# jordi-adell/mcarray

Hardware: AMD Instinct MI355X
Metric: STFT frames/sec, 8-mic GCC-PHAT + SRP-PHAT(361) + delay-and-sum beamform @48kHz/1024-pt (higher is better)
Workload: dtype f32 (SRP operands adaptive); 1 GPU; BASELINE configs[2] geometry (8-mic ULA 0.04 m, 48 kHz, N=1024, hop 512, 361 angles, 1 source, no power floor), 8 arrays x 4096 frames per GPU per step; channel rows padded by 64 floats; arrays_per_gpu=8, frames_per_array=4096, srp_precision=adaptive, parallelism=arrays sharded over 1 GPU(s), all_gather of DOA bins+prob

## Files before the change

include/mcarray_hip.h:

```cpp
#ifndef MCARRAY_HIP_H
#define MCARRAY_HIP_H

#ifdef __cplusplus
extern "C" {
#endif

typedef enum {
    MCA_HIP_OK = 0,
    MCA_HIP_ERR_INVALID_ARGUMENT = -1,
    MCA_HIP_ERR_HIP = -2,
    MCA_HIP_ERR_OUT_OF_MEMORY = -3,
    MCA_HIP_ERR_UNSUPPORTED = -4,
    MCA_HIP_ERR_NO_DEVICE = -5
} mca_hip_status;

typedef enum {
    MCA_HIP_SRP_FP32 = 0,
    MCA_HIP_SRP_FP16X3 = 1,
    MCA_HIP_SRP_FP16 = 2,
    MCA_HIP_SRP_ADAPTIVE = 3
} mca_hip_srp_precision;

typedef enum { MCA_HIP_GCC_PHAT = 0, MCA_HIP_GCC_NONE = 1 } mca_hip_gcc_weighting;

// ... 115 lines not shown
int mca_hip_mask_reset(mca_hip_mask_ctx *ctx);
int mca_hip_mask_get_thresholds(const mca_hip_mask_ctx *ctx, double *thresholds, double *center_freqs);
int mca_hip_mask_frames_dev(mca_hip_mask_ctx *ctx, const float *pcm_dev, long long stream_stride, long long ch_stride,
                            int n_streams, int n_frames, float *out_pcm_dev, int *decisions_dev, void *stream);
int mca_hip_mask_frames_host(mca_hip_mask_ctx *ctx, const float *pcm, int n_streams, int n_frames, float *out_pcm,
                             int *decisions);
int mca_hip_mask_process_frame(mca_hip_mask_ctx *ctx, double *left, double *right, int ccs_len, int *decisions);
long long mca_hip_mask_state_size(const mca_hip_mask_ctx *ctx);
int mca_hip_mask_state_save(mca_hip_mask_ctx *ctx, void *blob, long long blob_bytes);
int mca_hip_mask_state_load(mca_hip_mask_ctx *ctx, const void *blob, long long blob_bytes);

typedef struct mca_hip_mb_ctx mca_hip_mb_ctx;
typedef struct {
    int struct_size;
    int device;
    int sample_rate;
    int fft_size;
    const double *mic_xyz;
    int nbins;
    int use_power_floor;
    int max_arrays;
} mca_hip_mb_config;
int  mca_hip_mb_create(const mca_hip_mb_config *cfg, mca_hip_mb_ctx **out);
void mca_hip_mb_destroy(mca_hip_mb_ctx *ctx);
const char *mca_hip_mb_last_error(const mca_hip_mb_ctx *ctx);
int  mca_hip_mb_reset(mca_hip_mb_ctx *ctx, void *stream);
int  mca_hip_mb_num_steps(const mca_hip_mb_ctx *ctx);
int  mca_hip_mb_get_filters(const mca_hip_mb_ctx *ctx, double *out);
int mca_hip_mb_frames_dev(mca_hip_mb_ctx *ctx, const float *pcm_dev, long long array_stride, long long ch_stride,
                          int n_arrays, int n_frames, float *doa_rad_dev, float *prob_dev, unsigned char *voiced_dev,
                          float *power_dev, int *band_idx_dev, float *energy_in_doa_dev, float *band_corr_dev, void *stream);
int mca_hip_mb_frames_host(mca_hip_mb_ctx *ctx, const float *pcm, int n_arrays, int n_frames, float *doa_rad, float *prob,
                           unsigned char *voiced, float *power, int *band_idx, float *energy_in_doa, float *band_corr);
long long mca_hip_mb_state_size(const mca_hip_mb_ctx *ctx);
int mca_hip_mb_state_save(mca_hip_mb_ctx *ctx, void *blob, long long blob_bytes);
int mca_hip_mb_state_load(mca_hip_mb_ctx *ctx, const void *blob, long long blob_bytes);

typedef struct mca_hip_mvdr_ctx mca_hip_mvdr_ctx;
typedef struct {
    int struct_size;
    int device;
    int sample_rate;
    int fft_size;
    int n_mics;
    const double *mic_xyz;
    double alpha;
    double loading;
    int max_streams;
} mca_hip_mvdr_config;
int  mca_hip_mvdr_create(const mca_hip_mvdr_config *cfg, mca_hip_mvdr_ctx **out);
void mca_hip_mvdr_destroy(mca_hip_mvdr_ctx *ctx);
const char *mca_hip_mvdr_last_error(const mca_hip_mvdr_ctx *ctx);
int  mca_hip_mvdr_reset(mca_hip_mvdr_ctx *ctx, void *stream);
int mca_hip_mvdr_frames_dev(mca_hip_mvdr_ctx *ctx, const float *pcm_dev, long long stream_stride, long long mic_stride,
                            int n_streams, int n_frames, const float *doa_rad_dev, float *out_pcm_dev,
                            float *out_spec_dev, void *stream);
int mca_hip_mvdr_frames_host(mca_hip_mvdr_ctx *ctx, const float *pcm, int n_streams, int n_frames, const float *doa_rad,
                             float *out_pcm, float *out_spec);
int mca_hip_mvdr_get_covariance(mca_hip_mvdr_ctx *ctx, int stream_index, double *out);
long long mca_hip_mvdr_state_size(const mca_hip_mvdr_ctx *ctx);
int mca_hip_mvdr_state_save(mca_hip_mvdr_ctx *ctx, void *blob, long long blob_bytes);
int mca_hip_mvdr_state_load(mca_hip_mvdr_ctx *ctx, const void *blob, long long blob_bytes);
int mca_hip_mvdr_set_timing(mca_hip_mvdr_ctx *ctx, int enable);
int mca_hip_mvdr_get_timing(mca_hip_mvdr_ctx *ctx, int kernel_id, int *launches, double *total_ms);

typedef enum {
    MCA_HIP_K_STFT_PHAT = 0,
    MCA_HIP_K_SRP_GEMM = 1,
    MCA_HIP_K_SCAN_PICK = 2,
    MCA_HIP_K_BEAMFORM = 3,
    MCA_HIP_K_GCC2_SCAN = 4,
    MCA_HIP_K_MASK = 5,
    MCA_HIP_K_FOLD = 6,
    MCA_HIP_K_REPAIR = 7,
    MCA_HIP_K_COUNT = 8
} mca_hip_kernel_id;
int mca_hip_set_timing(mca_hip_ctx *ctx, int enable);
int mca_hip_set_timing_mask(mca_hip_ctx *ctx, unsigned kernel_mask);
int mca_hip_get_timing(mca_hip_ctx *ctx, int kernel_id, int *launches, double *total_ms);
int mca_hip_reset_timing(mca_hip_ctx *ctx);
int mca_hip_get_repair_stats(mca_hip_ctx *ctx, unsigned long long *frames, unsigned long long *flagged_frames,
                             unsigned long long *recomputed_frames);
int mca_hip_get_repair_columns(mca_hip_ctx *ctx, unsigned long long *candidate_columns, unsigned long long *whole_row_frames);

const char *mca_hip_version(void);

#ifdef __cplusplus
}
#endif
#endif
```

mcarray_amd/_lib.py:

```python
import ctypes as C
import os

_HERE = os.path.dirname(os.path.abspath(__file__))
LIB_PATH = os.environ.get("MCA_HIP_LIB", os.path.join(_HERE, "libmcarray_hip.so"))

c_dp = C.POINTER(C.c_double)
c_fp = C.POINTER(C.c_float)
c_ip = C.POINTER(C.c_int)


class MCArrayHipError(RuntimeError):
    """Raised for every non-zero status of the C ABI (the C++ side throws mca::MCArrayException)."""


class Config(C.Structure):
    _fields_ = [
        ("struct_size", C.c_int),
        ("device", C.c_int),
        ("sample_rate", C.c_int),
        ("fft_size", C.c_int),
        ("n_mics", C.c_int),
        ("mic_xyz", c_dp),
        ("doa_step_deg", C.c_double),
        ("n_sources", C.c_int),
# ... 66 lines not shown
    ("mca_hip_state_load", C.c_int, [C.c_void_p, C.c_void_p, C.c_longlong]),
    ("mca_hip_localise_frames_dev", C.c_int,
     [C.c_void_p, C.c_void_p, C.c_longlong, C.c_longlong, C.c_int, C.c_int, C.c_void_p, C.c_void_p, C.c_void_p,
      C.c_void_p, C.c_void_p]),
    ("mca_hip_separate_frames_dev", C.c_int,
     [C.c_void_p, C.c_void_p, C.c_longlong, C.c_longlong, C.c_int, C.c_int, C.c_void_p, C.c_void_p, C.c_void_p]),
    ("mca_hip_separate_frames_bins_dev", C.c_int,
     [C.c_void_p, C.c_void_p, C.c_longlong, C.c_longlong, C.c_int, C.c_int, C.c_void_p, C.c_void_p, C.c_void_p, C.c_void_p]),
    ("mca_hip_process_frames_dev", C.c_int,
     [C.c_void_p, C.c_void_p, C.c_longlong, C.c_longlong, C.c_int, C.c_int, C.c_void_p, C.c_void_p, C.c_void_p,
      C.c_void_p, C.c_void_p, C.c_void_p]),
    ("mca_hip_copy_gate", C.c_int, [C.c_void_p, C.c_void_p, c_fp]),
    ("mca_hip_process_frames_host", C.c_int,
     [C.c_void_p, c_fp, C.c_int, C.c_int, c_ip, c_fp, c_fp, c_fp, c_fp]),
    ("mca_hip_steering_process_frame", C.c_int,
     [C.c_void_p, C.POINTER(c_dp), C.c_int, c_dp, c_dp, c_ip, C.c_int]),
    ("mca_hip_beamformer_process_frame", C.c_int, [C.c_void_p, C.POINTER(c_dp), C.c_int, c_dp, C.c_double]),
    ("mca_hip_fft_log_power", C.c_int, [C.c_void_p, C.POINTER(c_dp), C.c_int, c_dp]),
    ("mca_hip_get_energy", C.c_int, [C.c_void_p, c_dp]),
    ("mca_hip_gcc2_frames_dev", C.c_int,
     [C.c_void_p, C.c_void_p, C.c_longlong, C.c_longlong, C.c_int, C.c_int, C.c_void_p, C.c_void_p, C.c_void_p,
      C.c_void_p, C.c_void_p]),
    ("mca_hip_gcc2_frames_host", C.c_int, [C.c_void_p, c_fp, C.c_int, C.c_int, c_ip, c_fp, c_fp, c_fp]),
    ("mca_hip_gcc2_set_probability", C.c_int, [C.c_void_p, C.c_int, c_dp, c_dp, C.c_int]),
    ("mca_hip_gcc2_set_probability_dev", C.c_int, [C.c_void_p, C.c_int, C.c_void_p, C.c_void_p, C.c_int, C.c_void_p]),
    ("mca_hip_gcc2_process_frame", C.c_int,
     [C.c_void_p, C.POINTER(c_dp), C.c_int, c_ip, c_dp, c_dp, c_dp, c_ip, c_dp]),
    ("mca_hip_gcc2_frame_set_probability", C.c_int, [C.c_void_p, c_dp, c_dp, C.c_int]),
    ("mca_hip_mask_create", C.c_int, [C.POINTER(MaskConfig), C.POINTER(C.c_void_p)]),
    ("mca_hip_mask_destroy", None, [C.c_void_p]),
    ("mca_hip_mask_last_error", C.c_char_p, [C.c_void_p]),
    ("mca_hip_mask_reset", C.c_int, [C.c_void_p]),
    ("mca_hip_mask_get_thresholds", C.c_int, [C.c_void_p, c_dp, c_dp]),
    ("mca_hip_mask_frames_dev", C.c_int,
     [C.c_void_p, C.c_void_p, C.c_longlong, C.c_longlong, C.c_int, C.c_int, C.c_void_p, C.c_void_p, C.c_void_p]),
    ("mca_hip_mask_frames_host", C.c_int, [C.c_void_p, c_fp, C.c_int, C.c_int, c_fp, c_ip]),
    ("mca_hip_mask_process_frame", C.c_int, [C.c_void_p, c_dp, c_dp, C.c_int, c_ip]),
    ("mca_hip_mb_create", C.c_int, [C.POINTER(MbConfig), C.POINTER(C.c_void_p)]),
    ("mca_hip_mb_destroy", None, [C.c_void_p]),
    ("mca_hip_mb_last_error", C.c_char_p, [C.c_void_p]),
    ("mca_hip_mb_reset", C.c_int, [C.c_void_p, C.c_void_p]),
    ("mca_hip_mb_num_steps", C.c_int, [C.c_void_p]),
    ("mca_hip_mb_get_filters", C.c_int, [C.c_void_p, c_dp]),
    ("mca_hip_mb_frames_dev", C.c_int,
     [C.c_void_p, C.c_void_p, C.c_longlong, C.c_longlong, C.c_int, C.c_int, C.c_void_p, C.c_void_p, C.c_void_p,
      C.c_void_p, C.c_void_p, C.c_void_p, C.c_void_p, C.c_void_p]),
    ("mca_hip_mb_frames_host", C.c_int,
     [C.c_void_p, c_fp, C.c_int, C.c_int, c_fp, c_fp, C.c_void_p, c_fp, c_ip, c_fp, c_fp]),
    ("mca_hip_process_frames_host_i16", C.c_int, [C.c_void_p, C.POINTER(C.c_short), C.c_int, C.c_int, c_ip, c_fp, c_fp, c_fp, c_fp]),
    ("mca_hip_graph_create", C.c_int,
     [C.c_void_p, C.c_void_p, C.c_longlong, C.c_longlong, C.c_int, C.c_int, C.c_void_p, C.c_void_p, C.c_void_p, C.c_void_p, C.c_void_p,
      C.POINTER(C.c_void_p)]),
    ("mca_hip_graph_launch", C.c_int, [C.c_void_p, C.c_void_p]),
    ("mca_hip_graph_destroy", None, [C.c_void_p]),
    ("mca_hip_mvdr_create", C.c_int, [C.POINTER(MvdrConfig), C.POINTER(C.c_void_p)]),
    ("mca_hip_mvdr_destroy", None, [C.c_void_p]),
    ("mca_hip_mvdr_last_error", C.c_char_p, [C.c_void_p]),
    ("mca_hip_mvdr_reset", C.c_int, [C.c_void_p, C.c_void_p]),
    ("mca_hip_mvdr_frames_dev", C.c_int,
     [C.c_void_p, C.c_void_p, C.c_longlong, C.c_longlong, C.c_int, C.c_int, C.c_void_p, C.c_void_p, C.c_void_p, C.c_void_p]),
    ("mca_hip_mvdr_frames_host", C.c_int, [C.c_void_p, c_fp, C.c_int, C.c_int, c_fp, c_fp, c_fp]),
    ("mca_hip_mvdr_get_covariance", C.c_int, [C.c_void_p, C.c_int, c_dp]),
    ("mca_hip_mvdr_set_timing", C.c_int, [C.c_void_p, C.c_int]),
    ("mca_hip_mvdr_get_timing", C.c_int, [C.c_void_p, C.c_int, c_ip, c_dp]),
    ("mca_hip_mask_state_size", C.c_longlong, [C.c_void_p]),
    ("mca_hip_mask_state_save", C.c_int, [C.c_void_p, C.c_void_p, C.c_longlong]),
    ("mca_hip_mask_state_load", C.c_int, [C.c_void_p, C.c_void_p, C.c_longlong]),
    ("mca_hip_mb_state_size", C.c_longlong, [C.c_void_p]),
    ("mca_hip_mb_state_save", C.c_int, [C.c_void_p, C.c_void_p, C.c_longlong]),
    ("mca_hip_mb_state_load", C.c_int, [C.c_void_p, C.c_void_p, C.c_longlong]),
    ("mca_hip_mvdr_state_size", C.c_longlong, [C.c_void_p]),
    ("mca_hip_mvdr_state_save", C.c_int, [C.c_void_p, C.c_void_p, C.c_longlong]),
    ("mca_hip_mvdr_state_load", C.c_int, [C.c_void_p, C.c_void_p, C.c_longlong]),
    ("mca_hip_set_timing", C.c_int, [C.c_void_p, C.c_int]),
    ("mca_hip_set_timing_mask", C.c_int, [C.c_void_p, C.c_uint]),
    ("mca_hip_get_timing", C.c_int, [C.c_void_p, C.c_int, c_ip, c_dp]),
    ("mca_hip_reset_timing", C.c_int, [C.c_void_p]),
    ("mca_hip_host_alloc", C.c_void_p, [C.c_longlong]),
    ("mca_hip_host_free", None, [C.c_void_p]),
    ("mca_hip_host_register", C.c_int, [C.c_void_p, C.c_longlong]),
    ("mca_hip_host_unregister", C.c_int, [C.c_void_p]),
    ("mca_hip_get_repair_stats", C.c_int, [C.c_void_p, C.POINTER(C.c_ulonglong), C.POINTER(C.c_ulonglong), C.POINTER(C.c_ulonglong)]),
    ("mca_hip_get_repair_columns", C.c_int, [C.c_void_p, C.POINTER(C.c_ulonglong), C.POINTER(C.c_ulonglong)]),
    ("mca_hip_version", C.c_char_p, []),
]

_LIB = None


def _pin_single_hip_runtime():
    import importlib.util
    spec = importlib.util.find_spec("torch")
    if spec is None or not spec.submodule_search_locations:
        return
    cand = os.path.join(list(spec.submodule_search_locations)[0], "lib", "libamdhip64.so")
    if os.path.exists(cand):
        C.CDLL(cand, mode=C.RTLD_GLOBAL)


def load():
    global _LIB
    if _LIB is None:
        if not os.path.exists(LIB_PATH):
            raise MCArrayHipError(
                "%s not found: the HIP extension is not built (run __graft_entry__.build()); "
                "mcarray_amd has no CPU fallback" % LIB_PATH)
        _pin_single_hip_runtime()
        lib = C.CDLL(LIB_PATH)
        for name, res, args in SYMBOLS:
            fn = getattr(lib, name)
            fn.restype = res
            fn.argtypes = args
        _LIB = lib
    return _LIB
```

mcarray_amd/api.py:

```python
import ctypes as C

import numpy as np

from . import _lib
from ._lib import MCArrayHipError

SRP_FP32, SRP_FP16X3, SRP_FP16, SRP_ADAPTIVE = 0, 1, 2, 3
GCC_PHAT, GCC_NONE = 0, 1
K_STFT_PHAT, K_SRP_GEMM, K_SCAN_PICK, K_BEAMFORM, K_GCC2_SCAN, K_MASK, K_FOLD, K_REPAIR = 0, 1, 2, 3, 4, 5, 6, 7
KERNEL_NAMES = {K_STFT_PHAT: "k_stft_phat", K_SRP_GEMM: "k_srp_gemm", K_SCAN_PICK: "k_scan_pick", K_BEAMFORM: "k_beamform_ola",
                K_FOLD: "k_sum_planes", K_REPAIR: "repair"}


class PinnedBuffer:

    def __init__(self, shape, dtype):
        self._lib = _lib.load()
        self.nbytes = int(np.prod(shape)) * np.dtype(dtype).itemsize
        self.ptr = self._lib.mca_hip_host_alloc(max(self.nbytes, 1))
        if not self.ptr:
            raise MCArrayHipError("mca_hip_host_alloc(%d) failed" % self.nbytes)
        raw = (C.c_char * max(self.nbytes, 1)).from_address(self.ptr)
        self.array = np.frombuffer(raw, dtype=dtype, count=int(np.prod(shape))).reshape(shape)

# ... 200 lines not shown
    def gcc2_set_probability(self, doas, array_index=0):
        doas = np.ascontiguousarray(doas, dtype=np.float64).reshape(-1)
        probs = np.empty(len(doas))
        self._check(self._lib.mca_hip_gcc2_set_probability(self.h, int(array_index), doas.ctypes.data_as(_lib.c_dp),
                                                           probs.ctypes.data_as(_lib.c_dp), len(doas)))
        return probs

    def gcc2_set_probability_dev(self, doas, probs, stream=None):
        if doas.dim() != 2 or tuple(probs.shape) != tuple(doas.shape) or not doas.is_contiguous() or not probs.is_contiguous():
            raise MCArrayHipError("doas and probs must be contiguous [A][n] tensors of one shape")
        A, n = doas.shape
        self._check(self._lib.mca_hip_gcc2_set_probability_dev(self.h, A, C.c_void_p(doas.data_ptr()), C.c_void_p(probs.data_ptr()), n,
                                                               stream))

    def gcc2_process_frame(self, frames):
        frames, arr = self._rows(frames)
        v, i = C.c_int(0), C.c_int(0)
        doa, prob, power = C.c_double(0), C.c_double(0), C.c_double(0)
        corr = np.empty(self.D)
        self._check(self._lib.mca_hip_gcc2_process_frame(self.h, arr, frames.shape[1], C.byref(v), C.byref(doa), C.byref(prob),
                                                         C.byref(power), C.byref(i), corr.ctypes.data_as(_lib.c_dp)))
        return dict(voiced=bool(v.value), doa=doa.value, prob=prob.value, power=power.value, argmax=i.value, corr=corr)

    def gcc2_frame_set_probability(self, doas):
        doas = np.ascontiguousarray(doas, dtype=np.float64).reshape(-1)
        probs = np.empty(len(doas))
        self._check(self._lib.mca_hip_gcc2_frame_set_probability(self.h, doas.ctypes.data_as(_lib.c_dp), probs.ctypes.data_as(_lib.c_dp),
                                                                 len(doas)))
        return probs

    def _rows(self, frames):
        frames = np.ascontiguousarray(frames, dtype=np.float64)
        if frames.shape[0] != self.M:
            raise MCArrayHipError("expected %d channel spectra" % self.M)
        arr = (_lib.c_dp * self.M)()
        for c in range(self.M):
            arr[c] = frames[c].ctypes.data_as(_lib.c_dp)
        return frames, arr

    def steering_process_frame(self, frames, n_sources=1):
        frames, arr = self._rows(frames)
        doa = np.empty(n_sources)
        prob = np.empty(n_sources)
        bins = np.empty(n_sources, dtype=np.int32)
        self._check(self._lib.mca_hip_steering_process_frame(self.h, arr, frames.shape[1], doa.ctypes.data_as(_lib.c_dp),
                                                             prob.ctypes.data_as(_lib.c_dp), bins.ctypes.data_as(_lib.c_ip),
                                                             n_sources))
        return doa, prob, bins

    def beamformer_process_frame(self, frames, doa):
        frames, arr = self._rows(frames)
        out = np.empty(frames.shape[1])
        self._check(self._lib.mca_hip_beamformer_process_frame(self.h, arr, frames.shape[1], out.ctypes.data_as(_lib.c_dp), float(doa)))
        return out

    def fft_log_power(self, frames):
        frames, arr = self._rows(frames)
        p = C.c_double(0)
        self._check(self._lib.mca_hip_fft_log_power(self.h, arr, frames.shape[1], C.byref(p)))
        return p.value

    def energy(self):
        out = np.empty(self.D)
        self._check(self._lib.mca_hip_get_energy(self.h, out.ctypes.data_as(_lib.c_dp)))
        return out

    def set_timing(self, enable):
        self._check(self._lib.mca_hip_set_timing(self.h, int(enable)))

    def set_timing_kernels(self, kernel_ids):
        mask = 0
        for k in kernel_ids:
            mask |= 1 << int(k)
        self._check(self._lib.mca_hip_set_timing_mask(self.h, mask))

    def reset_timing(self):
        self._check(self._lib.mca_hip_reset_timing(self.h))

    def repair_stats(self):
        a, b, c_ = C.c_ulonglong(0), C.c_ulonglong(0), C.c_ulonglong(0)
        self._check(self._lib.mca_hip_get_repair_stats(self.h, C.byref(a), C.byref(b), C.byref(c_)))
        return {"frames": a.value, "flagged": b.value, "recomputed": c_.value}

    def repair_columns(self):
        a, b = C.c_ulonglong(0), C.c_ulonglong(0)
        self._check(self._lib.mca_hip_get_repair_columns(self.h, C.byref(a), C.byref(b)))
        return {"candidate_columns": a.value, "whole_row_frames": b.value}

    def get_timing(self, kernel_id):
        n = C.c_int(0)
        ms = C.c_double(0)
        self._check(self._lib.mca_hip_get_timing(self.h, kernel_id, C.byref(n), C.byref(ms)))
        return n.value, ms.value


class StreamGraph:

    def __init__(self, ctx, h, keep):
        self.ctx, self.h, self._keep = ctx, h, keep
        self._lib = ctx._lib

    def launch(self, stream=None):
        rc = self.ctx._lib.mca_hip_graph_launch(self.h, stream)
        if rc != 0:
            raise MCArrayHipError("libmcarray_hip error %d: %s" % (rc, self.ctx._lib.mca_hip_last_error(self.ctx.h).decode()))

    def close(self):
        if getattr(self, "h", None):
            self._lib.mca_hip_graph_destroy(self.h)
        self.h = None

    def __del__(self):
        self.close()


class SteeringBeamforming:

    def __init__(self, sample_rate, mic_positions, fft_ccs_length, nchannels=None, doa_step_deg=5.0, device=0):
        self.ctx = Context(sample_rate, mic_positions, fft_ccs_length - 2, doa_step_deg, n_sources=4, device=device)
        if nchannels is not None and nchannels != self.ctx.M:
            raise MCArrayHipError("nchannels does not match the array description")

    def process_frame(self, analysis_frames, n_sources=1):
        return self.ctx.steering_process_frame(analysis_frames, n_sources)


class Beamformer:

    def __init__(self, sample_rate, mic_positions, fft_ccs_length, nchannels=None, device=0):
        self.ctx = Context(sample_rate, mic_positions, fft_ccs_length - 2, device=device)

    def process_frame(self, analysis_frames, doa):
        return self.ctx.beamformer_process_frame(analysis_frames, doa)


def calculate_order_from_sample_rate(sample_rate, frame_seconds):
    order = int(np.floor(np.log2(sample_rate * frame_seconds) + 0.5))
    return min(max(order, 8), 14)


class SourceSeparationAndLocalisation:

    FRAME_SECONDS = 0.025

    def __init__(self, sample_rate, mic_positions, n_sources=1, use_power_floor=False, doa_step_deg=5.0, fft_size=None,
                 srp_precision=SRP_FP32, device=0):
        if fft_size is None:
            fft_size = 1 << calculate_order_from_sample_rate(sample_rate, self.FRAME_SECONDS)
        self.ctx = Context(sample_rate, mic_positions, fft_size, doa_step_deg, n_sources, use_power_floor, srp_precision, 1, device)
        self.callback = None

    def set_callback(self, cb):
        self.callback = cb

    def process(self, pcm):
        r = self.ctx.process_frames_host(np.asarray(pcm, dtype=np.float32)[None], want_energy=False, want_audio=True)
        if self.callback is not None:
            deg = r["doa"][0].astype(np.float64) * (180.0 / np.pi)
            for t in range(deg.shape[0]):
                if "voiced" in r and not r["voiced"][0, t]:
                    continue
                self.callback(deg[t], r["prob"][0, t], r["power"][0, t] if "power" in r else None, self.ctx.S)
        return r["out"][0], r


class SourceLocalisation(SourceSeparationAndLocalisation):
# ... 309 lines not shown
```

mcarray_amd/csrc/api.hip:

```cpp
#include "../../include/mcarray_hip.h"
#include "fft1024c.h"
#include "kernels.h"
#include "knobs.h"
#include "stage.h"

#include <chrono>
#include <cmath>
#include <cstdio>
#include <cstdlib>
#include <cstring>
#include <string>
#include <thread>
#include <vector>

using namespace mca;

namespace {

std::string g_create_error;

struct TimedEvent { int id; hipEvent_t a, b; };

}

struct mca_hip_graph;

#define MCA_MAX_LANES 1

constexpr int FB_LAG = 2, FB_RING = 64, FB_WAIT_MS = 4000;
struct Knobs {
    bool fb_enabled = true;
    long long adapt_min_rows = 4096;
    int adapt_max_sources = 1;
    double tau_scale = 1.0;
    long long ws_max_bytes = 4LL << 30;
    bool force_generic = false;
    bool no_n2048 = false;
    bool scan_carry = false;
    int cand = -1;
    bool lazy_tails = true;
};

constexpr int REPAIR_ITEMS = 768;
constexpr int LIST_GRID = 512;
constexpr int CAND_GRID = 512;
constexpr int REPICK_GRID = 256;

struct Workspace {
    void *d_A = nullptr; size_t a_bytes = 0;
    void *d_Ax = nullptr; size_t ax_bytes = 0;
    float *d_C = nullptr; size_t c_bytes = 0;
    int c_planes = 1;
    bool partial_done = false;
    int part_planes = 1;
    long long c_plane = 0;
    float *d_Cx = nullptr; size_t cx_bytes = 0;
    float *d_part = nullptr, *d_estart = nullptr; int *d_nv = nullptr; size_t scan_ws_chunks = 0;
    float *d_power = nullptr; unsigned char *d_voiced = nullptr; float *d_power_out = nullptr; size_t gate_frames = 0;
    int *d_list_full = nullptr, *d_need_full = nullptr;
    unsigned char *d_flags = nullptr; int *d_chunk_from = nullptr, *d_list = nullptr, *d_need = nullptr; unsigned *d_umask = nullptr; size_t adapt_frames = 0, adapt_chunks = 0, adapt_groups = 0;
    unsigned char *d_unsure = nullptr;
    int *d_nlist = nullptr, *d_last_vchunk = nullptr; size_t lastv_arrays = 0;
    int last_a0 = 0, last_arrays = 0;
    void release()
    {
        auto F = [](void *q) { if (q) (void)hipFree(q); };
        F(d_A); F(d_Ax); F(d_C); F(d_Cx); F(d_part); F(d_estart); F(d_nv); F(d_power); F(d_voiced); F(d_power_out);
        F(d_flags); F(d_chunk_from); F(d_list); F(d_need); F(d_umask); F(d_nlist); F(d_last_vchunk); F(d_unsure); F(d_list_full); F(d_need_full);
        *this = Workspace();
    }
};

struct G2FrameState {
    double power_floor = 0, samples = 0, noise_estimated = 0;
    double silence = 0;
    double corr_mem = 0, doa_mem = 0;
    double doa = 0, prob = -1;
};

struct mca_hip_ctx {
    mca_hip_config cfg{};
    std::vector<double> xyz;
    int M = 0, P = 0, G = 0, D = 0, Dp = 0, K = 0, N = 0, H = 0, logH = 0, Kp = 0, S = 1, prec = 0;
    bool ula = false, stream_ok = false, generic = false;
    bool n512 = false;
    bool n2048 = false;
    std::string stream_why;
    float step = 0.f;
    std::vector<float> delays, grid;
    std::vector<int2> pairs;
    float *d_window = nullptr, *d_grid = nullptr, *d_delays = nullptr;
    float2 *d_tw = nullptr;
    double *d_micx = nullptr;
    int2 *d_pairs = nullptr;
    void *d_B = nullptr, *d_Bt = nullptr;
    bool merged = false; int n_merged = 0, Kp_m = 0;
    void *d_Bm = nullptr, *d_Btm = nullptr; unsigned short *d_mrank = nullptr;
    float2 *d_bftab = nullptr; int bf_pairs = 0;
    float *d_E[2] = {nullptr, nullptr};
    float *d_tail[2] = {nullptr, nullptr};
    int e_cur = 0, tail_cur = 0;
    Workspace lanes[MCA_MAX_LANES];
    int cur_lane = 0, a0 = 0;
    long long plan_rows = 0;
    int plan_arrays = 0;
    int n_lanes_last = 1;
    hipStream_t io_stream[3] = {}; hipEvent_t io_ev[8] = {};
    Workspace &ws() { return lanes[cur_lane]; }
    double *d_gate_state = nullptr;
    int *d_last_bin = nullptr; float *d_last_rad = nullptr, *d_last_prob = nullptr;
    int last_arrays = 0, last_frames = 0;
    float *d_doa[2] = {nullptr, nullptr};
    int doa_cur = 0;
    long long gcc2_frames_done = 0;
    long long *d_vdone[2] = {nullptr, nullptr};
    int *d_g2_vidx = nullptr, *d_g2_nv = nullptr; float *d_g2_rad = nullptr, *d_g2_prob = nullptr; size_t g2_rows = 0;
    unsigned char *d_g2_reset = nullptr;
    int *d_g2_post0 = nullptr;
    int *d_silence = nullptr;
    unsigned long long ws_gen = 0;
    std::vector<mca_hip_graph *> graphs;
    int tab_planes = 1;
    unsigned long long *d_rstats = nullptr;
    float *d_hist_pcm[2] = {nullptr, nullptr};
    float *d_hist_C[2] = {nullptr, nullptr};
    float *d_ehist[2] = {nullptr, nullptr};
    int hist_cur = 0, hist_n = 0;
    bool hist_pending = false;
    bool lazy_now = false;
    bool host_call = false;
    bool lazy_entry = false;
    int n_cu = 256;
    unsigned long long adapt_frames_total = 0;
    float tau_en = 0.f;
    Knobs kn;
    bool adapt_suspended = false, capturing = false;
    int fb_left = 0, fb_backoff = 8, fb_state = 0;
    bool cand_heavy = false;
    unsigned long long fb_probe_seq = 0;
    unsigned long long *h_probe = nullptr;
    unsigned long long fb_calls = 0, fb_seq_seen = 0, fb_groups_prev = 0, fb_frames_prev = 0, fb_flagged_prev = 0;
    unsigned long long fb_frames_ring[FB_RING] = {};
    unsigned long long fb_m = 0;
    unsigned long long fb_launch_m[FB_RING] = {};
    bool fb_lost = false;
    int a_row_elems = 0, a_planes = 1, a_elem = 4;
    double *d_fr = nullptr; size_t fr_elems = 0;
    double *d_E64[2] = {nullptr, nullptr}; int e64_cur = 0;
    double *d_res = nullptr;
    int *d_bins = nullptr;
    double *d_out64 = nullptr; size_t out64_elems = 0;
    double *d_g2f_corr[2] = {nullptr, nullptr}; int g2f_cur = 0;
    double *d_g2f_res = nullptr;
    G2FrameState g2f;
    std::vector<double> h_stage;
    StagePool stage;
    unsigned timing = 0;
    bool timing_open = false;
    std::vector<TimedEvent> events;
    std::vector<hipEvent_t> pool;
    int t_launches[MCA_HIP_K_COUNT] = {};
    double t_ms[MCA_HIP_K_COUNT] = {};
    std::string err;
};

namespace {

int fail(mca_hip_ctx *c, int code, const std::string &msg)
{
    if (c) c->err = msg; else g_create_error = msg;
    return code;
}

#define HIP_TRY(ctx, expr)                                                                              \
    do {                                                                                                \
        hipError_t _e = (expr);                                                                         \
        if (_e != hipSuccess)                                                                           \
            return fail(ctx, _e == hipErrorOutOfMemory ? MCA_HIP_ERR_OUT_OF_MEMORY : MCA_HIP_ERR_HIP,   \
                        std::string(#expr) + ": " + hipGetErrorString(_e));                            \
    } while (0)

double speed_of_sound() { return 346.1; }
float doa_idx2angle(int idx, float step) { float pr = (float)idx * step; return (float)((double)pr - M_PI_2); }
float doa_to_delay_far_field(float doa, float microDist)
{
    return (float)(((double)microDist * std::sin((double)doa)) / speed_of_sound());
}
float doa_to_delay_samples(float doa, float microDist, int fs) { return doa_to_delay_far_field(doa, microDist) * (float)fs; }
double distance(const std::vector<double> &xyz, int i, int j)
{
    return std::sqrt(std::pow(xyz[3 * j] - xyz[3 * i], 2) + std::pow(xyz[3 * j + 1] - xyz[3 * i + 1], 2) +
                     std::pow(xyz[3 * j + 2] - xyz[3 * i + 2], 2));
}

void free_ctx(mca_hip_ctx *c)
{
    if (!c) return;
    auto F = [](void *p) { if (p) (void)hipFree(p); };
    F(c->d_window); F(c->d_tw); F(c->d_grid); F(c->d_delays); F(c->d_micx); F(c->d_pairs); F(c->d_B); F(c->d_Bt); F(c->d_bftab); F(c->d_Bm); F(c->d_Btm); F(c->d_mrank);
    F(c->d_E[0]); F(c->d_E[1]); F(c->d_tail[0]); F(c->d_tail[1]); F(c->d_doa[0]); F(c->d_doa[1]); F(c->d_vdone[0]); F(c->d_vdone[1]); F(c->d_g2_vidx); F(c->d_g2_nv); F(c->d_g2_rad); F(c->d_g2_prob);
    F(c->d_g2_reset); F(c->d_g2_post0); F(c->d_silence);
    F(c->d_rstats); F(c->d_gate_state);
    for (int i = 0; i < 2; ++i) { F(c->d_hist_pcm[i]); F(c->d_hist_C[i]); F(c->d_ehist[i]); }
    if (c->h_probe) (void)hipHostFree(c->h_probe);
    for (Workspace &w : c->lanes) w.release();
    for (auto &e : c->io_ev) if (e) (void)hipEventDestroy(e);
    for (auto &q : c->io_stream) if (q) (void)hipStreamDestroy(q);
    F(c->d_last_bin); F(c->d_last_rad); F(c->d_last_prob);
    F(c->d_fr); F(c->d_E64[0]); F(c->d_E64[1]); F(c->d_res); F(c->d_bins); F(c->d_out64);
    F(c->d_g2f_corr[0]); F(c->d_g2f_corr[1]); F(c->d_g2f_res);
    c->stage.release();
    for (auto &e : c->events) { (void)hipEventDestroy(e.a); (void)hipEventDestroy(e.b); }
    for (auto &e : c->pool) (void)hipEventDestroy(e);
    delete c;
}

int round_up(int v, int m) { return (v + m - 1) / m * m; }

Knobs read_knobs(const mca_hip_config &cfg)
{
    Knobs k;
    auto geti = [](const char *v, long long dflt) { return v ? std::atoll(v) : dflt; };
    k.fb_enabled = cfg.adaptive_fallback != MCA_HIP_ADAPT_FALLBACK_OFF;
    if (const char *v = env_str("MCA_HIP_ADAPT_FALLBACK")) k.fb_enabled = std::atoi(v) != 0;
    k.adapt_min_rows = geti(env_str("MCA_HIP_ADAPT_MIN_ROWS"), cfg.adaptive_min_rows > 0 ? cfg.adaptive_min_rows : 4096);
    k.adapt_max_sources = (int)geti(env_str("MCA_HIP_ADAPT_MAX_SOURCES"), cfg.adaptive_max_sources > 0 ? cfg.adaptive_max_sources : 1);
    if (const char *v = env_str("MCA_HIP_ADAPT_TAU_SCALE")) k.tau_scale = std::atof(v);
    if (const char *v = env_str("MCA_HIP_WS_MAX_MB")) k.ws_max_bytes = (long long)std::atoll(v) << 20;
    k.force_generic = env_str("MCA_HIP_FORCE_GENERIC") != nullptr;
    k.scan_carry = cfg.scan_carry != 0 || env_str("MCA_HIP_SCAN_CARRY") != nullptr;
    if (const char *v = env_str("MCA_HIP_ADAPT_LAZY")) k.lazy_tails = std::atoi(v) != 0;
    if (const char *v = env_str("MCA_HIP_ADAPT_CAND")) k.cand = std::atoi(v) != 0 ? 1 : 0;
    k.no_n2048 = env_str("MCA_HIP_NO_N2048") != nullptr;
    return k;
}

int init_last_state(mca_hip_ctx *c, hipStream_t st)
{
    const size_t n = (size_t)c->cfg.max_arrays * MCA_MAX_SOURCES;
    std::vector<int> b(n, -1); std::vector<float> pr(n, -1.f);
    HIP_TRY(c, hipMemcpyAsync(c->d_last_bin, b.data(), n * 4, hipMemcpyHostToDevice, st));
    HIP_TRY(c, hipMemsetAsync(c->d_last_rad, 0, n * 4, st));
    HIP_TRY(c, hipMemcpyAsync(c->d_last_prob, pr.data(), n * 4, hipMemcpyHostToDevice, st));
    HIP_TRY(c, hipMemsetAsync(c->d_gate_state, 0, (size_t)c->cfg.max_arrays * 4 * 8, st));
    HIP_TRY(c, hipStreamSynchronize(st));
    return MCA_HIP_OK;
}

int build_steering_table(mca_hip_ctx *c)
{
    const int K = c->K, D = c->D, Dp = c->Dp, Kp = c->Kp;
    std::vector<int> first_pair(c->G);
    if (c->ula) { for (int g = 0; g < c->G; ++g) first_pair[g] = g;  }
    else for (int g = 0; g < c->G; ++g) first_pair[g] = g;
    const double N = 2.0 * (K - 1);
    if (c->prec == MCA_HIP_SRP_FP32) {
        std::vector<float> B((size_t)Kp * Dp, 0.f);
        for (int g = 0; g < c->G; ++g)
            for (int k = 0; k < K; ++k)
                for (int d = 0; d < D; ++d) {
                    double ph = 2.0 * M_PI * (double)k * (double)c->delays[(size_t)first_pair[g] * D + d] / N;
                    size_t r = ((size_t)g * K + k) * 2;
                    B[r * Dp + d] = (float)std::cos(ph);
                    B[(r + 1) * Dp + d] = (float)(-std::sin(ph));
                }
        HIP_TRY(c, hipMalloc(&c->d_B, B.size() * sizeof(float)));
        HIP_TRY(c, hipMemcpy(c->d_B, B.data(), B.size() * sizeof(float), hipMemcpyHostToDevice));
    } else {
        const int planes = c->tab_planes;
        std::vector<_Float16> B((size_t)planes * Dp * Kp, (_Float16)0.f);
        for (int g = 0; g < c->G; ++g)
            for (int d = 0; d < D; ++d)
                for (int k = 0; k < K; ++k) {
                    double ph = 2.0 * M_PI * (double)k * (double)c->delays[(size_t)first_pair[g] * D + d] / N;
                    float v[2] = {(float)std::cos(ph), (float)(-std::sin(ph))};
                    for (int q = 0; q < 2; ++q) {
                        size_t kk = ((size_t)g * K + k) * 2 + q;
                        _Float16 hi = (_Float16)v[q];
                        B[(size_t)d * Kp + kk] = hi;
                        if (planes == 2) B[((size_t)Dp + d) * Kp + kk] = (_Float16)(v[q] - (float)hi);
                    }
                }
        HIP_TRY(c, hipMalloc(&c->d_B, B.size() * sizeof(_Float16)));
        HIP_TRY(c, hipMemcpy(c->d_B, B.data(), B.size() * sizeof(_Float16), hipMemcpyHostToDevice));
        if (Dp == 384) {
            const int ns32 = Kp / 32;
            std::vector<_Float16> Bt(B.size());
// ... 382 lines not shown
{
    StftPhatArgs sa = a;
    const int fp = c->M == 4 ? 2 : 1, mr = c->M == 4 ? 4 : 8;
    if (!sa.list) {
        sa.fpb = 16;
        while (sa.fpb > 2 && (long long)grid.y * ((sa.n_frames + sa.fpb - 1) / sa.fpb) < 512) sa.fpb >>= 1;
        grid.x = (sa.n_frames + sa.fpb - 1) / sa.fpb;
    }
    const size_t smem6 = ((size_t)fp * mr * 1026 + F1K_TWORDS + 8 * F1K_SCRATCH + (size_t)sa.fpb * c->M) * sizeof(float2) + (size_t)sa.fpb * 8 * sizeof(float);
#define L2048(MT, U)                                                                                                      \
    do {                                                                                                                  \
        HIP_TRY(c, hipFuncSetAttribute(reinterpret_cast<const void *>(&k_stft_phat_2048<MT, U, OutT, false>), hipFuncAttributeMaxDynamicSharedMemorySize, (int)smem6)); \
        hipLaunchKernelGGL((k_stft_phat_2048<MT, U, OutT, false>), grid, dim3(512), smem6, st, sa);                              \
    } while (0)
    bool done = false;
    if constexpr (sizeof(OutT) == 2) {
        if (sa.mrank && sa.a_planes == 1 && !sa.list && c->ula && (c->M == 8 || c->M == 4)) {
            if (c->M == 8) {
                HIP_TRY(c, hipFuncSetAttribute(reinterpret_cast<const void *>(&k_stft_phat_2048<8, true, _Float16, true>), hipFuncAttributeMaxDynamicSharedMemorySize, (int)smem6));
                hipLaunchKernelGGL((k_stft_phat_2048<8, true, _Float16, true>), grid, dim3(512), smem6, st, sa);
            } else {
                HIP_TRY(c, hipFuncSetAttribute(reinterpret_cast<const void *>(&k_stft_phat_2048<4, true, _Float16, true>), hipFuncAttributeMaxDynamicSharedMemorySize, (int)smem6));
                hipLaunchKernelGGL((k_stft_phat_2048<4, true, _Float16, true>), grid, dim3(512), smem6, st, sa);
            }
            done = true;
        }
    }
    if (done) { }
    else if (c->M == 8 && c->ula) L2048(8, true); else if (c->M == 8) L2048(8, false);
    else if (c->M == 4 && c->ula) L2048(4, true); else if (c->M == 4) L2048(4, false);
    else if (c->ula) L2048(0, true); else L2048(0, false);
#undef L2048
    HIP_TRY(c, hipGetLastError());
    return MCA_HIP_OK;
}

template <typename OutT>
int launch_stft(mca_hip_ctx *c, const StftPhatArgs &a, dim3 grid, size_t smem, hipStream_t st)
{
    const int M = c->M; const bool ula = c->ula;
    if (n2048_analysis(c)) return launch_stft_2048<OutT>(c, a, grid, st);
    if (c->n512) return launch_stft_512<OutT>(c, a, grid, st);
    if constexpr (sizeof(OutT) == 2) {
        if (wave16_applies(c) && a.a_planes == 1 && !a.list) {
            StftPhatArgs w = a;
            w.fpb = 16;
            while (w.fpb > 1 && (long long)grid.y * ((a.n_frames + w.fpb - 1) / w.fpb) < 2048) w.fpb >>= 1;
            dim3 gw(((a.n_frames + w.fpb - 1) / w.fpb + 3) / 4, grid.y);
            if ((gw.x & 1) == 0 && (long long)gw.x * gw.y == 2LL * c->n_cu && (long long)gw.x * 4 * w.fpb == a.n_frames) {
                const int sk = (3 * w.fpb + 8) / 16;
                if (sk > 0 && sk < w.fpb) { w.skew = sk; gw = dim3(gw.y, gw.x); }
            }
            const int fpa = w.fpb + w.skew;
            const size_t smw = (size_t)(F1K_TWORDS + 4 * F1K_SCRATCH + 2 * 4 * fpa * 8) * sizeof(float2) + (1024 + 4 * fpa) * sizeof(float);
            if (a.power) {
                HIP_TRY(c, hipFuncSetAttribute(reinterpret_cast<const void *>(&k_stft_phat_wave16<true>), hipFuncAttributeMaxDynamicSharedMemorySize, (int)smw));
                hipLaunchKernelGGL(k_stft_phat_wave16<true>, gw, dim3(256), smw, st, w);
            } else {
                HIP_TRY(c, hipFuncSetAttribute(reinterpret_cast<const void *>(&k_stft_phat_wave16<false>), hipFuncAttributeMaxDynamicSharedMemorySize, (int)smw));
                hipLaunchKernelGGL(k_stft_phat_wave16<false>, gw, dim3(256), smw, st, w);
            }
            HIP_TRY(c, hipGetLastError());
            return MCA_HIP_OK;
        }
    }
    if (M == 8 || M == 4) {
        StftPhatArgs w = a;
        dim3 gw;
        if (a.list) { w.fpb = 1; gw = dim3(grid.x, 1); }
        else {
            w.fpb = 16;
            while (w.fpb > 1 && (long long)grid.y * ((a.n_frames + w.fpb - 1) / w.fpb) < 2048) w.fpb >>= 1;
            gw = dim3(((a.n_frames + w.fpb - 1) / w.fpb + 3) / 4, grid.y);
        }
        if (!a.list && M == 8 && (gw.x & 1) == 0 && (long long)gw.x * gw.y == 2LL * c->n_cu && (long long)gw.x * 4 * w.fpb == a.n_frames) {
            const int sk = (3 * w.fpb + 8) / 16;
            if (sk > 0 && sk < w.fpb) {
                w.skew = sk;
                gw = dim3(gw.y, gw.x);
            }
        }
        const bool mg = w.mrank != nullptr && !a.list;
        const int nrank = 2 * (M - 1) * 64 * 4 + 8, regw = mg ? std::max(F1K_SCRATCH, (w.n_merged + 63) & ~63) : F1K_SCRATCH;
        const size_t smw = (size_t)(F1K_TWORDS + (mg ? nrank / 4 : 0) + 4 * regw + (mg ? 0 : 4 * (w.fpb + w.skew) * (M / 2))) * sizeof(float2);
        const bool pl2 = a.a_planes == 2, pw = a.power != nullptr;
#define LAUNCH_K(K)                                                                                                 \
        do {                                                                                                         \
            if (smw > 64 * 1024) HIP_TRY(c, hipFuncSetAttribute(reinterpret_cast<const void *>(&K), hipFuncAttributeMaxDynamicSharedMemorySize, (int)smw)); \
            hipLaunchKernelGGL(K, gw, dim3(256), smw, st, w);                                                        \
        } while (0)
#define LAUNCH_W2(MT, U, PL2, NP)                                                                                  \
        do {                                                                                                         \
            if (pw) LAUNCH_K((k_stft_phat_wave<MT, U, OutT, PL2, true, NP, false>));                                 \
            else LAUNCH_K((k_stft_phat_wave<MT, U, OutT, PL2, false, NP, false>));                                   \
        } while (0)
#define LAUNCH_W(MT, U)                                                                                              \
        do {                                                                                                         \
            if constexpr (sizeof(OutT) == 2) {                                                                       \
                if (pl2 && w.cand_on && a.list && !pw) LAUNCH_K((k_stft_phat_wave<MT, U, OutT, true, false, false, false, true>)); \
                else if (pl2) LAUNCH_W2(MT, U, true, false); else LAUNCH_W2(MT, U, false, false);                    \
            }                                                                                                        \
            else { if (a.no_phat) LAUNCH_W2(MT, U, false, true); else LAUNCH_W2(MT, U, false, false); }              \
        } while (0)
        if constexpr (sizeof(OutT) == 2) {
            if (mg) {
                if (M == 8) { if (pw) LAUNCH_K((k_stft_phat_wave<8, true, OutT, false, true, false, true>)); else LAUNCH_K((k_stft_phat_wave<8, true, OutT, false, false, false, true>)); }
                else { if (pw) LAUNCH_K((k_stft_phat_wave<4, true, OutT, false, true, false, true>)); else LAUNCH_K((k_stft_phat_wave<4, true, OutT, false, false, false, true>)); }
                HIP_TRY(c, hipGetLastError());
                return MCA_HIP_OK;
            }
        }
        if (M == 8 && ula) LAUNCH_W(8, true); else if (M == 8) LAUNCH_W(8, false);
        else if (ula) LAUNCH_W(4, true); else LAUNCH_W(4, false);
#undef LAUNCH_W2
#undef LAUNCH_K
#undef LAUNCH_W
        HIP_TRY(c, hipGetLastError());
        return MCA_HIP_OK;
    }
#define LAUNCH(MT, U)                                                                                        \
    do {                                                                                                     \
        if (smem > 64 * 1024)                                                                                \
            HIP_TRY(c, hipFuncSetAttribute(reinterpret_cast<const void *>(&k_stft_phat<MT, U, OutT>),        \
                                           hipFuncAttributeMaxDynamicSharedMemorySize, (int)smem));          \
        hipLaunchKernelGGL((k_stft_phat<MT, U, OutT>), grid, dim3(512), smem, st, a);                        \
    } while (0)
#define LAUNCH_FEW(MT, U)                                                                                    \
    do {                                                                                                     \
        const size_t smf = ((size_t)8 * FFT_SCRATCH + TW_WORDS + (size_t)a.fpb * MT) * sizeof(float2) + (size_t)a.fpb * 8 * sizeof(float); \
        if (smf > 64 * 1024)                                                                                 \
            HIP_TRY(c, hipFuncSetAttribute(reinterpret_cast<const void *>(&k_stft_phat_few<MT, U, OutT>),    \
                                           hipFuncAttributeMaxDynamicSharedMemorySize, (int)smf));           \
        hipLaunchKernelGGL((k_stft_phat_few<MT, U, OutT>), grid, dim3(512), smf, st, a);                     \
    } while (0)
    if (M == 2 && !ula) LAUNCH_FEW(2, false);
    else if (M == 16 && ula) LAUNCH(16, true);
    else if (ula) LAUNCH(0, true);
    else LAUNCH(0, false);
#undef LAUNCH
#undef LAUNCH_FEW
    HIP_TRY(c, hipGetLastError());
    return MCA_HIP_OK;
}

int check_stream_args(mca_hip_ctx *c, const float *pcm, long long array_stride, long long mic_stride, int n_arrays, int n_frames)
{
    if (!c) return MCA_HIP_ERR_INVALID_ARGUMENT;
    if (!c->stream_ok) return fail(c, MCA_HIP_ERR_UNSUPPORTED, c->stream_why);
    if (!pcm) return fail(c, MCA_HIP_ERR_INVALID_ARGUMENT, "pcm_dev is NULL");
    if (n_arrays < 1 || n_arrays > c->cfg.max_arrays) return fail(c, MCA_HIP_ERR_INVALID_ARGUMENT, "n_arrays outside [1, max_arrays]");
    if (n_frames < 1) return fail(c, MCA_HIP_ERR_INVALID_ARGUMENT, "n_frames < 1");
    const long long need = (long long)(n_frames + 1) * c->H;
    if (mic_stride < need) return fail(c, MCA_HIP_ERR_INVALID_ARGUMENT, "mic_stride shorter than (n_frames+1)*hop samples");
    if (n_arrays > 1 && array_stride < (long long)(c->M - 1) * mic_stride + need) return fail(c, MCA_HIP_ERR_INVALID_ARGUMENT, "array_stride too short");
    if ((mic_stride & 1) || (array_stride & 1) || (reinterpret_cast<uintptr_t>(pcm) & 7))
        return fail(c, MCA_HIP_ERR_INVALID_ARGUMENT, "pcm_dev must be 8-byte aligned with even strides (float2 loads)");
    return MCA_HIP_OK;
}

}

extern "C" {

static int settle_history(mca_hip_ctx *c, hipStream_t st);

const char *mca_hip_version(void) { return "mcarray-hip 0.1.0 (gfx950)"; }

const char *mca_hip_last_error(const mca_hip_ctx *ctx) { return ctx ? ctx->err.c_str() : g_create_error.c_str(); }

int mca_hip_create(const mca_hip_config *cfg, mca_hip_ctx **out)
{
    if (!cfg || !out) return fail(nullptr, MCA_HIP_ERR_INVALID_ARGUMENT, "cfg/out is NULL");
    *out = nullptr;
    constexpr int size_r2 = (int)offsetof(mca_hip_config, gcc_weighting), size_r3 = (size_r2 + 4 + 7) / 8 * 8;
    static_assert(size_r3 <= (int)offsetof(mca_hip_config, adaptive_min_rows), "round-3 struct size");
    if (cfg->struct_size != (int)sizeof(mca_hip_config) && cfg->struct_size != size_r2 && cfg->struct_size != size_r3)
        return fail(nullptr, MCA_HIP_ERR_INVALID_ARGUMENT, "struct_size mismatch");
    mca_hip_config cfg_full{};
    std::memcpy(&cfg_full, cfg, cfg->struct_size == size_r3 ? (size_t)offsetof(mca_hip_config, adaptive_fallback) : (size_t)cfg->struct_size);
    cfg_full.struct_size = (int)sizeof(mca_hip_config);
    cfg = &cfg_full;
    if (cfg->gcc_weighting != MCA_HIP_GCC_PHAT && cfg->gcc_weighting != MCA_HIP_GCC_NONE)
        return fail(nullptr, MCA_HIP_ERR_INVALID_ARGUMENT, "gcc_weighting must be MCA_HIP_GCC_PHAT or MCA_HIP_GCC_NONE");
    if (cfg->gcc_weighting == MCA_HIP_GCC_NONE && cfg->srp_precision != MCA_HIP_SRP_FP32)
        return fail(nullptr, MCA_HIP_ERR_UNSUPPORTED, "gcc_weighting NONE needs srp_precision MCA_HIP_SRP_FP32 (un-normalised spectra do not fit fp16 operands)");
    if (cfg->n_mics < 2 || cfg->n_mics > MCA_MAX_MICS) return fail(nullptr, MCA_HIP_ERR_INVALID_ARGUMENT, "n_mics must be in [2,16]");
    if (!cfg->mic_xyz) return fail(nullptr, MCA_HIP_ERR_INVALID_ARGUMENT, "mic_xyz is NULL");
    if (cfg->n_sources < 1 || cfg->n_sources > MCA_MAX_SOURCES) return fail(nullptr, MCA_HIP_ERR_INVALID_ARGUMENT, "n_sources must be in [1,4]");
    if (cfg->fft_size < 16 || (cfg->fft_size & 1) || cfg->fft_size > 8192) return fail(nullptr, MCA_HIP_ERR_INVALID_ARGUMENT, "fft_size must be even, 16..8192");
// ... 105 lines not shown
        (rc = zalloc((void **)&c->d_tail[0], na * c->S * c->H * 4)) || (rc = zalloc((void **)&c->d_tail[1], na * c->S * c->H * 4)) ||
        (rc = zalloc((void **)&c->d_gate_state, na * 4 * 8)) || (rc = zalloc((void **)&c->d_last_bin, na * MCA_MAX_SOURCES * 4)) ||
        (rc = zalloc((void **)&c->d_last_rad, na * MCA_MAX_SOURCES * 4)) || (rc = zalloc((void **)&c->d_last_prob, na * MCA_MAX_SOURCES * 4)) ||
        (rc = zalloc((void **)&c->d_doa[0], na * 4)) || (rc = zalloc((void **)&c->d_doa[1], na * 4)) ||
        (rc = zalloc((void **)&c->d_vdone[0], na * 8)) || (rc = zalloc((void **)&c->d_vdone[1], na * 8)) ||
        (rc = zalloc((void **)&c->d_silence, na * 4)) || (rc = zalloc((void **)&c->d_g2_post0, na * 4)) ||
        (rc = zalloc((void **)&c->d_rstats, 32)) ||
        (rc = zalloc((void **)&c->d_E64[0], c->D * 8)) || (rc = zalloc((void **)&c->d_E64[1], c->D * 8)) ||
        (rc = zalloc((void **)&c->d_res, (2 * MCA_MAX_SOURCES + 1) * 8)) || (rc = zalloc((void **)&c->d_bins, MCA_MAX_SOURCES * 4)) ||
        (rc = zalloc((void **)&c->d_g2f_corr[0], c->D * 8)) || (rc = zalloc((void **)&c->d_g2f_corr[1], c->D * 8)) ||
        (rc = zalloc((void **)&c->d_g2f_res, 4 * 8))) {
        g_create_error = c->err; free_ctx(c); return rc;
    }
    if (lazy_context(c)) {
        for (int i = 0; i < 2; ++i)
            if ((rc = zalloc((void **)&c->d_hist_pcm[i], na * c->M * HIST_SAMPLES * 4)) || (rc = zalloc((void **)&c->d_hist_C[i], na * HIST_FRAMES * c->Dp * 4)) ||
                (rc = zalloc((void **)&c->d_ehist[i], na * c->D * 4))) { g_create_error = c->err; free_ctx(c); return rc; }
    }
    if (c->prec == MCA_HIP_SRP_ADAPTIVE && c->kn.fb_enabled) {
        if (hipHostMalloc((void **)&c->h_probe, FB_RING * 32, hipHostMallocDefault) == hipSuccess) std::memset(c->h_probe, 0, FB_RING * 32);
        else { c->h_probe = nullptr; (void)hipGetLastError(); }
    }
    if (c->stream_ok && ((rc = build_steering_table(c)) || (rc = build_merged_tables(c)))) { g_create_error = c->err; free_ctx(c); return rc; }
    if ((rc = init_last_state(c, nullptr))) { g_create_error = c->err; free_ctx(c); return rc; }
    *out = c;
    return MCA_HIP_OK;
}

static void graph_drop_recordings(mca_hip_graph *g);
static void graph_orphan(mca_hip_graph *g);

void mca_hip_destroy(mca_hip_ctx *ctx)
{
    if (!ctx) return;
    (void)hipSetDevice(ctx->cfg.device);
    (void)hipDeviceSynchronize();
    for (mca_hip_graph *g : ctx->graphs) graph_orphan(g);
    ctx->graphs.clear();
    free_ctx(ctx);
}

int mca_hip_num_steps(const mca_hip_ctx *c) { return c ? c->D : MCA_HIP_ERR_INVALID_ARGUMENT; }
int mca_hip_num_pairs(const mca_hip_ctx *c) { return c ? c->P : MCA_HIP_ERR_INVALID_ARGUMENT; }
int mca_hip_num_groups(const mca_hip_ctx *c) { return c ? c->G : MCA_HIP_ERR_INVALID_ARGUMENT; }

int mca_hip_get_pair_delays(const mca_hip_ctx *c, float *out)
{
    if (!c || !out) return MCA_HIP_ERR_INVALID_ARGUMENT;
    std::memcpy(out, c->delays.data(), c->delays.size() * sizeof(float));
    return MCA_HIP_OK;
}

int mca_hip_get_doa_grid(const mca_hip_ctx *c, float *out)
{
    if (!c || !out) return MCA_HIP_ERR_INVALID_ARGUMENT;
    std::memcpy(out, c->grid.data(), c->grid.size() * sizeof(float));
    return MCA_HIP_OK;
}

int mca_hip_reset(mca_hip_ctx *c, void *stream)
{
    if (!c) return MCA_HIP_ERR_INVALID_ARGUMENT;
    hipStream_t st = (hipStream_t)stream;
    const size_t na = (size_t)c->cfg.max_arrays;
    for (int i = 0; i < 2; ++i) {
        HIP_TRY(c, hipMemsetAsync(c->d_E[i], 0, na * c->D * 4, st));
        HIP_TRY(c, hipMemsetAsync(c->d_tail[i], 0, na * c->S * c->H * 4, st));
        HIP_TRY(c, hipMemsetAsync(c->d_E64[i], 0, (size_t)c->D * 8, st));
        HIP_TRY(c, hipMemsetAsync(c->d_g2f_corr[i], 0, (size_t)c->D * 8, st));
        HIP_TRY(c, hipMemsetAsync(c->d_doa[i], 0, na * 4, st));
        HIP_TRY(c, hipMemsetAsync(c->d_vdone[i], 0, na * 8, st));
    }
    HIP_TRY(c, hipMemsetAsync(c->d_silence, 0, na * 4, st));
    c->adapt_suspended = false; c->fb_state = 0; c->fb_left = 0; c->fb_backoff = 8; c->cand_heavy = false;
    c->fb_lost = false; c->fb_seq_seen = c->fb_calls;
    c->hist_pending = false;
    for (Workspace &w : c->lanes) {
        if (w.d_need) HIP_TRY(c, hipMemsetAsync(w.d_need, 0, w.adapt_groups * 4, st));
        if (w.d_need_full) HIP_TRY(c, hipMemsetAsync(w.d_need_full, 0, w.adapt_groups * 4, st));
        if (w.d_umask) HIP_TRY(c, hipMemsetAsync(w.d_umask, 0, w.adapt_groups * (c->Dp / 32) * 4, st));
        if (w.d_chunk_from) HIP_TRY(c, hipMemsetAsync(w.d_chunk_from, 0x7f, w.adapt_chunks * 4, st));
        if (w.d_nlist) HIP_TRY(c, hipMemsetAsync(w.d_nlist, 0, 16, st));
    }
    c->gcc2_frames_done = 0;
    c->g2f = G2FrameState();
    return init_last_state(c, st);
}

extern "C++" {
namespace {

struct StateHeader {
    unsigned magic; int version, M, D, S, H, max_arrays, use_floor;
    unsigned delays_hash;
    long long gcc2_frames_done;
};
constexpr unsigned STATE_MAGIC = 0x4d434153u;
constexpr int STATE_VERSION = 3;

unsigned delays_hash(const mca_hip_ctx *c)
{
    unsigned h = 2166136261u;
    const unsigned char *p = reinterpret_cast<const unsigned char *>(c->delays.data());
    for (size_t i = 0; i < c->delays.size() * sizeof(float); ++i) { h ^= p[i]; h *= 16777619u; }
    return h;
}

struct StatePart { void *ptr; size_t bytes; };
std::vector<StatePart> state_parts(mca_hip_ctx *c)
{
    const size_t na = (size_t)c->cfg.max_arrays;
    return {
        {c->d_E[c->e_cur], na * c->D * 4}, {c->d_tail[c->tail_cur], na * c->S * c->H * 4}, {c->d_gate_state, na * 4 * 8},
        {c->d_last_bin, na * MCA_MAX_SOURCES * 4}, {c->d_last_rad, na * MCA_MAX_SOURCES * 4}, {c->d_last_prob, na * MCA_MAX_SOURCES * 4},
        {c->d_doa[c->doa_cur], na * 4}, {c->d_E64[c->e64_cur], (size_t)c->D * 8}, {c->d_vdone[c->doa_cur], na * 8},
        {c->d_silence, na * 4},
        {c->d_g2f_corr[c->g2f_cur], (size_t)c->D * 8},
    };
}

size_t frame_part_bytes(const mca_hip_ctx *c) { return (size_t)c->D * 8 + sizeof(G2FrameState); }
static_assert(sizeof(G2FrameState) == 8 * sizeof(double), "G2FrameState is the 8 doubles of the blob");

}
}

long long mca_hip_state_size(const mca_hip_ctx *c)
{
    if (!c) return MCA_HIP_ERR_INVALID_ARGUMENT;
    long long n = sizeof(StateHeader) + (long long)sizeof(G2FrameState);
    for (const StatePart &p : state_parts(const_cast<mca_hip_ctx *>(c))) n += (long long)p.bytes;
    return n;
}

int mca_hip_state_save(mca_hip_ctx *c, void *blob, long long blob_bytes)
{
    if (!c) return MCA_HIP_ERR_INVALID_ARGUMENT;
    if (!blob || blob_bytes < mca_hip_state_size(c)) return fail(c, MCA_HIP_ERR_INVALID_ARGUMENT, "state blob is NULL or smaller than mca_hip_state_size()");
    HIP_TRY(c, hipSetDevice(c->cfg.device));
    if (c->hist_pending) {
        HIP_TRY(c, hipDeviceSynchronize());
        const int rc = settle_history(c, nullptr);
        if (rc) return rc;
    }
    HIP_TRY(c, hipDeviceSynchronize());
    StateHeader h{STATE_MAGIC, STATE_VERSION, c->M, c->D, c->S, c->H, c->cfg.max_arrays, c->cfg.use_power_floor, delays_hash(c), c->gcc2_frames_done};
    unsigned char *out = static_cast<unsigned char *>(blob);
    std::memcpy(out, &h, sizeof(h)); out += sizeof(h);
    for (const StatePart &p : state_parts(c)) { HIP_TRY(c, hipMemcpy(out, p.ptr, p.bytes, hipMemcpyDeviceToHost)); out += p.bytes; }
    std::memcpy(out, &c->g2f, sizeof(G2FrameState));
    return MCA_HIP_OK;
}

int mca_hip_state_load(mca_hip_ctx *c, const void *blob, long long blob_bytes)
{
    if (!c) return MCA_HIP_ERR_INVALID_ARGUMENT;
    if (!blob || blob_bytes < (long long)sizeof(StateHeader)) return fail(c, MCA_HIP_ERR_INVALID_ARGUMENT, "state blob is NULL or truncated");
    StateHeader h;
    std::memcpy(&h, blob, sizeof(h));
    if (h.magic != STATE_MAGIC || h.version < 1 || h.version > STATE_VERSION) return fail(c, MCA_HIP_ERR_INVALID_ARGUMENT, "not a state blob of this library version");
    if (h.M != c->M || h.D != c->D || h.S != c->S || h.H != c->H || h.max_arrays != c->cfg.max_arrays || h.use_floor != c->cfg.use_power_floor ||
        h.delays_hash != delays_hash(c))
        return fail(c, MCA_HIP_ERR_INVALID_ARGUMENT, "state blob was saved by a context with a different configuration");
    const long long short_by = (h.version == 1 ? (long long)c->cfg.max_arrays * 4 : 0) +
                               (h.version < 3 ? (long long)frame_part_bytes(c) : 0);
    if (blob_bytes < mca_hip_state_size(c) - short_by) return fail(c, MCA_HIP_ERR_INVALID_ARGUMENT, "state blob is truncated");
    HIP_TRY(c, hipSetDevice(c->cfg.device));
    HIP_TRY(c, hipDeviceSynchronize());
    const unsigned char *in = static_cast<const unsigned char *>(blob) + sizeof(h);
    for (const StatePart &p : state_parts(c)) {
        if (h.version == 1 && p.ptr == c->d_silence) { HIP_TRY(c, hipMemset(p.ptr, 0, p.bytes)); continue; }
        if (h.version < 3 && p.ptr == c->d_g2f_corr[c->g2f_cur]) { HIP_TRY(c, hipMemset(p.ptr, 0, p.bytes)); continue; }
        HIP_TRY(c, hipMemcpy(p.ptr, in, p.bytes, hipMemcpyHostToDevice)); in += p.bytes;
    }
    if (h.version >= 3) std::memcpy(&c->g2f, in, sizeof(G2FrameState));
    else c->g2f = G2FrameState();
    c->gcc2_frames_done = h.gcc2_frames_done;
    c->hist_pending = false;
    return MCA_HIP_OK;
}

static int reserve_lane(mca_hip_ctx *c, int n_arrays, int n_frames)
{
    const int n_chunks = (n_frames + SCAN_CHUNK - 1) / SCAN_CHUNK;
    int rc;
    if (c->prec == MCA_HIP_SRP_ADAPTIVE && adaptive_shape(c, n_arrays, n_frames)) {
        set_call_planes(c, 1);
        if ((rc = ensure_adapt_workspace(c, n_arrays, n_frames, n_chunks))) return rc;
        const long long fc1 = chunk_frames_for(c, n_arrays, n_frames);
        if ((rc = ensure_workspace(c, (long long)n_arrays * fc1, (long long)n_arrays * n_frames))) return rc;
        if (!c->adapt_suspended) return ensure_scan_workspace(c, n_arrays, n_frames, n_chunks);
    }
    if (c->prec == MCA_HIP_SRP_ADAPTIVE) set_call_planes(c, 2);
    long long fc = chunk_frames_for(c, n_arrays, n_frames);
    rc = ensure_workspace(c, (long long)n_arrays * fc, (long long)n_arrays * n_frames);
    if (rc) return rc;
    return ensure_scan_workspace(c, n_arrays, n_frames, n_chunks);
}

static int reserve_impl(mca_hip_ctx *c, int n_arrays, int n_frames)
{
    HIP_TRY(c, hipSetDevice(c->cfg.device));
    c->cur_lane = 0;
    return reserve_lane(c, n_arrays, n_frames);
}

int mca_hip_reserve(mca_hip_ctx *c, int n_arrays, int n_frames)
{
    if (!c || n_arrays < 1 || n_frames < 1) return MCA_HIP_ERR_INVALID_ARGUMENT;
    return reserve_impl(c, n_arrays, n_frames);
}

static int run_correlation_map(mca_hip_ctx *c, const float *pcm, long long array_stride, long long mic_stride,
                               int n_arrays, int n_frames, hipStream_t st)
{
    int rc;
    const long long fc = chunk_frames_for(c, n_arrays, n_frames);
    if ((rc = ensure_workspace(c, (long long)n_arrays * fc, (long long)n_arrays * n_frames))) return rc;
    if ((rc = ensure_scan_workspace(c, n_arrays, n_frames, (n_frames + SCAN_CHUNK - 1) / SCAN_CHUNK))) return rc;
    bool fused_partial = SCAN_CHUNK == 32 && c->a_planes == 1 && !c->cfg.use_power_floor && n_frames % SCAN_CHUNK == 0 && fc % SCAN_CHUNK == 0 &&
                         plan_gemm(c, (long long)n_arrays * fc).ksplit <= 2;
    for (int f0 = 0; fused_partial && f0 < n_frames; f0 += (int)fc)
        fused_partial = plan_gemm(c, (long long)n_arrays * std::min<long long>(fc, n_frames - f0)).v2;
    c->ws().partial_done = fused_partial;
    c->ws().part_planes = fused_partial ? plan_gemm(c, (long long)n_arrays * fc).ksplit : 1;
    for (int f0 = 0; f0 < n_frames; f0 += (int)fc) {
        const int nf = (int)std::min<long long>(fc, n_frames - f0);
        StftPhatArgs sa{};
        sa.pcm = pcm; sa.array_stride = array_stride; sa.mic_stride = mic_stride;
        sa.M = c->M; sa.n_frames = nf; sa.frame0 = f0;
        sa.fpb = 16;
        while (sa.fpb > 1 && (long long)n_arrays * ((nf + sa.fpb - 1) / sa.fpb) < 256) sa.fpb >>= 1;
        sa.power = c->cfg.use_power_floor ? c->ws().d_power : nullptr; sa.total_frames = n_frames;
        sa.window = c->d_window; sa.A = a_buf(c); sa.Kp = c->Kp; sa.a_row_elems = c->a_row_elems; sa.a_planes = c->a_planes;
        if (c->merged && c->a_planes == 1) { sa.mrank = c->d_mrank; sa.n_merged = c->n_merged; }
        sa.N = c->N; sa.logH = c->logH; sa.kg = c->K; sa.ula = c->ula ? 1 : 0; sa.tw = c->d_tw;
        sa.no_phat = c->cfg.gcc_weighting == MCA_HIP_GCC_NONE ? 1 : 0;
        if (c->prec == MCA_HIP_SRP_ADAPTIVE && c->a_planes == 1 && wave16_applies(c)) sa.unsure = c->ws().d_unsure;
        if (c->lazy_now && cand_call(c, true)) sa.dead = c->ws().d_unsure;
        if (c->lazy_now) sa.hist_out = c->d_hist_pcm[c->hist_cur ^ 1];
        time_begin(c, MCA_HIP_K_STFT_PHAT, st);
        if (c->n512) {
            rc = c->prec == MCA_HIP_SRP_FP32 ? launch_stft_512<float>(c, sa, dim3(0, n_arrays), st) : launch_stft_512<_Float16>(c, sa, dim3(0, n_arrays), st);
        } else if ((c->N == 4096 || c->N == 2048) && c->M == 2 && c->stream_ok) {
            sa.fpb = 8;
            while (sa.fpb > 2 && (long long)n_arrays * ((nf + sa.fpb - 1) / sa.fpb) < 512) sa.fpb >>= 1;
            const size_t smem4 = ((size_t)16 * 258 + 8 * FFT_SCRATCH + TW_WIN) * sizeof(float2) + 4 * 8 * sizeof(float);
            dim3 g4((nf + sa.fpb - 1) / sa.fpb, n_arrays);
#define LSUB(RR, T)                                                                                                       \
            do {                                                                                                          \
                HIP_TRY(c, hipFuncSetAttribute(reinterpret_cast<const void *>(&k_stft_phat_sub2<RR, T>), hipFuncAttributeMaxDynamicSharedMemorySize, (int)smem4)); \
                hipLaunchKernelGGL((k_stft_phat_sub2<RR, T>), g4, dim3(512), smem4, st, sa);                              \
            } while (0)
            if (c->N == 4096) { if (c->prec == MCA_HIP_SRP_FP32) LSUB(8, float); else LSUB(8, _Float16); }
            else { if (c->prec == MCA_HIP_SRP_FP32) LSUB(4, float); else LSUB(4, _Float16); }
#undef LSUB
            rc = MCA_HIP_OK;
        } else if (n2048_analysis(c)) {
            rc = c->prec == MCA_HIP_SRP_FP32 ? launch_stft_2048<float>(c, sa, dim3(0, n_arrays), st) : launch_stft_2048<_Float16>(c, sa, dim3(0, n_arrays), st);
        } else if (c->generic) {
            const size_t smem1 = (size_t)c->M * (c->H + 1) * sizeof(float2) + 16;
#define GEN_LAUNCH(K)                                                                                                     \
            do {                                                                                                          \
                if (smem1 > 64 * 1024)                                                                                    \
                    HIP_TRY(c, hipFuncSetAttribute(reinterpret_cast<const void *>(&K), hipFuncAttributeMaxDynamicSharedMemorySize, (int)smem1)); \
                hipLaunchKernelGGL(K, dim3(nf, n_arrays), dim3(gen_threads(c, false)), smem1, st, sa);                                      \
            } while (0)
            if (c->prec == MCA_HIP_SRP_FP32) GEN_LAUNCH(k_stft_phat_gen<float>);
            else GEN_LAUNCH(k_stft_phat_gen<_Float16>);
#undef GEN_LAUNCH
            rc = MCA_HIP_OK;
        } else {
            dim3 g1((nf + sa.fpb - 1) / sa.fpb, n_arrays);
            const size_t smem1 = ((size_t)c->M * FFT_SCRATCH + TW_WORDS + (size_t)sa.fpb * c->M) * sizeof(float2) + (size_t)sa.fpb * 8 * sizeof(float);
            rc = c->prec == MCA_HIP_SRP_FP32 ? launch_stft<float>(c, sa, g1, smem1, st) : launch_stft<_Float16>(c, sa, g1, smem1, st);
        }
        time_end(c, st);
        if (rc) return rc;

        GemmArgs ga{};
        const bool mg = c->merged && c->a_planes == 1;
        ga.A = a_buf(c); ga.B = mg ? c->d_Bm : c->d_B; ga.C = c->ws().d_C; ga.Bt = mg ? c->d_Btm : c->d_Bt;
        ga.rows = n_arrays * nf; ga.chunk_frames = nf; ga.total_frames = n_frames; ga.frame0 = f0;
        ga.Kp = cur_kp(c); ga.Dp = c->Dp; ga.a_row_elems = c->a_row_elems;
        ga.c_plane_elems = (long long)n_arrays * n_frames * c->Dp;
        if (fused_partial) {
            ga.part = c->ws().d_part; ga.nvoiced = c->ws().d_nv; ga.D = c->D; ga.n_chunks = n_frames / SCAN_CHUNK;
            ga.part_plane_stride = (long long)n_arrays * ga.n_chunks * c->D;
            ga.scan_w[31] = 1 - 0.8f;
            for (int t = 30; t >= 0; --t) ga.scan_w[t] = ga.scan_w[t + 1] * 0.8f;
        }
        const bool v2 = plan_gemm(c, ga.rows).v2;
        const int ksplit = plan_gemm(c, (long long)n_arrays * fc).ksplit;
        c->ws().c_planes = ksplit; c->ws().c_plane = ga.c_plane_elems;
        time_begin(c, MCA_HIP_K_SRP_GEMM, st);
        if (v2) {
            const int np = c->a_planes;
            const size_t smem = (size_t)(np == 2 ? 2 : 4) * np * (256 + 384) * 64;
            dim3 gv((ga.rows + 255) / 256, ksplit);
#define V2_LAUNCH(K)                                                                                                      \
            do {                                                                                                          \
                HIP_TRY(c, hipFuncSetAttribute(reinterpret_cast<const void *>(&K), hipFuncAttributeMaxDynamicSharedMemorySize, (int)smem)); \
                hipLaunchKernelGGL(K, gv, dim3(512), smem, st, ga);                                                       \
            } while (0)
            if (c->a_planes == 2) V2_LAUNCH(k_srp_gemm_f16_v2);
            else V2_LAUNCH(k_srp_gemm_f16_v3);
#undef V2_LAUNCH
        } else {
            dim3 g2((ga.rows + 127) / 128, c->Dp == 64 ? 1 : c->Dp / 192, ksplit);
            if (c->prec == MCA_HIP_SRP_FP32) hipLaunchKernelGGL(k_srp_gemm_f32, g2, dim3(256), 0, st, ga);
            else if (c->Dp == 64 && c->a_planes == 2) hipLaunchKernelGGL((k_srp_gemm_f16<true, 64>), g2, dim3(256), 0, st, ga);
            else if (c->Dp == 64) hipLaunchKernelGGL((k_srp_gemm_f16<false, 64>), g2, dim3(256), 0, st, ga);
            else if (c->a_planes == 2) hipLaunchKernelGGL((k_srp_gemm_f16<true, 192>), g2, dim3(256), 0, st, ga);
            else hipLaunchKernelGGL((k_srp_gemm_f16<false, 192>), g2, dim3(256), 0, st, ga);
        }
        time_end(c, st);
        HIP_TRY(c, hipGetLastError());
    }
    if (c->ws().c_planes > 2) {
        const long long n4 = c->ws().c_plane / 4;
        time_begin(c, MCA_HIP_K_FOLD, st);
        hipLaunchKernelGGL(k_sum_planes, dim3((unsigned)((n4 + 255) / 256)), dim3(256), 0, st, c->ws().d_C, n4, c->ws().c_planes, c->ws().c_plane);
        time_end(c, st);
// ... 159 lines not shown
        const int pass_groups = (int)(pass_rows / REPAIR_GROUP);
        const long long all_groups = (long long)n_arrays * (gpa + (hist_valid ? HIST_UNITS : 0));
        set_call_planes(c, 2);
        for (long long g0 = 0; g0 < all_groups; g0 += pass_groups) {
            StftPhatArgs sa{};
            sa.pcm = pcm; sa.array_stride = array_stride; sa.mic_stride = mic_stride;
            sa.M = c->M; sa.n_frames = n_frames; sa.frame0 = 0; sa.fpb = REPAIR_GROUP; sa.total_frames = n_frames;
            sa.window = c->d_window; sa.A = c->ws().d_Ax; sa.Kp = c->Kp; sa.a_row_elems = c->a_row_elems; sa.a_planes = 2;
            sa.N = c->N; sa.logH = c->logH; sa.kg = c->K; sa.ula = c->ula ? 1 : 0; sa.tw = c->d_tw;
            sa.list = c->ws().d_list; sa.n_list = c->ws().d_nlist; sa.list0 = (int)g0; sa.list_cap = pass_groups; sa.groups_per_array = gpa;
            if (hist_valid) { sa.hist_in = c->d_hist_pcm[c->hist_cur]; sa.hist_base = n_arrays * gpa; }
            CandArgs ca{};
            if (pa.umask) {
                ca.A = c->ws().d_Ax; ca.B = c->d_B; ca.Kp = c->Kp; ca.Dp = c->Dp; ca.a_row_elems = c->a_row_elems;
                ca.list = c->ws().d_list; ca.n_list = c->ws().d_nlist; ca.list0 = (int)g0; ca.pass_rows = (int)pass_rows;
                ca.umask = c->ws().d_umask; ca.umask_words = pa.umask_words; ca.need = c->ws().d_need; ca.groups_per_array = gpa; ca.n_frames = n_frames;
                ca.C = c->ws().d_C; ca.c_planes = c->ws().c_planes; ca.c_plane_stride = c->ws().c_plane;
                if (hist_valid) { ca.hist_C = c->d_hist_C[c->hist_cur]; ca.hist_base = n_arrays * gpa; }
                if (c->M == 8 || c->M == 4) { sa.cand_on = 1; sa.cand = ca; }
            }
            const size_t smem1 = ((size_t)c->M * FFT_SCRATCH + TW_WORDS + (size_t)sa.fpb * c->M) * sizeof(float2) + (size_t)sa.fpb * 8 * sizeof(float);
            if ((rc = launch_stft<_Float16>(c, sa, dim3(std::min(pass_groups, LIST_GRID), 1), smem1, st))) { set_call_planes(c, 1); return rc; }
            if (pa.umask && sa.cand_on) continue;
            if (pa.umask) {
                const long long max_items = pass_rows / REPAIR_GROUP;
                hipLaunchKernelGGL(k_srp_cand, dim3((unsigned)std::min<long long>(max_items, CAND_GRID)), dim3(1024), 0, st, ca);
                continue;
            }
            RepairPatchArgs pp{};
            pp.groups_per_array = gpa;
            pp.C = c->ws().d_C; pp.c_planes = c->ws().c_planes; pp.c_plane_stride = c->ws().c_plane; pp.n_frames = n_frames;
            if (hist_valid) { pp.hist_C = c->d_hist_C[c->hist_cur]; pp.hist_base = n_arrays * gpa; }
            launch_repair_contraction(c, c->ws(), g0, pass_rows, n_arrays, pp, st);
        }
        for (long long g0 = 0; mixed && g0 < all_groups; g0 += pass_groups) {
            StftPhatArgs sa{};
            sa.pcm = pcm; sa.array_stride = array_stride; sa.mic_stride = mic_stride;
            sa.M = c->M; sa.n_frames = n_frames; sa.frame0 = 0; sa.fpb = REPAIR_GROUP; sa.total_frames = n_frames;
            sa.window = c->d_window; sa.A = c->ws().d_Ax; sa.Kp = c->Kp; sa.a_row_elems = c->a_row_elems; sa.a_planes = 2;
            sa.N = c->N; sa.logH = c->logH; sa.kg = c->K; sa.ula = c->ula ? 1 : 0; sa.tw = c->d_tw;
            sa.list = pa.list_full; sa.n_list = pa.n_list_full; sa.list0 = (int)g0; sa.list_cap = pass_groups; sa.groups_per_array = gpa;
            const size_t smem1 = ((size_t)c->M * FFT_SCRATCH + TW_WORDS + (size_t)sa.fpb * c->M) * sizeof(float2) + (size_t)sa.fpb * 8 * sizeof(float);
            if ((rc = launch_stft<_Float16>(c, sa, dim3(std::min(pass_groups, LIST_GRID), 1), smem1, st))) { set_call_planes(c, 1); return rc; }
            RepairPatchArgs pp{};
            pp.groups_per_array = gpa;
            pp.C = c->ws().d_C; pp.c_planes = c->ws().c_planes; pp.c_plane_stride = c->ws().c_plane; pp.n_frames = n_frames;
            launch_repair_contraction(c, c->ws(), g0, pass_rows, n_arrays, pp, st, pa.list_full, pa.n_list_full, pa.need_full);
        }
        set_call_planes(c, 1);
        const size_t smem4 = (size_t)32 * (c->Dp + 8) * sizeof(float);
#define LAUNCH_REPICK(PL)                                                                                                           \
        do {                                                                                                                        \
            if (smem4 > 64 * 1024)                                                    \
                HIP_TRY(c, hipFuncSetAttribute(reinterpret_cast<const void *>(&k_scan_repick<PL>), hipFuncAttributeMaxDynamicSharedMemorySize, (int)smem4)); \
            hipLaunchKernelGGL((k_scan_repick<PL>), dim3((unsigned)std::min<long long>((long long)pa.n_chunks * n_arrays, REPICK_GRID)), dim3(std::max(nthr, 512)), smem4, st, pa); \
        } while (0)
        if (ppl == 2) LAUNCH_REPICK(2); else if (ppl == 6) LAUNCH_REPICK(6); else LAUNCH_REPICK(8);
#undef LAUNCH_REPICK
        if (gate) hipLaunchKernelGGL(k_doa_fill, dim3(n_arrays), dim3(1024), 0, st, fa);
        time_end(c, st);
        HIP_TRY(c, hipGetLastError());
        c->adapt_frames_total += (unsigned long long)n_arrays * n_frames;
    }
    if (lazy) { c->hist_cur ^= 1; c->hist_n = n_arrays; c->hist_pending = true; }
    else c->hist_pending = false;
    c->ws().last_a0 = c->a0; c->ws().last_arrays = n_arrays;
    return MCA_HIP_OK;
}

int mca_hip_get_repair_stats(mca_hip_ctx *c, unsigned long long *frames, unsigned long long *flagged_frames,
                             unsigned long long *recomputed_frames)
{
    if (!c) return MCA_HIP_ERR_INVALID_ARGUMENT;
    HIP_TRY(c, hipSetDevice(c->cfg.device));
    HIP_TRY(c, hipDeviceSynchronize());
    unsigned long long st[2] = {0, 0};
    HIP_TRY(c, hipMemcpy(st, c->d_rstats, sizeof(st), hipMemcpyDeviceToHost));
    if (frames) *frames = c->adapt_frames_total;
    if (flagged_frames) *flagged_frames = st[0];
    if (recomputed_frames) *recomputed_frames = st[1] * REPAIR_GROUP;
    return MCA_HIP_OK;
}

int mca_hip_get_repair_columns(mca_hip_ctx *c, unsigned long long *candidate_columns, unsigned long long *whole_row_frames)
{
    if (!c) return MCA_HIP_ERR_INVALID_ARGUMENT;
    HIP_TRY(c, hipSetDevice(c->cfg.device));
    HIP_TRY(c, hipDeviceSynchronize());
    unsigned long long st[4] = {0, 0, 0, 0};
    HIP_TRY(c, hipMemcpy(st, c->d_rstats, sizeof(st), hipMemcpyDeviceToHost));
    if (candidate_columns) *candidate_columns = st[2];
    if (whole_row_frames) *whole_row_frames = st[3];
    return MCA_HIP_OK;
}

static bool wave_beamformer_applies(const mca_hip_ctx *c)
{
    return !c->generic && !c->n512 && (c->S <= 2 || c->M <= 8) && c->M >= 2 && c->M <= MCA_MAX_MICS;
}

static int ensure_bf_table(mca_hip_ctx *c)
{
    if (!c->d_bftab && c->n2048) {
        HIP_TRY(c, hipMalloc((void **)&c->d_bftab, (size_t)(c->D + 1) * c->M * 1032 * sizeof(float2)));
        c->bf_pairs = c->M;
        const double unit = (double)c->cfg.sample_rate / (double)c->N / 346.1;
        hipLaunchKernelGGL(k_bf_table_2048, dim3(c->D + 1, c->M), dim3(256), 0, nullptr, c->d_bftab, c->d_grid, c->d_micx, c->M, unit);
        HIP_TRY(c, hipGetLastError());
        HIP_TRY(c, hipDeviceSynchronize());
        return MCA_HIP_OK;
    }
    if (c->d_bftab || !wave_beamformer_applies(c)) return MCA_HIP_OK;
    const int np = (c->M + 1) / 2;
    HIP_TRY(c, hipMalloc((void **)&c->d_bftab, (size_t)(c->D + 1) * np * 1024 * sizeof(float2)));
    c->bf_pairs = np;
    const double unit = (double)c->cfg.sample_rate / (double)FFT_N / 346.1;
    hipLaunchKernelGGL(k_bf_table, dim3(c->D + 1, np), dim3(256), 0, nullptr, c->d_bftab, c->d_grid, c->d_micx, c->M, np, unit);
    HIP_TRY(c, hipGetLastError());
    HIP_TRY(c, hipDeviceSynchronize());
    return MCA_HIP_OK;
}

static int separate_impl(mca_hip_ctx *c, const float *pcm, long long array_stride, long long mic_stride,
                         int n_arrays, int n_frames, const float *doa_rad, float *out_pcm, hipStream_t st, const int *doa_bin = nullptr)
{
    const size_t a0 = (size_t)c->a0;
    if (doa_bin && c->d_bftab && c->n2048 && (reinterpret_cast<uintptr_t>(out_pcm) & 7) == 0) {
        BeamformWaveArgs wa{};
        wa.pcm = pcm; wa.array_stride = array_stride; wa.mic_stride = mic_stride;
        wa.M = c->M; wa.n_pairs = c->M; wa.n_frames = n_frames; wa.S = c->S;
        wa.ft = 16;
        for (int ft = 2; ft <= 64; ++ft)
            if ((long long)n_arrays * c->S * ((n_frames + 4 * ft - 2) / (4 * ft - 1)) <= 2LL * c->n_cu) { wa.ft = ft; break; }
        wa.window = c->d_window; wa.doa_bin = doa_bin; wa.table = c->d_bftab; wa.out = out_pcm;
        wa.tail_in = c->d_tail[c->tail_cur] + a0 * c->S * c->H; wa.tail_out = c->d_tail[c->tail_cur ^ 1] + a0 * c->S * c->H;
        const int wgs = (n_frames + 4 * wa.ft - 2) / (4 * wa.ft - 1);
        const size_t smem_w = (size_t)(F1K_TWORDS + 4 * F1K_SCRATCH + 4 * 512) * sizeof(float2);
        time_begin(c, MCA_HIP_K_BEAMFORM, st);
        hipLaunchKernelGGL(k_beamform_wave_2048, dim3(wgs, n_arrays, c->S), dim3(256), smem_w, st, wa);
        time_end(c, st);
        HIP_TRY(c, hipGetLastError());
        return MCA_HIP_OK;
    }
    if (doa_bin && c->d_bftab && wave_beamformer_applies(c)) {
        BeamformWaveArgs wa{};
        wa.pcm = pcm; wa.array_stride = array_stride; wa.mic_stride = mic_stride;
        wa.M = c->M; wa.n_pairs = c->bf_pairs; wa.n_frames = n_frames; wa.S = c->S;
        wa.window = c->d_window; wa.doa_bin = doa_bin; wa.table = c->d_bftab; wa.out = out_pcm;
        wa.tail_in = c->d_tail[c->tail_cur] + a0 * c->S * c->H; wa.tail_out = c->d_tail[c->tail_cur ^ 1] + a0 * c->S * c->H;
        if (c->S >= 2 && c->M <= 8) {
            wa.ft = 16;
            while (wa.ft > 2 && (long long)n_arrays * ((n_frames + wa.ft - 1) / wa.ft) < 2048) wa.ft >>= 1;
            const int runs = (n_frames + wa.ft - 1) / wa.ft;
            const size_t smem_ms = (size_t)(F1K_TWORDS + 4 * F1K_SCRATCH) * sizeof(float2) + (size_t)4 * c->S * FFT_H * sizeof(float);
            const dim3 gms((runs + 3) / 4, n_arrays);
            time_begin(c, MCA_HIP_K_BEAMFORM, st);
#define BFMS(NPT)                                                                                                                   \
            do {                                                                                                                    \
                if (smem_ms > 64 * 1024) {                                                                                          \
                    HIP_TRY(c, hipFuncSetAttribute(reinterpret_cast<const void *>(&k_beamform_wave_ms<NPT, false>), hipFuncAttributeMaxDynamicSharedMemorySize, (int)smem_ms)); \
                    HIP_TRY(c, hipFuncSetAttribute(reinterpret_cast<const void *>(&k_beamform_wave_ms<NPT, true>), hipFuncAttributeMaxDynamicSharedMemorySize, (int)smem_ms));  \
                }                                                                                                                   \
                if (c->M & 1) hipLaunchKernelGGL((k_beamform_wave_ms<NPT, true>), gms, dim3(256), smem_ms, st, wa);                 \
                else hipLaunchKernelGGL((k_beamform_wave_ms<NPT, false>), gms, dim3(256), smem_ms, st, wa);                         \
            } while (0)
            if (c->bf_pairs == 1) {
                if (smem_ms > 64 * 1024) HIP_TRY(c, hipFuncSetAttribute(reinterpret_cast<const void *>(&k_beamform_wave_ms<1, false>), hipFuncAttributeMaxDynamicSharedMemorySize, (int)smem_ms));
                hipLaunchKernelGGL((k_beamform_wave_ms<1, false>), gms, dim3(256), smem_ms, st, wa);
            }
            else if (c->bf_pairs == 2) BFMS(2);
            else if (c->bf_pairs == 3) BFMS(3);
            else BFMS(4);
#undef BFMS
            time_end(c, st);
            HIP_TRY(c, hipGetLastError());
            return MCA_HIP_OK;
        }
        wa.ft = 2;
        while (wa.ft < 256 && (long long)n_arrays * c->S * ((n_frames + 4 * wa.ft - 2) / (4 * wa.ft - 1)) > 512) ++wa.ft;
        const int wgs = (n_frames + 4 * wa.ft - 2) / (4 * wa.ft - 1);
        const size_t smem = (size_t)(F1K_TWORDS + 4 * F1K_SCRATCH) * sizeof(float2) + 4 * FFT_H * sizeof(float);
        dim3 gb(wgs, n_arrays, c->S);
        if (c->S == 1 && (wgs & 1) == 0 && wa.ft >= 8 && (long long)wgs * n_arrays > (long long)c->n_cu * 3 / 2 && (long long)wgs * n_arrays <= 2LL * c->n_cu) {
            wa.skew = (3 * wa.ft + 8) / 16;
            if (wa.skew >= wa.ft) wa.skew = 0;
            else gb = dim3(n_arrays, wgs, c->S);
        }
        time_begin(c, MCA_HIP_K_BEAMFORM, st);
        if (c->M & 1) hipLaunchKernelGGL(k_beamform_wave<true>, gb, dim3(256), smem, st, wa);
        else hipLaunchKernelGGL(k_beamform_wave<false>, gb, dim3(256), smem, st, wa);
        time_end(c, st);
        HIP_TRY(c, hipGetLastError());
        return MCA_HIP_OK;
    }
    BeamformArgs ba{};
    ba.pcm = pcm; ba.array_stride = array_stride; ba.mic_stride = mic_stride;
    ba.M = c->M; ba.Mpad = c->M; ba.S = c->S; ba.n_frames = n_frames; ba.fs = c->cfg.sample_rate;
    ba.ft = 64;
    long long want_wgs = 512;
    if (c->generic) {
        const size_t smem_g = (size_t)(c->M + c->S) * (c->H + 1) * sizeof(float2) + (size_t)c->S * c->H * sizeof(float);
        const long long per_cu = std::max<long long>(1, std::min<long long>((160 * 1024) / (long long)smem_g, 2048 / gen_threads(c, true)));
// ... 35 lines not shown
        HIP_TRY(c, hipGetLastError());
        return MCA_HIP_OK;
    }
    ba.nb = std::max(1, BF_NB / c->S);
    const size_t smem = ((size_t)ba.M + ba.nb * c->S) * FFT_SCRATCH * sizeof(float2) + (size_t)c->S * c->M * 49 * sizeof(float2) +
                        TW_WORDS * sizeof(float2) + (size_t)ba.nb * c->M * (1 + c->S) * sizeof(float2) +
                        (size_t)(ba.ft + 1) * c->S * sizeof(double);
    if (smem > 160 * 1024) return fail(c, MCA_HIP_ERR_UNSUPPORTED, "n_mics/n_sources combination exceeds the 160 KiB LDS of a CU");
    dim3 g((n_frames + ba.ft - 1) / ba.ft, n_arrays);
    time_begin(c, MCA_HIP_K_BEAMFORM, st);
#define BF_LAUNCH(K)                                                                                                     \
    do {                                                                                                                 \
        if (smem > 64 * 1024)                                                                                            \
            HIP_TRY(c, hipFuncSetAttribute(reinterpret_cast<const void *>(&K), hipFuncAttributeMaxDynamicSharedMemorySize, (int)smem)); \
        hipLaunchKernelGGL(K, g, dim3(512), smem, st, ba);                                                               \
    } while (0)
    if (c->M <= 8) BF_LAUNCH((k_beamform_ola<1, 4>));
    else BF_LAUNCH((k_beamform_ola<2, 2>));
#undef BF_LAUNCH
    time_end(c, st);
    HIP_TRY(c, hipGetLastError());
    return MCA_HIP_OK;
}

int mca_hip_localise_frames_dev(mca_hip_ctx *c, const float *pcm, long long array_stride, long long mic_stride,
                                int n_arrays, int n_frames, int *doa_bin, float *doa_rad, float *prob,
                                float *energy, void *stream)
{
    int rc = check_stream_args(c, pcm, array_stride, mic_stride, n_arrays, n_frames);
    if (rc) return rc;
    if (!doa_bin) return fail(c, MCA_HIP_ERR_INVALID_ARGUMENT, "doa_bin_dev is NULL");
    c->n_lanes_last = 1; c->cur_lane = 0; c->a0 = 0;
    adapt_policy_begin(c, n_arrays, n_frames);
    c->lazy_entry = !c->host_call;
    rc = localise_impl(c, pcm, array_stride, mic_stride, n_arrays, n_frames, doa_bin, doa_rad, prob, energy, (hipStream_t)stream);
    c->lazy_entry = false;
    if (rc) return rc;
    c->last_arrays = n_arrays; c->last_frames = n_frames;
    c->e_cur ^= 1;
    return MCA_HIP_OK;
}

static int separate_frames_dev_bins(mca_hip_ctx *c, const float *pcm, long long array_stride, long long mic_stride,
                                    int n_arrays, int n_frames, const float *doa_rad, float *out_pcm, void *stream, const int *doa_bin)
{
    int rc = check_stream_args(c, pcm, array_stride, mic_stride, n_arrays, n_frames);
    if (rc) return rc;
    if (!doa_rad || !out_pcm) return fail(c, MCA_HIP_ERR_INVALID_ARGUMENT, "doa_rad_dev/out_pcm_dev is NULL");
    c->n_lanes_last = 1; c->cur_lane = 0; c->a0 = 0;
    rc = separate_impl(c, pcm, array_stride, mic_stride, n_arrays, n_frames, doa_rad, out_pcm, (hipStream_t)stream, doa_bin);
    if (rc) return rc;
    c->tail_cur ^= 1;
    return MCA_HIP_OK;
}

int mca_hip_separate_frames_dev(mca_hip_ctx *c, const float *pcm, long long array_stride, long long mic_stride,
                                int n_arrays, int n_frames, const float *doa_rad, float *out_pcm, void *stream)
{
    return separate_frames_dev_bins(c, pcm, array_stride, mic_stride, n_arrays, n_frames, doa_rad, out_pcm, stream, nullptr);
}

int mca_hip_separate_frames_bins_dev(mca_hip_ctx *c, const float *pcm, long long array_stride, long long mic_stride,
                                     int n_arrays, int n_frames, const int *doa_bin, const float *doa_rad, float *out_pcm, void *stream)
{
    if (!c) return MCA_HIP_ERR_INVALID_ARGUMENT;
    if (!doa_bin) return fail(c, MCA_HIP_ERR_INVALID_ARGUMENT, "doa_bin_dev is NULL");
    int rc = ensure_bf_table(c);
    if (rc) return rc;
    return separate_frames_dev_bins(c, pcm, array_stride, mic_stride, n_arrays, n_frames, doa_rad, out_pcm, stream, doa_bin);
}

int mca_hip_process_frames_dev(mca_hip_ctx *c, const float *pcm, long long array_stride, long long mic_stride,
                               int n_arrays, int n_frames, int *doa_bin, float *doa_rad, float *prob,
                               float *energy, float *out_pcm, void *stream)
{
    if (!c) return MCA_HIP_ERR_INVALID_ARGUMENT;
    if (!doa_rad) return fail(c, MCA_HIP_ERR_INVALID_ARGUMENT, "doa_rad_dev is NULL (the separation stage steers with it)");
    int rc = check_stream_args(c, pcm, array_stride, mic_stride, n_arrays, n_frames);
    if (rc) return rc;
    if (!doa_bin) return fail(c, MCA_HIP_ERR_INVALID_ARGUMENT, "doa_bin_dev is NULL");
    if (!out_pcm) return fail(c, MCA_HIP_ERR_INVALID_ARGUMENT, "doa_rad_dev/out_pcm_dev is NULL");
    if ((rc = ensure_bf_table(c))) return rc;
    c->n_lanes_last = 1; c->cur_lane = 0; c->a0 = 0;
    adapt_policy_begin(c, n_arrays, n_frames);
    c->lazy_entry = !c->host_call;
    rc = localise_impl(c, pcm, array_stride, mic_stride, n_arrays, n_frames, doa_bin, doa_rad, prob, energy, (hipStream_t)stream);
    c->lazy_entry = false;
    if (!rc) rc = separate_impl(c, pcm, array_stride, mic_stride, n_arrays, n_frames, doa_rad, out_pcm, (hipStream_t)stream, doa_bin);
    if (rc) return rc;
    c->last_arrays = n_arrays; c->last_frames = n_frames;
    c->e_cur ^= 1; c->tail_cur ^= 1;
    return MCA_HIP_OK;
}

struct mca_hip_graph {
    mca_hip_ctx *c = nullptr;
    const float *pcm = nullptr; long long array_stride = 0, mic_stride = 0;
    int n_arrays = 0, n_frames = 0;
    int *doa_bin = nullptr; float *doa_rad = nullptr, *prob = nullptr, *energy = nullptr, *out_pcm = nullptr;
    hipStream_t cap = nullptr;
    hipGraph_t graph[4] = {};
    hipGraphExec_t exec[4] = {};
    unsigned long long ws_gen = 0;
};

static void graph_orphan(mca_hip_graph *g);
static void graph_drop_recordings(mca_hip_graph *g)
{
    for (int i = 0; i < 4; ++i) {
        if (g->exec[i]) (void)hipGraphExecDestroy(g->exec[i]);
        if (g->graph[i]) (void)hipGraphDestroy(g->graph[i]);
        g->exec[i] = nullptr; g->graph[i] = nullptr;
    }
}

static void graph_orphan(mca_hip_graph *g) { graph_drop_recordings(g); g->c = nullptr; }

int mca_hip_graph_create(mca_hip_ctx *c, const float *pcm, long long array_stride, long long mic_stride, int n_arrays,
                         int n_frames, int *doa_bin, float *doa_rad, float *prob, float *energy, float *out_pcm,
                         mca_hip_graph **out)
{
    if (!out) return fail(c, MCA_HIP_ERR_INVALID_ARGUMENT, "out is NULL");
    *out = nullptr;
    int rc = check_stream_args(c, pcm, array_stride, mic_stride, n_arrays, n_frames);
    if (rc) return rc;
    if (!doa_bin && !out_pcm) return fail(c, MCA_HIP_ERR_INVALID_ARGUMENT, "doa_bin_dev and out_pcm_dev are both NULL: nothing to record");
    if (out_pcm && !doa_rad) return fail(c, MCA_HIP_ERR_INVALID_ARGUMENT, "doa_rad_dev is NULL (the separation stage steers with it)");
    HIP_TRY(c, hipSetDevice(c->cfg.device));
    if (doa_bin && (rc = reserve_impl(c, n_arrays, n_frames))) return rc;
    if (out_pcm && (rc = ensure_bf_table(c))) return rc;
    mca_hip_graph *g = new mca_hip_graph();
    g->c = c; g->pcm = pcm; g->array_stride = array_stride; g->mic_stride = mic_stride; g->n_arrays = n_arrays; g->n_frames = n_frames;
    g->doa_bin = doa_bin; g->doa_rad = doa_rad; g->prob = prob; g->energy = energy; g->out_pcm = out_pcm;
    if (hipStreamCreateWithFlags(&g->cap, hipStreamNonBlocking) != hipSuccess) { delete g; return fail(c, MCA_HIP_ERR_HIP, "hipStreamCreateWithFlags failed"); }
    g->ws_gen = c->ws_gen;
    c->graphs.push_back(g);
    *out = g;
    return MCA_HIP_OK;
}

static int graph_record(mca_hip_graph *g, int idx)
{
    mca_hip_ctx *c = g->c;
    const int e_cur = c->e_cur, tail_cur = c->tail_cur;
    const unsigned timing = c->timing;
    const unsigned long long adapt_frames = c->adapt_frames_total;
    c->timing = 0;
    const bool suspended = c->adapt_suspended;
    c->adapt_suspended = false; c->capturing = true;
    struct Restore { mca_hip_ctx *c; bool s; ~Restore() { c->adapt_suspended = s; c->capturing = false; } } restore{c, suspended};
    HIP_TRY(c, hipStreamBeginCapture(g->cap, hipStreamCaptureModeRelaxed));
    int rc = MCA_HIP_OK;
    if (g->doa_bin)
        rc = mca_hip_localise_frames_dev(c, g->pcm, g->array_stride, g->mic_stride, g->n_arrays, g->n_frames, g->doa_bin, g->doa_rad,
                                         g->prob, g->energy, g->cap);
    if (!rc && g->out_pcm)
        rc = separate_frames_dev_bins(c, g->pcm, g->array_stride, g->mic_stride, g->n_arrays, g->n_frames, g->doa_rad, g->out_pcm, g->cap, g->doa_bin);
    hipGraph_t graph = nullptr;
    const hipError_t e = hipStreamEndCapture(g->cap, &graph);
    c->timing = timing;
    c->e_cur = e_cur; c->tail_cur = tail_cur;
    c->adapt_frames_total = adapt_frames;
    if (rc) { if (graph) (void)hipGraphDestroy(graph); return rc; }
    if (e != hipSuccess) return fail(c, MCA_HIP_ERR_HIP, std::string("hipStreamEndCapture: ") + hipGetErrorString(e));
    g->graph[idx] = graph;
    HIP_TRY(c, hipGraphInstantiate(&g->exec[idx], graph, nullptr, nullptr, 0));
    return MCA_HIP_OK;
}

int mca_hip_graph_launch(mca_hip_graph *g, void *stream)
{
// ... 566 lines not shown
```

mcarray_amd/csrc/kernels.h:

```cpp
#pragma once
#include "mca_internal.h"

namespace mca {

template <int MT, bool ULA, typename OutT> __global__ void k_stft_phat(StftPhatArgs p);
template <int MT, bool ULA, typename OutT> __global__ void k_stft_phat_few(StftPhatArgs p);
__global__ void k_sum_planes(float *C, long long n4, int planes, long long stride);
__global__ void k_scan_partial(ScanPickArgs p);
__global__ void k_scan_carry(ScanPickArgs p);
template <int PL, int MODE> __global__ void k_scan_pick(ScanPickArgs p);
template <int PL> __global__ void k_scan_repick(ScanPickArgs p);
__global__ void k_repair_patch(RepairPatchArgs p);
__global__ void k_hist_list(int *list, int *n_list, int *need, int n_units);
__global__ void k_hist_settle(const float *e_hist, const float *hist_C, float *state, int *n_list, int D, int Dp, float mu, float omu);
__global__ void k_gate(GateArgs p);
__global__ void k_doa_fill(DoaFillArgs p);
template <int CPW, int OCC> __global__ void k_beamform_ola(BeamformArgs p);
template <typename OutT> __global__ void k_stft_phat_gen(StftPhatArgs p);
template <int MT, bool ULA, typename OutT> __global__ void k_stft_phat_512(StftPhatArgs p);
__global__ void k_beamform_512(BeamformArgs p);
template <int R, typename OutT> __global__ void k_stft_phat_sub2(StftPhatArgs p);
__global__ void k_beamform_gen(BeamformArgs p);
__global__ void k_bf_table(float2 *tab, const float *grid, const double *mic_x, int M, int n_pairs, double unit);
template <bool ODD> __global__ void k_beamform_wave(BeamformWaveArgs p);
template <bool POWER> __global__ void k_stft_phat_wave16(StftPhatArgs p);
template <int MT, bool ULA, typename OutT, bool MERGE = false> __global__ void k_stft_phat_2048(StftPhatArgs p);
__global__ void k_bf_table_2048(float2 *tab, const float *grid, const double *mic_x, int M, double unit);
__global__ void k_beamform_wave_2048(BeamformWaveArgs p);
template <int NPT, bool ODD> __global__ void k_beamform_wave_ms(BeamformWaveArgs p);
template <int MT, bool ULA, typename OutT, bool PL2, bool POWER, bool NOPHAT, bool MERGE, bool CAND = false> __global__ void k_stft_phat_wave(StftPhatArgs p);

__global__ void k_srp_gemm_f32(GemmArgs p);
template <bool SPLIT, int BN> __global__ void k_srp_gemm_f16(GemmArgs p);
__global__ void k_srp_gemm_f16_v2(GemmArgs p);
__global__ void k_srp_gemm_f16_v3(GemmArgs p);
template <int BN> __global__ void k_srp_gemm_repair(GemmArgs p);
__global__ void k_srp_cand(CandArgs p);

template <typename T> struct C2;
template <typename T>
__global__ void k_frame_srp(const C2<T> *X, int K, int D, int P, const int2 *pairs, const float *delays,
                            const T *E_in, T *E_out, T mu, T omu, int no_phat);
template <typename T>
__global__ void k_frame_pick(const T *E, int D, int P, int S, const float *grid, T *doa, T *prob, int *bins);
template <typename T>
__global__ void k_frame_beamform(const C2<T> *X, int M, int K, int fs, const double *mic_x, double doa, C2<T> *Y);
template <typename T> __global__ void k_frame_power(const C2<T> *X, int M, int K, T *out);

__global__ void k_gcc2_scan(Gcc2ScanArgs p);
__global__ void k_gcc2_compact(const unsigned char *voiced, int n_frames, int *vidx, int *nv, const int *post0, int *silence,
                               int windows_to_decay, unsigned char *vreset);
__global__ void k_gcc2_fill(Gcc2FillArgs p);
template <typename TC, typename TA>
__global__ void k_gcc2_prob(const TC *corr, long long corr_stride, int D, float step, const float *grid, const TA *doas, TA *probs, int n);
template <typename T>
__global__ void k_frame_gcc2(const T *corr, int D, float step, const float *grid, double doa_prev, double doa_mem, double one_minus_doa_mem,
                             double *res);
__global__ void k_mask_stream(MaskArgs p);
__global__ void k_mask_stream_gen(MaskGenArgs p);
__global__ void k_mask_stream_2048(MaskGenArgs p);
__global__ void k_mask_frame(MaskFrameArgs p);
__global__ void k_mb_analyse(MbAnalyseArgs p);
__global__ void k_mb_analyse_1024(MbAnalyseArgs p, int fpb);
__global__ void k_mb_analyse_512(MbAnalyseArgs p, int fpb);
__global__ void k_mb_scan(MbScanArgs p);
__global__ void k_mb_summary(MbSummaryArgs p);
__global__ void k_mvdr_analyse(MvdrAnalyseArgs p);
__global__ void k_mvdr_analyse_1024(MvdrAnalyseArgs p, int fpb);
__global__ void k_mvdr_analyse_512(MvdrAnalyseArgs p, int fpb);
template <int Q, bool FULL> __global__ void k_mvdr_solve(MvdrSolveArgs p);
__global__ void k_mvdr_synth(MvdrSynthArgs p);

}
```

mcarray_amd/csrc/kernels_wave.hip:

```cpp
#include <type_traits>

#include "fft1024c.h"
#include "mca_internal.h"
#include "cand_unit.h"
#include "phat_pairs.h"
#include "pair_balance.h"

namespace mca {

__global__ __launch_bounds__(256) void k_bf_table(float2 *tab, const float *grid, const double *mic_x, int M, int n_pairs, double unit)
{
    const int d = blockIdx.x, pr = blockIdx.y;
    const double doa = d == 0 ? 0.0 : (double)grid[d - 1];
    const double cd = cos(doa + 1.57079632679489661923);
    const double sc = 1.0 / ((double)M * 1024.0);
    float2 *row = tab + ((long long)d * n_pairs + pr) * 1024;
    for (int k = threadIdx.x; k < 1024; k += 256) {
        const int kap = k <= 512 ? k : k - 1024;
        double pa[2] = {0.0, 0.0}, pb[2] = {0.0, 0.0};
        for (int e = 0; e < 2; ++e) {
            const int c = 2 * pr + e;
            if (c >= M) continue;
            double turns = (double)kap * (unit * mic_x[c] * cd);
            turns -= rint(turns);
            double sn, cs;
            sincospi(2.0 * turns, &sn, &cs);
            if (k == 512) sn = 0.0;
            (e == 0 ? pa : pb)[0] = cs; (e == 0 ? pa : pb)[1] = sn;
        }
        row[k] = make_float2((float)((pa[0] + pb[1]) * sc), (float)((pa[1] - pb[0]) * sc));
    }
}

__device__ __forceinline__ float2 win_lo(float a, float b, v2f w)
{
    v2f x = {a, b}, r;
    asm("v_pk_mul_f32 %0, %1, %2 op_sel:[0,0] op_sel_hi:[1,0]" : "=v"(r) : "v"(x), "v"(w));
    return from_v2f(r);
}
__device__ __forceinline__ float2 win_hi(float a, float b, v2f w)
{
    v2f x = {a, b}, r;
    asm("v_pk_mul_f32 %0, %2, %1 op_sel:[1,0] op_sel_hi:[1,1]" : "=v"(r) : "v"(x), "v"(w));
    return from_v2f(r);
}

template <bool ODD>
__global__ __launch_bounds__(256, 2) void k_beamform_wave(BeamformWaveArgs p)
{
    constexpr int FOPT = 7;
    extern __shared__ __attribute__((aligned(16))) unsigned char smem_raw[];
    float2 *tab = reinterpret_cast<float2 *>(smem_raw);
    const int tid = threadIdx.x, lane = tid & 63, wave = __builtin_amdgcn_readfirstlane(tid >> 6);
    float2 *buf = tab + F1K_TWORDS + wave * F1K_SCRATCH;
    float *xcarry = reinterpret_cast<float *>(tab + F1K_TWORDS + 4 * F1K_SCRATCH);
    f1k_table_init(tab, tid, 256);
    F1kLane lc;
    lc.init(lane);
    __syncthreads();
    lc.load_t1(tab, lane);

    const int a = p.skew ? blockIdx.x : blockIdx.y;
    const long long as = (long long)a * p.S + blockIdx.z;
    int w0 = (int)blockIdx.x * (4 * p.ft - 1), ft = p.ft;
    if (p.skew) {
        const int g = blockIdx.y, half = gridDim.y >> 1, hi = p.ft + p.skew, lo = p.ft - p.skew;
        ft = g < half ? hi : lo;
        w0 = g < half ? g * (4 * hi - 1) : half * (4 * hi - 1) + (g - half) * (4 * lo - 1);
    }
    const int t0 = wave == 0 ? w0 : w0 + wave * ft - 1;
    const int t1 = min(w0 + (wave + 1) * ft - 1, p.n_frames);
    const bool active = t0 < t1;
    const bool lead_in = wave == 0 && t0 > 0;
    const bool deferred = wave > 0;
    const int tfirst = lead_in ? t0 - 1 : t0;
    const int NP = p.n_pairs;
    float carry[8], first[8];
#pragma unroll
    for (int i = 0; i < 8; ++i) { carry[i] = 0.f; first[i] = 0.f; }

    if (active) {
        v2f win[8];
#pragma unroll
        for (int i = 0; i < 8; ++i) { win[i].x = p.window[lane + 128 * i]; win[i].y = p.window[lane + 128 * i + 64]; }
        if (t0 == 0) {
#pragma unroll
            for (int i = 0; i < 8; ++i) carry[i] = p.tail_in[as * FFT_H + lane + 64 * i];
        }
        const float *base = p.pcm + (long long)a * p.array_stride + lane;
// ... 148 lines not shown
                fft1024c<true, 3>(y, buf, lane, tab, lc, [&]() { load_pair(min(t + 1, t1 - 1), 0); });
            } else {
                fft1024c<true, 3>(y, buf, lane, tab, lc);
                trow = row_of(t, s + 1);
#pragma unroll
                for (int i = 0; i < 16; ++i) T[i] = trow[64 * dr16(i)];
            }
            float *cs = carry + s * FFT_H;
            if (t >= t0) {
                float *o = p.out + ((long long)a * S + s) * p.n_frames * FFT_H + (long long)t * FFT_H + lane;
#pragma unroll
                for (int i = 0; i < 8; ++i) o[64 * i] = cs[64 * i] + y[dr16(i)].x;
            }
#pragma unroll
            for (int i = 0; i < 8; ++i) cs[64 * i] = y[dr16(i + 8)].x;
        };
        for (int s = 0; s + 1 < S; ++s) source(s, std::false_type());
        source(S - 1, std::true_type());
    }
    if (t1 == p.n_frames) {
        for (int s = 0; s < S; ++s) {
#pragma unroll
            for (int i = 0; i < 8; ++i) p.tail_out[((long long)a * S + s) * FFT_H + lane + 64 * i] = carry[s * FFT_H + 64 * i];
        }
    }
}
template __global__ void k_beamform_wave_ms<1, false>(BeamformWaveArgs);
template __global__ void k_beamform_wave_ms<2, false>(BeamformWaveArgs); template __global__ void k_beamform_wave_ms<2, true>(BeamformWaveArgs);
template __global__ void k_beamform_wave_ms<3, false>(BeamformWaveArgs); template __global__ void k_beamform_wave_ms<3, true>(BeamformWaveArgs);
template __global__ void k_beamform_wave_ms<4, false>(BeamformWaveArgs); template __global__ void k_beamform_wave_ms<4, true>(BeamformWaveArgs);

template <bool NOPHAT = false>
__device__ __forceinline__ float2 whiten4(float2 z, float &pw, float thr = 4e-30f, float unit = 0.5f)
{
    v2f zv = to_v2f(z), sq, r;
    asm("v_pk_mul_f32 %0, %1, %1" : "=v"(sq) : "v"(zv));
    pw = sq.x + sq.y;
    const float s = NOPHAT ? unit : (pw > thr ? __builtin_amdgcn_rsqf(pw) : 0.f);
    v2f sv = {s, s};
    asm("v_pk_mul_f32 %0, %1, %2 op_sel_hi:[1,0]" : "=v"(r) : "v"(zv), "v"(sv));
    return from_v2f(r);
}

template <bool PL2>
__device__ __forceinline__ void store_a_wave(_Float16 *row, unsigned voff, int cidx, float2 v, int Kp)
{
    const float2_t vv = {v.x, v.y};
    const half2_t hi = __builtin_convertvector(vv, half2_t);
    char *b = reinterpret_cast<char *>(row + 2 * cidx);
    *reinterpret_cast<half2_t *>(b + voff) = hi;
    if (PL2) {
        const float2_t back = __builtin_convertvector(hi, float2_t);
        *reinterpret_cast<half2_t *>(reinterpret_cast<char *>(row + Kp + 2 * cidx) + voff) = __builtin_convertvector(vv - back, half2_t);
    }
}
template <bool PL2>
__device__ __forceinline__ void store_a_wave(float *row, unsigned voff, int cidx, float2 v, int)
{
    *reinterpret_cast<float2 *>(reinterpret_cast<char *>(row + 2 * cidx) + 2 * voff) = v;
}

__device__ __forceinline__ unsigned or3(unsigned a, unsigned b, unsigned c)
{
    unsigned r;
    asm("v_or3_b32 %0, %1, %2, %3" : "=v"(r) : "v"(a), "v"(b), "v"(c));
    return r;
}

typedef __attribute__((address_space(3))) float lds_float_t;

__device__ __forceinline__ float wave_sum64(float v)
{
    asm("s_nop 1\n\tv_add_f32_dpp %0, %0, %0 quad_perm:[1,0,3,2] row_mask:0xf bank_mask:0xf\n\t"
        "s_nop 1\n\tv_add_f32_dpp %0, %0, %0 quad_perm:[2,3,0,1] row_mask:0xf bank_mask:0xf\n\t"
        "s_nop 1\n\tv_add_f32_dpp %0, %0, %0 row_ror:4 row_mask:0xf bank_mask:0xf\n\t"
        "s_nop 1\n\tv_add_f32_dpp %0, %0, %0 row_ror:8 row_mask:0xf bank_mask:0xf\n\t"
        "s_nop 1\n\tv_add_f32_dpp %0, %0, %0 row_bcast:15 row_mask:0xa bank_mask:0xf\n\t"
        "s_nop 1\n\tv_add_f32_dpp %0, %0, %0 row_bcast:31 row_mask:0xc bank_mask:0xf\n\t"
        "s_nop 1"
        : "+v"(v));
    return __int_as_float(__builtin_amdgcn_readlane(__float_as_int(v), 63));
}

template <int MT, bool ULA, typename OutT, bool PL2, bool POWER, bool NOPHAT, bool MERGE, bool CAND = false>
__global__ __launch_bounds__(512) void k_stft_phat_wave(StftPhatArgs p)
{
    static_assert(!MERGE || (ULA && !PL2 && !NOPHAT && sizeof(OutT) == 2), "the merged index serves the one-plane fp16 rows of a ULA");
    constexpr int NP = MT / 2, NOUT = PairOut<MT, ULA>::N;
    constexpr int NRANK = 2 * (MT - 1) * 64 * 4 + 8;
    extern __shared__ __attribute__((aligned(16))) unsigned char smem_raw[];
    float2 *tab = reinterpret_cast<float2 *>(smem_raw);
    const int tid = threadIdx.x, lane = tid & 63, wave = __builtin_amdgcn_readfirstlane(tid >> 6);
    const int nw = (int)blockDim.x >> 6, nthr = (int)blockDim.x;
    const unsigned short *rankl = reinterpret_cast<const unsigned short *>(tab + F1K_TWORDS);
    const int nmp = MERGE ? (p.n_merged + 63) & ~63 : 0;
    const int regw = MERGE ? max(F1K_SCRATCH, nmp) : F1K_SCRATCH;
    float2 *wbase = tab + F1K_TWORDS + (MERGE ? NRANK / 4 : 0);
    float2 *buf = wbase + wave * regw;
    float2 *nyq = wbase + nw * regw + wave * ((p.fpb + p.skew) * NP);
    const int n_list_now = p.list ? *p.n_list : 0;
    const int e_first = (p.list && p.list0 + (int)blockIdx.x < n_list_now) ? p.list[p.list0 + (int)blockIdx.x] : 0;
    f1k_table_init(tab, tid, nthr);
    if (MERGE) {
        unsigned short *ot = reinterpret_cast<unsigned short *>(tab + F1K_TWORDS);
        for (int e = tid; e < 2 * (MT - 1) * 64 * 4; e += nthr) {
            const int s4 = e & 3, ln = (e >> 2) & 63, gh = e >> 8, g = (gh >> 1) + 1, h = gh & 1;
            const int lm = ln <= 32 ? ln : 96 - ln;
            ot[e] = p.mrank[(lm + 64 * (4 * h + s4)) * g];
        }
        if (tid < MT - 1) ot[2 * (MT - 1) * 64 * 4 + tid] = p.mrank[512 * (tid + 1)];
    }
    F1kLane lc;
    lc.init(lane);
    __syncthreads();
    const int lam = lane <= 32 ? lane : 96 - lane;
    const unsigned voff = (unsigned)lam * 4u;
    const bool self = (lane & 31) == 0;
    v2f win[8];
#pragma unroll
    for (int i = 0; i < 8; ++i) { win[i].x = p.window[lane + 128 * i]; win[i].y = p.window[lane + 128 * i + 64]; }

    const int li_end = p.list ? min(n_list_now, p.list0 + p.list_cap) : 1, li_step = p.list ? (int)gridDim.x : 1;
    for (int li = p.list ? p.list0 + (int)blockIdx.x : 0; li < li_end; li += li_step) {
        int a = blockIdx.y;
        int f_begin = ((int)blockIdx.x * nw + wave) * p.fpb, f_end = min(f_begin + p.fpb, p.n_frames);
        if (p.skew) {
            const int g = blockIdx.y, half = gridDim.y >> 1, hi = p.fpb + p.skew, lo = p.fpb - p.skew;
            a = blockIdx.x;
            if (g < half) { f_begin = (g * nw + wave) * hi; f_end = f_begin + hi; }
            else { f_begin = half * nw * hi + ((g - half) * nw + wave) * lo; f_end = f_begin + lo; }
        }
        long long row_base = (long long)a * p.n_frames;
        bool hist_unit = false;
        int e_unit = 0;
        if (p.list) {
            const int e = li == p.list0 + (int)blockIdx.x ? e_first : p.list[li];
            e_unit = e;
            hist_unit = p.hist_in != nullptr && e >= p.hist_base;
            const int eu = hist_unit ? e - p.hist_base : e, upa = hist_unit ? HIST_UNITS : p.groups_per_array;
            a = eu / upa;
            const int g_begin = (eu - a * upa) * REPAIR_GROUP;
            row_base = (long long)(li - p.list0) * REPAIR_GROUP - g_begin;
            f_begin = g_begin + wave; f_end = min(f_begin + 1, hist_unit ? HIST_FRAMES : p.n_frames);
        }
        const bool has_frame = f_begin < f_end;
        if (!has_frame && !CAND) continue;
        if (has_frame) {
        const float *base = hist_unit ? p.hist_in + (long long)a * MT * HIST_SAMPLES + lane : p.pcm + (long long)a * p.array_stride + lane;
        const long long mstride = hist_unit ? (long long)HIST_SAMPLES : p.mic_stride;
        const int fr0 = hist_unit ? 0 : p.frame0;
        float xa[16], xb[16];
        auto load_pair = [&](int f, int pr) {
            const float *pa = base + (long long)(2 * pr) * mstride + (long long)(fr0 + f) * FFT_H;
            const float *pb = pa + mstride;
#pragma unroll
            for (int i = 0; i < 16; ++i) { xa[i] = pa[64 * i]; xb[i] = pb[64 * i]; }
        };
        const int nfr = f_end - f_begin;
        const int rot = p.list ? 0 : (int)((unsigned)(5 * a + 3 * ((int)blockIdx.x * nw + wave)) % (unsigned)nfr);
        auto frame_of = [&](int i) { const int j = i + rot; return f_begin + (j >= nfr ? j - nfr : j); };
        load_pair(frame_of(0), 0);
        for (int fi = 0; fi < nfr; ++fi) {
            const int f = frame_of(fi);
            float2 Xh[MT][8], zn[NP];
            v2f ptime = {0.f, 0.f};
            bool any_alive = false;
#pragma unroll
            for (int pr = 0; pr < NP; ++pr) {
                float2 z[16];
                if (p.hist_out) {
                    const int j = p.frame0 + f - (p.total_frames - HIST_FRAMES);
                    if (j >= 0) {
                        float *ha = p.hist_out + ((long long)a * MT + 2 * pr) * HIST_SAMPLES + j * FFT_H + lane;
#pragma unroll
                        for (int i = 0; i < 8; ++i) { ha[64 * i] = xa[i]; ha[HIST_SAMPLES + 64 * i] = xb[i]; }
                        if (j == HIST_FRAMES - 1) {
#pragma unroll
                            for (int i = 0; i < 8; ++i) { ha[FFT_H + 64 * i] = xa[8 + i]; ha[HIST_SAMPLES + FFT_H + 64 * i] = xb[8 + i]; }
                        }
                    }
                }
#pragma unroll
                for (int i = 0; i < 8; ++i) { z[2 * i] = win_lo(xa[2 * i], xb[2 * i], win[i]); z[2 * i + 1] = win_hi(xa[2 * i + 1], xb[2 * i + 1], win[i]); }
                if (POWER) {
#pragma unroll
                    for (int i = 0; i < 16; ++i) { const v2f zv = to_v2f(z[i]); asm("v_pk_fma_f32 %0, %1, %1, %0" : "+v"(ptime) : "v"(zv)); }
                }
                float ma = max3abs(z[0].x, z[1].x, z[2].x), mb = max3abs(z[0].y, z[1].y, z[2].y);
#pragma unroll
                for (int i = 3; i < 15; i += 2) { ma = max3abs(ma, z[i].x, z[i + 1].x); mb = max3abs(mb, z[i].y, z[i + 1].y); }
                ma = max2abs(ma, z[15].x); mb = max2abs(mb, z[15].y);
                const PairBalance pb = pair_balance(ma, mb);
                const bool alive_a = pb.alive_a, alive_b = pb.alive_b;
                any_alive = any_alive || alive_a || alive_b;
                if (pb.scaled()) {
                    const float sa = pb.sa(), sb = pb.sb();
#pragma unroll
                    for (int i = 0; i < 16; ++i) z[i] = make_float2(z[i].x * sa, z[i].y * sb);
                }
                fft1024c<false, 3>(z, buf, lane, tab, lc, [&]() {
                    const bool lastp = pr == NP - 1, last = lastp && fi + 1 >= nfr;
                    load_pair(last ? f : (lastp ? frame_of(fi + 1) : f), last ? pr : (lastp ? 0 : pr + 1));
                }, lam);
                const float un_a = pb.un_a(), un_b = pb.un_b();
                if (MERGE) zn[pr] = make_float2(z[dr16(8)].x * un_a, z[dr16(8)].y * un_b);
                if (lane == 0) {
                    const float2 n = z[dr16(8)];
                    if (!MERGE) nyq[(f - f_begin) * NP + pr] = make_float2(n.x * un_a, n.y * un_b);
                    float2 t[16];
#pragma unroll
                    for (int j = 0; j < 16; ++j) t[j] = z[dr16(j)];
#pragma unroll
                    for (int j = 8; j < 16; ++j) z[dr16(j < 12 ? j + 4 : j - 4)] = t[(j + 1) & 15];
                } else if (self) {
#pragma unroll
                    for (int j = 8; j < 12; ++j) { const float2 t = z[dr16(j)]; z[dr16(j)] = z[dr16(j + 4)]; z[dr16(j + 4)] = t; }
                } else {
#pragma unroll
                    for (int j = 8; j < 12; ++j) {
                        float2 &u = z[dr16(j)], &w = z[dr16(j + 4)];
                        swap_rows32(u.x, w.x); swap_rows32(w.x, u.x);
                        swap_rows32(u.y, w.y); swap_rows32(w.y, u.y);
                    }
                }
                const float thr_a = PairBalance::thr(4e-30f, pb.na, alive_a), thr_b = PairBalance::thr(4e-30f, pb.nb, alive_b);
                const float half_a = PairBalance::down(0.5f, pb.na, alive_a), half_b = PairBalance::down(0.5f, pb.nb, alive_b);
#pragma unroll
                for (int s = 0; s < 8; ++s) {
                    const float2 zk = z[dr16(s)], zm = z[dr16(15 - s < 12 ? 15 - s + 4 : 15 - s - 4)];
                    const float2 a2 = make_float2(zk.x + zm.x, zk.y - zm.y);
                    const float2 b2 = make_float2(zk.y + zm.y, zm.x - zk.x);
                    float pwa, pwb;
                    Xh[2 * pr][s] = whiten4<NOPHAT>(a2, pwa, thr_a, half_a);
                    Xh[2 * pr + 1][s] = whiten4<NOPHAT>(b2, pwb, thr_b, half_b);
                }
            }
            if (p.dead && lane == 0) p.dead[(long long)a * p.total_frames + p.frame0 + f] = any_alive ? 0 : 1;
            OutT *arow = reinterpret_cast<OutT *>(p.A) + (row_base + f) * (long long)p.a_row_elems;
            if (MERGE) {
                float2 *S = buf;
                for (int j = lane; j < nmp / 2; j += 64) reinterpret_cast<float4 *>(S)[j] = make_float4(0.f, 0.f, 0.f, 0.f);
                wave_lds_fence();
                float xn[MT];
#pragma unroll
                for (int pr = 0; pr < NP; ++pr) {
                    float pw;
                    xn[2 * pr] = whiten4(make_float2(2.f * zn[pr].x, 0.f), pw).x;
                    xn[2 * pr + 1] = whiten4(make_float2(2.f * zn[pr].y, 0.f), pw).x;
                }
                const uint2 *offt = reinterpret_cast<const uint2 *>(rankl) + lane;
#pragma unroll
                for (int g = 1; g < MT; ++g) {
#pragma unroll
                    for (int h = 0; h < 2; ++h) {
                        const uint2 o4 = offt[(2 * (g - 1) + h) * 64];
                        const unsigned off[4] = {o4.x & 0xffffu, o4.x >> 16, o4.y & 0xffffu, o4.y >> 16};
                        float2 acc[4], cur[4];
#pragma unroll
                        for (int s2 = 0; s2 < 4; ++s2) {
                            acc[s2] = make_float2(0.f, 0.f);
#pragma unroll
                            for (int i = 0; i + g < MT; ++i) acc[s2] = cmacc(acc[s2], Xh[i][4 * h + s2], Xh[i + g][4 * h + s2]);
                        }
#pragma unroll
                        for (int s2 = 0; s2 < 4; ++s2) cur[s2] = S[off[s2]];
#pragma unroll
                        for (int s2 = 0; s2 < 4; ++s2) S[off[s2]] = cadd(cur[s2], acc[s2]);
                    }
                }
                if (lane == 0) {
                    float an[MT - 1], cn[MT - 1];
                    unsigned on[MT - 1];
#pragma unroll
                    for (int g = 1; g < MT; ++g) {
                        an[g - 1] = 0.f;
#pragma unroll
                        for (int i = 0; i + g < MT; ++i) an[g - 1] = fmaf(xn[i], xn[i + g], an[g - 1]);
                        on[g - 1] = rankl[2 * (MT - 1) * 64 * 4 + g - 1];
                    }
#pragma unroll
                    for (int g = 0; g < MT - 1; ++g) cn[g] = S[on[g]].x;
#pragma unroll
                    for (int g = 0; g < MT - 1; ++g) S[on[g]].x = cn[g] + an[g];
                }
                wave_lds_fence();
                typedef _Float16 half4_t __attribute__((ext_vector_type(4)));
                typedef float float4_t __attribute__((ext_vector_type(4)));
                for (int j = lane; j < nmp / 2; j += 64) {
                    const float4 v = reinterpret_cast<const float4 *>(S)[j];
                    const float4_t vv = {v.x, v.y, v.z, v.w};
                    reinterpret_cast<half4_t *>(arow)[j] = __builtin_convertvector(vv, half4_t);
                }
                wave_lds_fence();
            } else {
#pragma unroll
                for (int s = 0; s < 8; ++s) {
                    if constexpr (ULA) {
                        float2 r[MT], out[NOUT];
#pragma unroll
                        for (int m = 0; m < MT; ++m) r[m] = Xh[m][s];
                        pair_products<MT, ULA>(r, out);
#pragma unroll
                        for (int g = 0; g < NOUT; ++g) store_a_wave<PL2>(arow, voff, g * KG + 64 * s, out[g], p.Kp);
                    } else {
                        int pi = 0;
#pragma unroll
                        for (int i = 0; i < MT; ++i)
#pragma unroll
                            for (int j = i + 1; j < MT; ++j) { store_a_wave<PL2>(arow, voff, pi * KG + 64 * s, cmulc(Xh[i][s], Xh[j][s]), p.Kp); ++pi; }
                    }
                }
            }
            if (POWER) {
                const float pacc = wave_sum64(ptime.x + ptime.y);
                if (lane == 0) p.power[(long long)a * p.total_frames + p.frame0 + f] = pacc / (float)FFT_N / (float)MT;
            }
        }
        wave_lds_fence();
        if (!MERGE && lane < f_end - f_begin) {
            float2 xn[MT], out[NOUT];
#pragma unroll
            for (int pr = 0; pr < NP; ++pr) {
                const float2 n = nyq[lane * NP + pr];
                float pw;
                xn[2 * pr] = whiten4<NOPHAT>(make_float2(2.f * n.x, 0.f), pw);
                xn[2 * pr + 1] = whiten4<NOPHAT>(make_float2(2.f * n.y, 0.f), pw);
            }
            OutT *arow = reinterpret_cast<OutT *>(p.A) + (row_base + f_begin + lane) * (long long)p.a_row_elems;
            pair_products<MT, ULA>(xn, out);
#pragma unroll
            for (int g = 0; g < NOUT; ++g) store_a_wave<PL2>(arow, 0u, g * KG + FFT_H, out[g], p.Kp);
        }
        }
        wave_lds_fence();
        if constexpr (CAND) {
            static_assert(!CAND || PL2, "the candidate contraction reads the two-plane rows of the list mode");
            {
                __syncthreads();
                cand_unit<4>(p.cand, li - p.list0, e_unit, reinterpret_cast<unsigned char *>(wbase), tid);
            }
        }
    }
}

typedef _Float16 h2 __attribute__((ext_vector_type(2)));
__device__ __forceinline__ h2 rot_j_conj(h2 b)
{
    h2 r;
    const unsigned c = 0x3C00BC00u;
    asm("v_pk_mul_f16 %0, %1, %2 op_sel:[1,0] op_sel_hi:[0,1]" : "=v"(r) : "v"(b), "v"(c));
    return r;
}

template <bool POWER>
__global__ __launch_bounds__(256, 2) void k_stft_phat_wave16(StftPhatArgs p)
{
    constexpr int MT = 16, NP = 8;
    extern __shared__ __attribute__((aligned(16))) unsigned char smem_raw[];
    float2 *tab = reinterpret_cast<float2 *>(smem_raw);
    const int tid = threadIdx.x, lane = tid & 63, wave = __builtin_amdgcn_readfirstlane(tid >> 6);
    float2 *buf = tab + F1K_TWORDS + wave * F1K_SCRATCH;
    float *wtab = reinterpret_cast<float *>(tab + F1K_TWORDS + 4 * F1K_SCRATCH);
    const int fpa = p.fpb + p.skew;
    float2 *nyq = reinterpret_cast<float2 *>(wtab + 1024) + wave * (fpa * NP);
    float2 *nref = reinterpret_cast<float2 *>(wtab + 1024) + 4 * (fpa * NP) + wave * (fpa * NP);
    float *dcbad = reinterpret_cast<float *>(reinterpret_cast<float2 *>(wtab + 1024) + 8 * (fpa * NP)) + wave * fpa;
    constexpr float UNSURE = 1e-10f;
    for (int e = tid; e < 1024; e += 256) wtab[(e & 63) * 16 + (e >> 6)] = p.window[e];
    f1k_table_init(tab, tid, 256);
    F1kLane lc;
    lc.init(lane);
    __syncthreads();
    const int lam = lane <= 32 ? lane : 96 - lane;
    const unsigned voff = (unsigned)lam * 4u;
    const bool self = (lane & 31) == 0;
    const float4 *wq = reinterpret_cast<const float4 *>(wtab + lane * 16);

    const int a = p.skew ? blockIdx.x : blockIdx.y;
    int f_begin = ((int)blockIdx.x * 4 + wave) * p.fpb, f_end = min(f_begin + p.fpb, p.n_frames);
    if (p.skew) {
        const int g = blockIdx.y, half = gridDim.y >> 1, hi = p.fpb + p.skew, lo = p.fpb - p.skew;
        if (g < half) { f_begin = (g * 4 + wave) * hi; f_end = f_begin + hi; }
        else { f_begin = half * 4 * hi + ((g - half) * 4 + wave) * lo; f_end = f_begin + lo; }
    }
    if (f_begin >= f_end) return;
    const long long row_base = (long long)a * p.n_frames;
    const float *base = p.pcm + (long long)a * p.array_stride + lane;
    float xa[16], xb[16];
    auto load_pair = [&](int f, int pr) {
        const float *pa = base + (long long)(2 * pr) * p.mic_stride + (long long)(p.frame0 + f) * FFT_H;
        const float *pb = pa + p.mic_stride;
#pragma unroll
        for (int i = 0; i < 16; ++i) { xa[i] = pa[64 * i]; xb[i] = pb[64 * i]; }
    };
    const int nfr = f_end - f_begin;
    const int rot = (int)((unsigned)(5 * a + 3 * ((int)blockIdx.x * 4 + wave)) % (unsigned)nfr);
    auto frame_of = [&](int i) { const int j = i + rot; return f_begin + (j >= nfr ? j - nfr : j); };
    load_pair(frame_of(0), 0);
    for (int fi = 0; fi < nfr; ++fi) {
        const int f = frame_of(fi);
        h2 Xh[MT][8];
        v2f ptime = {0.f, 0.f};
        bool dc_unsure = false;
#pragma unroll
        for (int pr = 0; pr < NP; ++pr) {
            float2 z[16];
#pragma unroll
            for (int i4 = 0; i4 < 4; ++i4) {
                const float4 w4 = wq[i4];
                const v2f w01 = {w4.x, w4.y}, w23 = {w4.z, w4.w};
                z[4 * i4] = win_lo(xa[4 * i4], xb[4 * i4], w01); z[4 * i4 + 1] = win_hi(xa[4 * i4 + 1], xb[4 * i4 + 1], w01);
                z[4 * i4 + 2] = win_lo(xa[4 * i4 + 2], xb[4 * i4 + 2], w23); z[4 * i4 + 3] = win_hi(xa[4 * i4 + 3], xb[4 * i4 + 3], w23);
            }
            float ref_a = 0.f, ref_b = 0.f;
            if (POWER || p.unsure) {
                v2f pz = {0.f, 0.f};
#pragma unroll
                for (int i = 0; i < 16; ++i) { const v2f zv = to_v2f(z[i]); asm("v_pk_fma_f32 %0, %1, %1, %0" : "+v"(pz) : "v"(zv)); }
                if (POWER) { ptime.x += pz.x; ptime.y += pz.y; }
                if (p.unsure) { ref_a = 4.f * wave_sum64(pz.x); ref_b = 4.f * wave_sum64(pz.y); }
            }
            float ma = max3abs(z[0].x, z[1].x, z[2].x), mb = max3abs(z[0].y, z[1].y, z[2].y);
#pragma unroll
            for (int i = 3; i < 15; i += 2) { ma = max3abs(ma, z[i].x, z[i + 1].x); mb = max3abs(mb, z[i].y, z[i + 1].y); }
// ... 31 lines not shown
                }
            }
            float pw0a = 0.f, pw0b = 0.f;
            const float thr_a = PairBalance::thr(4e-30f, pb.na, alive_a), thr_b = PairBalance::thr(4e-30f, pb.nb, alive_b);
#pragma unroll
            for (int s = 0; s < 8; ++s) {
                const float2 zk = z[dr16(s)], zm = z[dr16(15 - s < 12 ? 15 - s + 4 : 15 - s - 4)];
                const float2 a2 = make_float2(zk.x + zm.x, zk.y - zm.y);
                const float2 b2 = make_float2(zk.y + zm.y, zm.x - zk.x);
                float pwa, pwb;
                const float2 wa = whiten4<false>(a2, pwa, thr_a), wb = whiten4<false>(b2, pwb, thr_b);
                const float2_t va = {wa.x, wa.y}, vb = {wb.x, wb.y};
                Xh[2 * pr][s] = __builtin_convertvector(va, h2);
                Xh[2 * pr + 1][s] = __builtin_convertvector(vb, h2);
                if (s == 0) { pw0a = pwa; pw0b = pwb; }
                if (s == 0 && p.unsure && lane == 0) {
                    nref[(f - f_begin) * NP + pr] = make_float2(ref_a, ref_b);
                    dc_unsure = dc_unsure || (pw0a < UNSURE * dc_a) || (pw0b < UNSURE * dc_b);
                }
            }
        }
        if (p.unsure && lane == 0) dcbad[f - f_begin] = dc_unsure ? 1.f : 0.f;
        _Float16 *arow = reinterpret_cast<_Float16 *>(p.A) + (row_base + f) * (long long)p.a_row_elems;
#pragma unroll
        for (int s = 0; s < 8; ++s) {
            __builtin_amdgcn_sched_barrier(0);
            h2 rj[MT];
#pragma unroll
            for (int j = 1; j < MT; ++j) rj[j] = rot_j_conj(Xh[j][s]);
            float re[MT - 1], im[MT - 1];
#pragma unroll
            for (int g = 0; g < MT - 1; ++g) { re[g] = 0.f; im[g] = 0.f; }
#pragma unroll
            for (int i = 0; i < MT; ++i)
#pragma unroll
                for (int j = i + 1; j < MT; ++j) {
                    re[j - i - 1] = __builtin_amdgcn_fdot2(Xh[i][s], Xh[j][s], re[j - i - 1], false);
                    im[j - i - 1] = __builtin_amdgcn_fdot2(Xh[i][s], rj[j], im[j - i - 1], false);
                }
#pragma unroll
            for (int g = 0; g < MT - 1; ++g) store_a_wave<false>(arow, voff, g * KG + 64 * s, make_float2(re[g], im[g]), p.Kp);
        }
        if (POWER) {
            const float pacc = wave_sum64(ptime.x + ptime.y);
            if (lane == 0) p.power[(long long)a * p.total_frames + p.frame0 + f] = pacc / (float)FFT_N / (float)MT;
        }
    }
    wave_lds_fence();
    if (lane < f_end - f_begin) {
        float2 xn[MT], out[MT - 1];
#pragma unroll
        for (int pr = 0; pr < NP; ++pr) {
            const float2 n = nyq[lane * NP + pr];
            float pw;
            xn[2 * pr] = whiten4<false>(make_float2(2.f * n.x, 0.f), pw);
            xn[2 * pr + 1] = whiten4<false>(make_float2(2.f * n.y, 0.f), pw);
        }
        if (p.unsure) {
            bool u = dcbad[lane] != 0.f;
#pragma unroll
            for (int pr = 0; pr < NP; ++pr) {
                const float2 n = nyq[lane * NP + pr], r = nref[lane * NP + pr];
                u = u || (4.f * n.x * n.x < UNSURE * r.x) || (4.f * n.y * n.y < UNSURE * r.y);
            }
            p.unsure[(long long)a * p.total_frames + p.frame0 + f_begin + lane] = u ? 1 : 0;
        }
        _Float16 *arow = reinterpret_cast<_Float16 *>(p.A) + (row_base + f_begin + lane) * (long long)p.a_row_elems;
        pair_products<MT, true>(xn, out);
#pragma unroll
        for (int g = 0; g < MT - 1; ++g) store_a_wave<false>(arow, 0u, g * KG + FFT_H, out[g], p.Kp);
    }
}
template __global__ void k_stft_phat_wave16<false>(StftPhatArgs);
template __global__ void k_stft_phat_wave16<true>(StftPhatArgs);

#define INST_SPW1(MT, ULA, T, PL2, NP) template __global__ void k_stft_phat_wave<MT, ULA, T, PL2, false, NP, false>(StftPhatArgs); \
                                       template __global__ void k_stft_phat_wave<MT, ULA, T, PL2, true, NP, false>(StftPhatArgs);
#define INST_SPW(MT, ULA) INST_SPW1(MT, ULA, _Float16, false, false) INST_SPW1(MT, ULA, _Float16, true, false) INST_SPW1(MT, ULA, float, false, false) \
                          INST_SPW1(MT, ULA, float, false, true)
INST_SPW(8, true) INST_SPW(8, false) INST_SPW(4, true) INST_SPW(4, false)
template __global__ void k_stft_phat_wave<8, true, _Float16, false, false, false, true>(StftPhatArgs);
template __global__ void k_stft_phat_wave<8, true, _Float16, false, true, false, true>(StftPhatArgs);
template __global__ void k_stft_phat_wave<4, true, _Float16, false, false, false, true>(StftPhatArgs);
template __global__ void k_stft_phat_wave<4, true, _Float16, false, true, false, true>(StftPhatArgs);
template __global__ void k_stft_phat_wave<8, true, _Float16, true, false, false, false, true>(StftPhatArgs);
template __global__ void k_stft_phat_wave<8, false, _Float16, true, false, false, false, true>(StftPhatArgs);
template __global__ void k_stft_phat_wave<4, true, _Float16, true, false, false, false, true>(StftPhatArgs);
template __global__ void k_stft_phat_wave<4, false, _Float16, true, false, false, false, true>(StftPhatArgs);

}
```

mcarray_amd/csrc/mca_internal.h:

```cpp
#pragma once
#include <hip/hip_runtime.h>

#define MCA_MAX_SOURCES 4
#define MCA_MAX_MICS 16

namespace mca {

constexpr int MK_NB = 4;
constexpr int MK_WARM = 8;
constexpr int BF_NB = 4;
constexpr int GCC2_DOAWARM = 64;
constexpr int SCAN_WARM = 96;
constexpr int KG = 513;
#ifndef MCA_SCAN_CHUNK
#define MCA_SCAN_CHUNK 32
#endif
#ifndef MCA_SCAN_SUB
#define MCA_SCAN_SUB 32
#endif
constexpr int SCAN_CHUNK = MCA_SCAN_CHUNK;
constexpr int SCAN_SUB = MCA_SCAN_SUB;
#ifndef MCA_SCAN_LD
#define MCA_SCAN_LD 8
#endif
constexpr int SCAN_LD = MCA_SCAN_LD;
#ifndef MCA_REPAIR_WARM
#define MCA_REPAIR_WARM 16
#endif
constexpr int REPAIR_WARM = MCA_REPAIR_WARM;
constexpr int REPAIR_GROUP = 4;
constexpr int HIST_FRAMES = REPAIR_WARM, HIST_UNITS = HIST_FRAMES / REPAIR_GROUP, HIST_SAMPLES = (HIST_FRAMES + 1) * 512;
static_assert(HIST_FRAMES % REPAIR_GROUP == 0, "history = whole repair units");

constexpr int CAND_WORDS_MAX = 20;
struct CandArgs {
    const void *A;
    const void *B;
    int Kp, Dp, a_row_elems;
    const int *list; const int *n_list; int list0, pass_rows;
    unsigned *umask; int umask_words;
    int *need;
    int groups_per_array, n_frames;
    float *C; int c_planes; long long c_plane_stride;
    float *hist_C; int hist_base;
};

struct StftPhatArgs {
    const float *pcm;
    long long array_stride, mic_stride;
    int M, n_frames, frame0, fpb;
    const float *window;
    void *A;
    int Kp;
    int a_row_elems;
    int a_planes;
    float *power;
    int total_frames;
    int N, logH, kg, ula;
    const float2 *tw;
    const int *list; const int *n_list; int list0, list_cap, groups_per_array;
    float *hist_out; const float *hist_in; int hist_base;
    const unsigned short *mrank; int n_merged;
    int no_phat;
    int skew;
    unsigned char *dead;
    unsigned char *unsure;
    int cand_on; CandArgs cand;
};

__device__ __forceinline__ void store_a(float *row, const StftPhatArgs &, int cidx, float2 v)
{
    reinterpret_cast<float2 *>(row)[cidx] = v;
}

typedef _Float16 half2_t __attribute__((ext_vector_type(2)));

typedef float float2_t __attribute__((ext_vector_type(2)));

__device__ __forceinline__ void store_a(_Float16 *row, const StftPhatArgs &p, int cidx, float2 v)
{
    const float2_t vv = {v.x, v.y};
    const half2_t hi = __builtin_convertvector(vv, half2_t);
    reinterpret_cast<half2_t *>(row)[cidx] = hi;
    if (p.a_planes == 2) {
        const float2_t back = __builtin_convertvector(hi, float2_t);
        const half2_t lo = __builtin_convertvector(vv - back, half2_t);
        reinterpret_cast<half2_t *>(row + p.Kp)[cidx] = lo;
    }
}

struct GemmArgs {
    const void *A;
    const void *B;
    float *C;
    int rows;
    int chunk_frames, total_frames, frame0;
    int Kp, Dp, a_row_elems;
    long long c_plane_elems;
    const void *Bt;
    const int *n_list; int list0;
    int repair_ksplit;
    int repair_items;
    float *part; int *nvoiced; int D, n_chunks;
    long long part_plane_stride;
    float scan_w[32];
};

struct ScanPickArgs {
    const float *C;
    int c_planes; long long c_plane_stride;
    int n_frames, Dp, D, P, S, chunk, n_chunks;
    float mu, one_minus_mu;
    float inv_norm;
    const float *state_in;
    float *state_out;
    float *part;
    int part_planes; long long part_plane_stride;
    int *nvoiced;
    float *e_start;
    const unsigned char *voiced;
    const float *grid;
    int *doa_bin; float *doa_rad; float *prob; float *energy;
    int mode;
    float tau;
    unsigned char *flags;
    int groups_per_array;
    int *need;
    int *list;
    int *n_list;
    int *chunk_from;
    int *clist; int *n_clist;
    int lookback;
    unsigned long long *probe;
    unsigned long long probe_seq;
    int *last_vchunk;
    unsigned long long *stats;
    const unsigned char *dead;
    const unsigned char *unsure;
    int lazy, hist_valid, hist_base;
    float *hist_C_out, *e_hist_out;
    const float *hist_C_in, *e_hist_in;
    unsigned *umask; int umask_words;
    int *need_full, *list_full, *n_list_full;
};

constexpr int REPAIR_KSPLIT_MAX = 32;
__host__ __device__ inline long long repair_plane_stride(int n_rows, int Dp) { return (long long)((n_rows + 127) / 128 * 128) * Dp; }
__host__ __device__ inline long long repair_cx_rows(long long pass_rows, int ksplit) { return ((pass_rows + 127) / 128 * 128) * ksplit; }
__host__ __device__ inline int repair_ksplit_eff(int ksplit, int n_rows, int Dp, int items_max)
{
// ... 200 lines not shown
```

Measured before the change: 48.51 million frames/s.

## Fuse speculative steered beamforming into STFT-PHAT kernel with separate synthesis pass

Adds a steer path for the 8-mic ULA adaptive/fp16 configuration. The STFT-PHAT kernel now also computes the delay-and-sum spectrum, using the previous call's last DOA bin as a predicted steering direction. A patch kernel recomputes frames whose actual DOA differs from the prediction, and a new synthesis kernel does the inverse FFT and overlap-add. This avoids re-reading PCM and redoing per-mic FFTs in the separate beamform stage. It adds host-side feedback on the miss rate that disables speculation when too many frames miss, plus extra LDS and register pressure in the fused STFT kernel.

```diff
diff --git a/include/mcarray_hip.h b/include/mcarray_hip.h
--- a/include/mcarray_hip.h
+++ b/include/mcarray_hip.h
@@ -221,6 +221,7 @@
 int mca_hip_get_repair_stats(mca_hip_ctx *ctx, unsigned long long *frames, unsigned long long *flagged_frames,
                              unsigned long long *recomputed_frames);
 int mca_hip_get_repair_columns(mca_hip_ctx *ctx, unsigned long long *candidate_columns, unsigned long long *whole_row_frames);
+int mca_hip_get_steer_stats(mca_hip_ctx *ctx, unsigned long long *frames, unsigned long long *missed_frames, unsigned long long *fused_calls);
 
 const char *mca_hip_version(void);
 
diff --git a/mcarray_amd/_lib.py b/mcarray_amd/_lib.py
--- a/mcarray_amd/_lib.py
+++ b/mcarray_amd/_lib.py
@@ -172,6 +172,7 @@
     ("mca_hip_host_unregister", C.c_int, [C.c_void_p]),
     ("mca_hip_get_repair_stats", C.c_int, [C.c_void_p, C.POINTER(C.c_ulonglong), C.POINTER(C.c_ulonglong), C.POINTER(C.c_ulonglong)]),
     ("mca_hip_get_repair_columns", C.c_int, [C.c_void_p, C.POINTER(C.c_ulonglong), C.POINTER(C.c_ulonglong)]),
+    ("mca_hip_get_steer_stats", C.c_int, [C.c_void_p, C.POINTER(C.c_ulonglong), C.POINTER(C.c_ulonglong), C.POINTER(C.c_ulonglong)]),
     ("mca_hip_version", C.c_char_p, []),
 ]
 
diff --git a/mcarray_amd/api.py b/mcarray_amd/api.py
--- a/mcarray_amd/api.py
+++ b/mcarray_amd/api.py
@@ -306,6 +306,11 @@
         self._check(self._lib.mca_hip_get_repair_stats(self.h, C.byref(a), C.byref(b), C.byref(c_)))
         return {"frames": a.value, "flagged": b.value, "recomputed": c_.value}
 
+    def steer_stats(self):
+        a, b, c_ = C.c_ulonglong(0), C.c_ulonglong(0), C.c_ulonglong(0)
+        self._check(self._lib.mca_hip_get_steer_stats(self.h, C.byref(a), C.byref(b), C.byref(c_)))
+        return {"frames": a.value, "missed": b.value, "fused_calls": c_.value}
+
     def repair_columns(self):
         a, b = C.c_ulonglong(0), C.c_ulonglong(0)
         self._check(self._lib.mca_hip_get_repair_columns(self.h, C.byref(a), C.byref(b)))
diff --git a/mcarray_amd/csrc/api.hip b/mcarray_amd/csrc/api.hip
--- a/mcarray_amd/csrc/api.hip
+++ b/mcarray_amd/csrc/api.hip
@@ -97,6 +97,13 @@
     bool merged = false; int n_merged = 0, Kp_m = 0;
     void *d_Bm = nullptr, *d_Btm = nullptr; unsigned short *d_mrank = nullptr;
     float2 *d_bftab = nullptr; int bf_pairs = 0;
+    float4 *d_steer_rows = nullptr; float2 *d_steer_q = nullptr; float *d_steer_nyq = nullptr; int *d_steer_pred = nullptr; unsigned long long *d_steer_miss = nullptr;
+    float2 *d_steer_Y = nullptr; size_t steer_Y_rows = 0; float *d_steer_tail = nullptr;
+    bool steer_now = false, steer_fused_now = false;
+    unsigned long long steer_frames_total = 0, steer_fused_calls = 0;
+    unsigned long long *h_steer = nullptr;
+    unsigned long long steer_seq = 0, steer_seq_seen = 0, steer_call_frames[FB_RING] = {};
+    bool steer_spec = true, steer_lost = false;
     float *d_E[2] = {nullptr, nullptr};
     float *d_tail[2] = {nullptr, nullptr};
     int e_cur = 0, tail_cur = 0;
@@ -197,12 +204,13 @@
 {
     if (!c) return;
     auto F = [](void *p) { if (p) (void)hipFree(p); };
-    F(c->d_window); F(c->d_tw); F(c->d_grid); F(c->d_delays); F(c->d_micx); F(c->d_pairs); F(c->d_B); F(c->d_Bt); F(c->d_bftab); F(c->d_Bm); F(c->d_Btm); F(c->d_mrank);
+    F(c->d_window); F(c->d_tw); F(c->d_grid); F(c->d_delays); F(c->d_micx); F(c->d_pairs); F(c->d_B); F(c->d_Bt); F(c->d_bftab); F(c->d_steer_rows); F(c->d_steer_q); F(c->d_steer_nyq); F(c->d_steer_pred); F(c->d_steer_miss); F(c->d_steer_Y); F(c->d_steer_tail); F(c->d_Bm); F(c->d_Btm); F(c->d_mrank);
     F(c->d_E[0]); F(c->d_E[1]); F(c->d_tail[0]); F(c->d_tail[1]); F(c->d_doa[0]); F(c->d_doa[1]); F(c->d_vdone[0]); F(c->d_vdone[1]); F(c->d_g2_vidx); F(c->d_g2_nv); F(c->d_g2_rad); F(c->d_g2_prob);
     F(c->d_g2_reset); F(c->d_g2_post0); F(c->d_silence);
     F(c->d_rstats); F(c->d_gate_state);
     for (int i = 0; i < 2; ++i) { F(c->d_hist_pcm[i]); F(c->d_hist_C[i]); F(c->d_ehist[i]); }
     if (c->h_probe) (void)hipHostFree(c->h_probe);
+    if (c->h_steer) (void)hipHostFree(c->h_steer);
     for (Workspace &w : c->lanes) w.release();
     for (auto &e : c->io_ev) if (e) (void)hipEventDestroy(e);
     for (auto &q : c->io_stream) if (q) (void)hipStreamDestroy(q);
@@ -751,7 +759,8 @@
         }
         const bool mg = w.mrank != nullptr && !a.list;
         const int nrank = 2 * (M - 1) * 64 * 4 + 8, regw = mg ? std::max(F1K_SCRATCH, (w.n_merged + 63) & ~63) : F1K_SCRATCH;
-        const size_t smw = (size_t)(F1K_TWORDS + (mg ? nrank / 4 : 0) + 4 * regw + (mg ? 0 : 4 * (w.fpb + w.skew) * (M / 2))) * sizeof(float2);
+        const bool fuse = mg && M == 8 && w.bf.rows != nullptr && a.power == nullptr && regw >= F1K_SCRATCH + STEER_LDS_ROWS * 64;
+        const size_t smw = (size_t)(F1K_TWORDS + (mg ? nrank / 4 : 0) + 4 * regw + (mg ? 0 : 4 * (w.fpb + w.skew) * (M / 2)) + (fuse ? 4 * STEER_QWORDS : 0)) * sizeof(float2);
         const bool pl2 = a.a_planes == 2, pw = a.power != nullptr;
 #define LAUNCH_K(K)                                                                                                 \
         do {                                                                                                         \
@@ -773,7 +782,8 @@
         } while (0)
         if constexpr (sizeof(OutT) == 2) {
             if (mg) {
-                if (M == 8) { if (pw) LAUNCH_K((k_stft_phat_wave<8, true, OutT, false, true, false, true>)); else LAUNCH_K((k_stft_phat_wave<8, true, OutT, false, false, false, true>)); }
+                if (fuse) { LAUNCH_K((k_stft_phat_wave<8, true, OutT, false, false, false, true, false, true>)); c->steer_fused_now = true; }
+                else if (M == 8) { if (pw) LAUNCH_K((k_stft_phat_wave<8, true, OutT, false, true, false, true>)); else LAUNCH_K((k_stft_phat_wave<8, true, OutT, false, false, false, true>)); }
                 else { if (pw) LAUNCH_K((k_stft_phat_wave<4, true, OutT, false, true, false, true>)); else LAUNCH_K((k_stft_phat_wave<4, true, OutT, false, false, false, true>)); }
                 HIP_TRY(c, hipGetLastError());
                 return MCA_HIP_OK;
@@ -1045,6 +1055,8 @@
         if (w.d_chunk_from) HIP_TRY(c, hipMemsetAsync(w.d_chunk_from, 0x7f, w.adapt_chunks * 4, st));
         if (w.d_nlist) HIP_TRY(c, hipMemsetAsync(w.d_nlist, 0, 16, st));
     }
+    if (c->d_steer_pred) HIP_TRY(c, hipMemsetAsync(c->d_steer_pred, 0xff, na * 4, st));
+    c->steer_spec = true; c->steer_lost = false; c->steer_seq_seen = c->steer_seq;
     c->gcc2_frames_done = 0;
     c->g2f = G2FrameState();
     return init_last_state(c, st);
@@ -1161,6 +1173,7 @@
     return ensure_scan_workspace(c, n_arrays, n_frames, n_chunks);
 }
 
+static int steer_reserve(mca_hip_ctx *c, int n_arrays, int n_frames);
 static int reserve_impl(mca_hip_ctx *c, int n_arrays, int n_frames)
 {
     HIP_TRY(c, hipSetDevice(c->cfg.device));
@@ -1171,7 +1184,8 @@
 int mca_hip_reserve(mca_hip_ctx *c, int n_arrays, int n_frames)
 {
     if (!c || n_arrays < 1 || n_frames < 1) return MCA_HIP_ERR_INVALID_ARGUMENT;
-    return reserve_impl(c, n_arrays, n_frames);
+    const int rc = reserve_impl(c, n_arrays, n_frames);
+    return rc ? rc : steer_reserve(c, n_arrays, n_frames);
 }
 
 static int run_correlation_map(mca_hip_ctx *c, const float *pcm, long long array_stride, long long mic_stride,
@@ -1202,6 +1216,9 @@
         if (c->prec == MCA_HIP_SRP_ADAPTIVE && c->a_planes == 1 && wave16_applies(c)) sa.unsure = c->ws().d_unsure;
         if (c->lazy_now && cand_call(c, true)) sa.dead = c->ws().d_unsure;
         if (c->lazy_now) sa.hist_out = c->d_hist_pcm[c->hist_cur ^ 1];
+        if (c->steer_now && sa.mrank && !sa.power) {
+            sa.bf.rows = c->d_steer_rows; sa.bf.q = c->d_steer_q; sa.bf.nyq = c->d_steer_nyq; sa.bf.pred = c->d_steer_pred + c->a0; sa.bf.Y = c->d_steer_Y;
+        }
         time_begin(c, MCA_HIP_K_STFT_PHAT, st);
         if (c->n512) {
             rc = c->prec == MCA_HIP_SRP_FP32 ? launch_stft_512<float>(c, sa, dim3(0, n_arrays), st) : launch_stft_512<_Float16>(c, sa, dim3(0, n_arrays), st);
@@ -1527,6 +1544,19 @@
     return MCA_HIP_OK;
 }
 
+int mca_hip_get_steer_stats(mca_hip_ctx *c, unsigned long long *frames, unsigned long long *missed_frames, unsigned long long *fused_calls)
+{
+    if (!c) return MCA_HIP_ERR_INVALID_ARGUMENT;
+    HIP_TRY(c, hipSetDevice(c->cfg.device));
+    HIP_TRY(c, hipDeviceSynchronize());
+    unsigned long long m = 0;
+    if (c->d_steer_miss) HIP_TRY(c, hipMemcpy(&m, c->d_steer_miss, sizeof(m), hipMemcpyDeviceToHost));
+    if (frames) *frames = c->steer_frames_total;
+    if (missed_frames) *missed_frames = m;
+    if (fused_calls) *fused_calls = c->steer_fused_calls;
+    return MCA_HIP_OK;
+}
+
 int mca_hip_get_repair_columns(mca_hip_ctx *c, unsigned long long *candidate_columns, unsigned long long *whole_row_frames)
 {
     if (!c) return MCA_HIP_ERR_INVALID_ARGUMENT;
@@ -1563,6 +1593,104 @@
     hipLaunchKernelGGL(k_bf_table, dim3(c->D + 1, np), dim3(256), 0, nullptr, c->d_bftab, c->d_grid, c->d_micx, c->M, np, unit);
     HIP_TRY(c, hipGetLastError());
     HIP_TRY(c, hipDeviceSynchronize());
+    return MCA_HIP_OK;
+}
+
+static bool steer_applies(const mca_hip_ctx *c)
+{
+    return !c->generic && !c->n512 && !c->n2048 && c->N == FFT_N && c->M == 8 && c->ula && c->S == 1 && !c->cfg.use_power_floor && c->merged &&
+           (c->prec == MCA_HIP_SRP_ADAPTIVE || c->prec == MCA_HIP_SRP_FP16) && c->cfg.gcc_weighting != MCA_HIP_GCC_NONE;
+}
+
+static int steer_pass_frames(const mca_hip_ctx *c, int n_arrays, int n_frames)
+{
+    const long long cap = ws_max_bytes(c) / ((long long)n_arrays * STEER_ROW * (long long)sizeof(float2));
+    return (int)std::max<long long>(1, std::min<long long>(n_frames, cap));
+}
+
+static void steer_policy_begin(mca_hip_ctx *c)
+{
+    const unsigned long long s = c->steer_seq + 1;
+    if (!c->h_steer || c->steer_lost || s <= FB_LAG) return;
+    const unsigned long long r = s - FB_LAG;
+    if (r <= c->steer_seq_seen) return;
+    const unsigned long long *slot = c->h_steer + 2 * ((r - 1) % FB_RING);
+    const auto t0 = std::chrono::steady_clock::now();
+    while (__atomic_load_n(&slot[1], __ATOMIC_ACQUIRE) != r) {
+        if (std::chrono::duration_cast<std::chrono::milliseconds>(std::chrono::steady_clock::now() - t0).count() > FB_WAIT_MS) { c->steer_lost = true; c->steer_spec = true; return; }
+        std::this_thread::yield();
+    }
+    c->steer_seq_seen = r;
+    c->steer_spec = __atomic_load_n(&slot[0], __ATOMIC_RELAXED) * STEER_MISS_DEN <= c->steer_call_frames[(r - 1) % FB_RING] * STEER_MISS_NUM;
+}
+
+static int steer_prepare(mca_hip_ctx *c, int n_arrays, int n_frames)
+{
+    if (!c->d_steer_rows) {
+        const size_t na = (size_t)c->cfg.max_arrays;
+        HIP_TRY(c, hipMalloc((void **)&c->d_steer_rows, (size_t)(c->D + 1) * 4 * 64 * sizeof(float4)));
+        HIP_TRY(c, hipMalloc((void **)&c->d_steer_q, (size_t)(c->D + 1) * c->M * 8 * sizeof(float2)));
+        HIP_TRY(c, hipMalloc((void **)&c->d_steer_nyq, (size_t)(c->D + 1) * c->M * sizeof(float)));
+        HIP_TRY(c, hipMalloc((void **)&c->d_steer_pred, na * sizeof(int)));
+        HIP_TRY(c, hipMalloc((void **)&c->d_steer_miss, 3 * sizeof(unsigned long long)));
+        if (hipHostMalloc((void **)&c->h_steer, FB_RING * 16, hipHostMallocDefault) == hipSuccess) std::memset(c->h_steer, 0, FB_RING * 16); else { c->h_steer = nullptr; (void)hipGetLastError(); }
+        HIP_TRY(c, hipMalloc((void **)&c->d_steer_tail, 2 * na * FFT_H * sizeof(float)));
+        HIP_TRY(c, hipMemset(c->d_steer_pred, 0xff, na * sizeof(int)));
+        HIP_TRY(c, hipMemset(c->d_steer_miss, 0, 3 * sizeof(unsigned long long)));
+        const double unit = (double)c->cfg.sample_rate / (double)FFT_N / 346.1;
+        hipLaunchKernelGGL(k_steer_table, dim3(c->D + 1, 4), dim3(64), 0, nullptr, c->d_steer_rows, c->d_steer_q, c->d_steer_nyq, c->d_grid, c->d_micx, c->M, unit);
+        HIP_TRY(c, hipGetLastError());
+        HIP_TRY(c, hipDeviceSynchronize());
+    }
+    const size_t rows = (size_t)n_arrays * steer_pass_frames(c, n_arrays, n_frames);
+    if (rows > c->steer_Y_rows) {
+        HIP_TRY(c, hipDeviceSynchronize());
+        if (c->d_steer_Y) (void)hipFree(c->d_steer_Y);
+        c->d_steer_Y = nullptr; c->steer_Y_rows = 0;
+        HIP_TRY(c, hipMalloc((void **)&c->d_steer_Y, rows * STEER_ROW * sizeof(float2)));
+        c->steer_Y_rows = rows;
+    }
+    return MCA_HIP_OK;
+}
+
+static int steer_reserve(mca_hip_ctx *c, int n_arrays, int n_frames) { return steer_applies(c) ? steer_prepare(c, n_arrays, n_frames) : MCA_HIP_OK; }
+
+static int steer_separate(mca_hip_ctx *c, const float *pcm, long long array_stride, long long mic_stride, int n_arrays, int n_frames,
+                          const int *doa_bin, float *out_pcm, hipStream_t st)
+{
+    const size_t a0 = (size_t)c->a0;
+    const int pf = steer_pass_frames(c, n_arrays, n_frames);
+    const bool fused = c->steer_fused_now && pf == n_frames;
+    const size_t smem = (size_t)(F1K_TWORDS + 4 * F1K_SCRATCH) * sizeof(float2);
+    float *tails[2] = {c->d_steer_tail, c->d_steer_tail + (size_t)c->cfg.max_arrays * FFT_H};
+    time_begin(c, MCA_HIP_K_BEAMFORM, st);
+    int pass = 0;
+    for (int f0 = 0; f0 < n_frames; f0 += pf, ++pass) {
+        const int f1 = std::min(n_frames, f0 + pf), np = f1 - f0;
+        const bool last = f1 == n_frames;
+        SteerPatchArgs pa{};
+        pa.pcm = pcm; pa.array_stride = array_stride; pa.mic_stride = mic_stride; pa.n_arrays = n_arrays; pa.n_frames = n_frames; pa.f0 = f0; pa.f1 = f1;
+        pa.window = c->d_window; pa.doa_bin = doa_bin; pa.all = fused ? 0 : 1; pa.miss = c->d_steer_miss;
+        pa.bf.rows = c->d_steer_rows; pa.bf.q = c->d_steer_q; pa.bf.nyq = c->d_steer_nyq; pa.bf.pred = c->d_steer_pred + a0; pa.bf.Y = c->d_steer_Y;
+        pa.y_f0 = f0; pa.y_frames = fused ? n_frames : np;
+        hipLaunchKernelGGL(k_steer_patch, dim3(std::min(STEER_PATCH_WGS, (np + 3) / 4)), dim3(256), smem, st, pa);
+        SteerSynthArgs sy{};
+        sy.Y = c->d_steer_Y; sy.n_frames = n_frames; sy.f0 = f0; sy.f1 = f1; sy.y_f0 = pa.y_f0; sy.y_frames = pa.y_frames;
+        sy.ft = 16;
+        while (sy.ft > 2 && (long long)n_arrays * ((np + sy.ft - 1) / sy.ft) < 1024) sy.ft >>= 1;
+        sy.out = out_pcm;
+        sy.tail_in = pass == 0 ? c->d_tail[c->tail_cur] + a0 * FFT_H : tails[(pass - 1) & 1];
+        sy.tail_out = last ? c->d_tail[c->tail_cur ^ 1] + a0 * FFT_H : tails[pass & 1];
+        sy.doa_bin = doa_bin; sy.pred_out = last ? c->d_steer_pred + a0 : nullptr;
+        if (last && c->h_steer) { sy.report = c->h_steer + 2 * (c->steer_seq % FB_RING); sy.seq = c->steer_seq + 1; sy.miss_total = c->d_steer_miss; }
+        const int runs = (np + sy.ft - 1) / sy.ft;
+        hipLaunchKernelGGL(k_steer_synth, dim3((runs + 3) / 4, n_arrays), dim3(256), smem, st, sy);
+    }
+    time_end(c, st);
+    HIP_TRY(c, hipGetLastError());
+    c->steer_call_frames[c->steer_seq % FB_RING] = (unsigned long long)n_arrays * n_frames; ++c->steer_seq;
+    c->steer_frames_total += (unsigned long long)n_arrays * n_frames;
+    if (fused) ++c->steer_fused_calls;
     return MCA_HIP_OK;
 }
 
@@ -1764,11 +1892,17 @@
     if (!out_pcm) return fail(c, MCA_HIP_ERR_INVALID_ARGUMENT, "doa_rad_dev/out_pcm_dev is NULL");
     if ((rc = ensure_bf_table(c))) return rc;
     c->n_lanes_last = 1; c->cur_lane = 0; c->a0 = 0;
+    const bool steer = steer_applies(c) && !c->host_call && !c->capturing;
+    if (steer && (rc = steer_prepare(c, n_arrays, n_frames))) return rc;
+    if (steer) steer_policy_begin(c);
+    c->steer_now = steer && c->steer_spec && steer_pass_frames(c, n_arrays, n_frames) == n_frames; c->steer_fused_now = false;
     adapt_policy_begin(c, n_arrays, n_frames);
     c->lazy_entry = !c->host_call;
     rc = localise_impl(c, pcm, array_stride, mic_stride, n_arrays, n_frames, doa_bin, doa_rad, prob, energy, (hipStream_t)stream);
     c->lazy_entry = false;
-    if (!rc) rc = separate_impl(c, pcm, array_stride, mic_stride, n_arrays, n_frames, doa_rad, out_pcm, (hipStream_t)stream, doa_bin);
+    c->steer_now = false;
+    if (!rc && steer) rc = steer_separate(c, pcm, array_stride, mic_stride, n_arrays, n_frames, doa_bin, out_pcm, (hipStream_t)stream);
+    else if (!rc) rc = separate_impl(c, pcm, array_stride, mic_stride, n_arrays, n_frames, doa_rad, out_pcm, (hipStream_t)stream, doa_bin);
     if (rc) return rc;
     c->last_arrays = n_arrays; c->last_frames = n_frames;
     c->e_cur ^= 1; c->tail_cur ^= 1;
diff --git a/mcarray_amd/csrc/kernels.h b/mcarray_amd/csrc/kernels.h
--- a/mcarray_amd/csrc/kernels.h
+++ b/mcarray_amd/csrc/kernels.h
@@ -28,7 +28,10 @@
 __global__ void k_bf_table_2048(float2 *tab, const float *grid, const double *mic_x, int M, double unit);
 __global__ void k_beamform_wave_2048(BeamformWaveArgs p);
 template <int NPT, bool ODD> __global__ void k_beamform_wave_ms(BeamformWaveArgs p);
-template <int MT, bool ULA, typename OutT, bool PL2, bool POWER, bool NOPHAT, bool MERGE, bool CAND = false> __global__ void k_stft_phat_wave(StftPhatArgs p);
+template <int MT, bool ULA, typename OutT, bool PL2, bool POWER, bool NOPHAT, bool MERGE, bool CAND = false, bool FUSE = false> __global__ void k_stft_phat_wave(StftPhatArgs p);
+__global__ void k_steer_table(float4 *rows, float2 *q, float *nyq, const float *grid, const double *mic_x, int M, double unit);
+__global__ void k_steer_patch(SteerPatchArgs p);
+__global__ void k_steer_synth(SteerSynthArgs p);
 
 __global__ void k_srp_gemm_f32(GemmArgs p);
 template <bool SPLIT, int BN> __global__ void k_srp_gemm_f16(GemmArgs p);
diff --git a/mcarray_amd/csrc/kernels_wave.hip b/mcarray_amd/csrc/kernels_wave.hip
--- a/mcarray_amd/csrc/kernels_wave.hip
+++ b/mcarray_amd/csrc/kernels_wave.hip
@@ -5,6 +5,7 @@
 #include "cand_unit.h"
 #include "phat_pairs.h"
 #include "pair_balance.h"
+#include "steer.h"
 
 namespace mca {
 
@@ -319,10 +320,11 @@
     return __int_as_float(__builtin_amdgcn_readlane(__float_as_int(v), 63));
 }
 
-template <int MT, bool ULA, typename OutT, bool PL2, bool POWER, bool NOPHAT, bool MERGE, bool CAND = false>
+template <int MT, bool ULA, typename OutT, bool PL2, bool POWER, bool NOPHAT, bool MERGE, bool CAND = false, bool FUSE = false>
 __global__ __launch_bounds__(512) void k_stft_phat_wave(StftPhatArgs p)
 {
     static_assert(!MERGE || (ULA && !PL2 && !NOPHAT && sizeof(OutT) == 2), "the merged index serves the one-plane fp16 rows of a ULA");
+    static_assert(!FUSE || (MERGE && MT == 8 && !POWER), "the steered half spectrum rides in the free words of the 8-microphone merged region");
     constexpr int NP = MT / 2, NOUT = PairOut<MT, ULA>::N;
     constexpr int NRANK = 2 * (MT - 1) * 64 * 4 + 8;
     extern __shared__ __attribute__((aligned(16))) unsigned char smem_raw[];
@@ -383,7 +385,8 @@
         const bool has_frame = f_begin < f_end;
         if (!has_frame && !CAND) continue;
         if (has_frame) {
-        const float *base = hist_unit ? p.hist_in + (long long)a * MT * HIST_SAMPLES + lane : p.pcm + (long long)a * p.array_stride + lane;
+        const unsigned lofs = FUSE ? (unsigned)lane : 0u;
+        const float *base = hist_unit ? p.hist_in + (long long)a * MT * HIST_SAMPLES + (FUSE ? 0 : lane) : p.pcm + (long long)a * p.array_stride + (FUSE ? 0 : lane);
         const long long mstride = hist_unit ? (long long)HIST_SAMPLES : p.mic_stride;
         const int fr0 = hist_unit ? 0 : p.frame0;
         float xa[16], xb[16];
@@ -391,15 +394,26 @@
             const float *pa = base + (long long)(2 * pr) * mstride + (long long)(fr0 + f) * FFT_H;
             const float *pb = pa + mstride;
 #pragma unroll
-            for (int i = 0; i < 16; ++i) { xa[i] = pa[64 * i]; xb[i] = pb[64 * i]; }
+            for (int i = 0; i < 16; ++i) { xa[i] = pa[lofs + 64 * i]; xb[i] = pb[lofs + 64 * i]; }
         };
         const int nfr = f_end - f_begin;
         const int rot = p.list ? 0 : (int)((unsigned)(5 * a + 3 * ((int)blockIdx.x * nw + wave)) % (unsigned)nfr);
         auto frame_of = [&](int i) { const int j = i + rot; return f_begin + (j >= nfr ? j - nfr : j); };
         load_pair(frame_of(0), 0);
+        const float4 *srow = nullptr; const float *snyq = nullptr;
+        float2 *Yl = buf + F1K_SCRATCH + lam;
+        float2 *Qs = wbase + nw * regw + wave * STEER_QWORDS;
+        if (FUSE) {
+            const int pred = __builtin_amdgcn_readfirstlane(p.bf.pred[a]) + 1;
+            srow = p.bf.rows + (long long)pred * (NP * 64);
+            snyq = p.bf.nyq + pred * MT;
+            if (lane < STEER_QWORDS) Qs[lane] = p.bf.q[(pred * MT + 2 * (lane / 14) + (lane & 1)) * 8 + (lane % 14) / 2 + 1];
+            wave_lds_fence();
+        }
         for (int fi = 0; fi < nfr; ++fi) {
             const int f = frame_of(fi);
             float2 Xh[MT][8], zn[NP];
+            float2 *yrow = FUSE ? p.bf.Y + ((long long)a * p.total_frames + p.frame0 + f) * STEER_ROW : nullptr;
             v2f ptime = {0.f, 0.f};
             bool any_alive = false;
 #pragma unroll
@@ -408,12 +422,12 @@
                 if (p.hist_out) {
                     const int j = p.frame0 + f - (p.total_frames - HIST_FRAMES);
                     if (j >= 0) {
-                        float *ha = p.hist_out + ((long long)a * MT + 2 * pr) * HIST_SAMPLES + j * FFT_H + lane;
-#pragma unroll
-                        for (int i = 0; i < 8; ++i) { ha[64 * i] = xa[i]; ha[HIST_SAMPLES + 64 * i] = xb[i]; }
+                        float *ha = p.hist_out + ((long long)a * MT + 2 * pr) * HIST_SAMPLES + j * FFT_H + (FUSE ? 0 : lane);
+#pragma unroll
+                        for (int i = 0; i < 8; ++i) { ha[lofs + 64 * i] = xa[i]; ha[lofs + HIST_SAMPLES + 64 * i] = xb[i]; }
                         if (j == HIST_FRAMES - 1) {
 #pragma unroll
-                            for (int i = 0; i < 8; ++i) { ha[FFT_H + 64 * i] = xa[8 + i]; ha[HIST_SAMPLES + FFT_H + 64 * i] = xb[8 + i]; }
+                            for (int i = 0; i < 8; ++i) { ha[lofs + FFT_H + 64 * i] = xa[8 + i]; ha[lofs + HIST_SAMPLES + FFT_H + 64 * i] = xb[8 + i]; }
                         }
                     }
                 }
@@ -435,12 +449,15 @@
 #pragma unroll
                     for (int i = 0; i < 16; ++i) z[i] = make_float2(z[i].x * sa, z[i].y * sb);
                 }
+                const float4 Bl = FUSE ? (srow + pr * 64)[(unsigned)lane] : make_float4(0.f, 0.f, 0.f, 0.f);
                 fft1024c<false, 3>(z, buf, lane, tab, lc, [&]() {
                     const bool lastp = pr == NP - 1, last = lastp && fi + 1 >= nfr;
+                    if (FUSE) { Yl[64 * STEER_Y_BASE] = make_float2(Bl.x, Bl.y); Yl[64 * (STEER_Y_BASE + 1)] = make_float2(Bl.z, Bl.w); }
                     load_pair(last ? f : (lastp ? frame_of(fi + 1) : f), last ? pr : (lastp ? 0 : pr + 1));
                 }, lam);
                 const float un_a = pb.un_a(), un_b = pb.un_b();
-                if (MERGE) zn[pr] = make_float2(z[dr16(8)].x * un_a, z[dr16(8)].y * un_b);
+                if (MERGE && !FUSE) zn[pr] = make_float2(z[dr16(8)].x * un_a, z[dr16(8)].y * un_b);
+                if (FUSE) { const float2 n = make_float2(z[dr16(8)].x * un_a, z[dr16(8)].y * un_b); if (pr < NP - 1) Yl[64 * (STEER_Y_ZN + pr)] = n; else zn[pr] = n; }
                 if (lane == 0) {
                     const float2 n = z[dr16(8)];
                     if (!MERGE) nyq[(f - f_begin) * NP + pr] = make_float2(n.x * un_a, n.y * un_b);
@@ -462,6 +479,8 @@
                 }
                 const float thr_a = PairBalance::thr(4e-30f, pb.na, alive_a), thr_b = PairBalance::thr(4e-30f, pb.nb, alive_b);
                 const float half_a = PairBalance::down(0.5f, pb.na, alive_a), half_b = PairBalance::down(0.5f, pb.nb, alive_b);
+                float4 Bu = make_float4(0.f, 0.f, 0.f, 0.f);
+                if (FUSE) { const float2 ba = Yl[64 * STEER_Y_BASE], bb = Yl[64 * (STEER_Y_BASE + 1)]; Bu = steer_base(make_float4(ba.x, ba.y, bb.x, bb.y), un_a, un_b); }
 #pragma unroll
                 for (int s = 0; s < 8; ++s) {
                     const float2 zk = z[dr16(s)], zm = z[dr16(15 - s < 12 ? 15 - s + 4 : 15 - s - 4)];
@@ -470,8 +489,20 @@
                     float pwa, pwb;
                     Xh[2 * pr][s] = whiten4<NOPHAT>(a2, pwa, thr_a, half_a);
                     Xh[2 * pr + 1][s] = whiten4<NOPHAT>(b2, pwb, thr_b, half_b);
-                }
-            }
+                    if (FUSE) {
+                        float2 y = pr == 0 ? make_float2(0.f, 0.f) : Yl[64 * s];
+                        if (s == 0) y = steer_mac<true>(y, a2, b2, Bu, a2, b2);
+                        else { const float4 qq = reinterpret_cast<const float4 *>(Qs)[pr * 7 + s - 1]; y = steer_mac<false>(y, a2, b2, Bu, make_float2(qq.x, qq.y), make_float2(qq.z, qq.w)); }
+                        if (pr < NP - 1) Yl[64 * s] = y;
+                        else yrow[(unsigned)lam + 64 * s] = s == 0 ? steer_dc(y, lane) : y;
+                    }
+                }
+            }
+            if (FUSE) {
+#pragma unroll
+                for (int pr = 0; pr < NP - 1; ++pr) zn[pr] = Yl[64 * (STEER_Y_ZN + pr)];
+            }
+            if (FUSE && lane == 0) yrow[FFT_H] = make_float2(steer_nyquist<NP>(zn, snyq), 0.f);
             if (p.dead && lane == 0) p.dead[(long long)a * p.total_frames + p.frame0 + f] = any_alive ? 0 : 1;
             OutT *arow = reinterpret_cast<OutT *>(p.A) + (row_base + f) * (long long)p.a_row_elems;
             if (MERGE) {
@@ -577,6 +608,195 @@
                 cand_unit<4>(p.cand, li - p.list0, e_unit, reinterpret_cast<unsigned char *>(wbase), tid);
             }
         }
+    }
+}
+
+__global__ __launch_bounds__(64) void k_steer_table(float4 *rows, float2 *q, float *nyq, const float *grid, const double *mic_x, int M, double unit)
+{
+    const int d = blockIdx.x, pr = blockIdx.y, lane = threadIdx.x, lam = lane <= 32 ? lane : 96 - lane;
+    const double doa = d == 0 ? 0.0 : (double)grid[d - 1];
+    const double cd = cos(doa + 1.57079632679489661923);
+    const double sc = 1.0 / ((double)M * 1024.0);
+    auto phasor = [&](int c, int k, double &cs, double &sn) {
+        double turns = (double)k * (unit * mic_x[c] * cd);
+        turns -= rint(turns);
+        sincospi(2.0 * turns, &sn, &cs);
+    };
+    double ca, sa, cb, sb;
+    phasor(2 * pr, lam, ca, sa); phasor(2 * pr + 1, lam, cb, sb);
+    rows[((long long)d * gridDim.y + pr) * 64 + lane] = make_float4((float)(ca * sc), (float)(sa * sc), (float)(cb * sc), (float)(sb * sc));
+    if (lane < 16) {
+        const int c = 2 * pr + (lane >> 3), s = lane & 7;
+        double cs, sn;
+        phasor(c, 64 * s, cs, sn);
+        q[((long long)d * M + c) * 8 + s] = make_float2((float)cs, (float)sn);
+    }
+    if (lane < 2) {
+        double cs, sn;
+        phasor(2 * pr + lane, 512, cs, sn);
+        nyq[d * M + 2 * pr + lane] = (float)(cs * sc);
+    }
+}
+
+__global__ __launch_bounds__(256, 2) void k_steer_patch(SteerPatchArgs p)
+{
+    constexpr int NP = 4, MT = 8;
+    extern __shared__ __attribute__((aligned(16))) unsigned char smem_raw[];
+    float2 *tab = reinterpret_cast<float2 *>(smem_raw);
+    const int tid = threadIdx.x, lane = tid & 63, wave = __builtin_amdgcn_readfirstlane(tid >> 6);
+    float2 *buf = tab + F1K_TWORDS + wave * F1K_SCRATCH;
+    const int npass = p.f1 - p.f0, stride = 4 * (int)gridDim.x;
+    int work = p.all;
+    if (!work) {
+        for (int a = 0; a < p.n_arrays; ++a) {
+            const int pred = p.bf.pred[a];
+            for (int fo = (int)blockIdx.x * 4 + wave + stride * lane; fo < npass; fo += stride * 64)
+                work |= p.doa_bin[(long long)a * p.n_frames + p.f0 + fo] != pred;
+        }
+    }
+    if (!__syncthreads_or(work)) return;
+    f1k_table_init(tab, tid, 256);
+    F1kLane lc;
+    lc.init(lane);
+    __syncthreads();
+    const int lam = lane <= 32 ? lane : 96 - lane;
+    const bool self = (lane & 31) == 0;
+    v2f win[8];
+#pragma unroll
+    for (int i = 0; i < 8; ++i) { win[i].x = p.window[lane + 128 * i]; win[i].y = p.window[lane + 128 * i + 64]; }
+    for (int a = 0; a < p.n_arrays; ++a) {
+        const int pred = __builtin_amdgcn_readfirstlane(p.bf.pred[a]);
+        const bool every = p.all != 0;
+        int missed = 0;
+        for (int fo = (int)blockIdx.x * 4 + wave; fo < npass; fo += stride) {
+            const int f = p.f0 + fo;
+            const int bin = __builtin_amdgcn_readfirstlane(p.doa_bin[(long long)a * p.n_frames + f]);
+            if (bin != pred) ++missed;
+            else if (!every) continue;
+            const float4 *srow = p.bf.rows + (long long)(bin + 1) * (NP * 64);
+            const float2 *qrow = p.bf.q + (long long)(bin + 1) * (MT * 8);
+            const float *base = p.pcm + (long long)a * p.array_stride + (long long)f * FFT_H;
+            float2 *yrow = p.bf.Y + ((long long)a * p.y_frames + f - p.y_f0) * STEER_ROW;
+            float xa[16], xb[16];
+            auto load_pair = [&](int pr) {
+                const float *pa = base + (long long)(2 * pr) * p.mic_stride, *pb = pa + p.mic_stride;
+#pragma unroll
+                for (int i = 0; i < 16; ++i) { xa[i] = pa[(unsigned)lane + 64 * i]; xb[i] = pb[(unsigned)lane + 64 * i]; }
+            };
+            load_pair(0);
+            float2 Y[8], zn[NP];
+#pragma unroll
+            for (int pr = 0; pr < NP; ++pr) {
+                float2 z[16];
+                float4 B;
+#pragma unroll
+                for (int i = 0; i < 8; ++i) { z[2 * i] = win_lo(xa[2 * i], xb[2 * i], win[i]); z[2 * i + 1] = win_hi(xa[2 * i + 1], xb[2 * i + 1], win[i]); }
+                float ma = max3abs(z[0].x, z[1].x, z[2].x), mb = max3abs(z[0].y, z[1].y, z[2].y);
+#pragma unroll
+                for (int i = 3; i < 15; i += 2) { ma = max3abs(ma, z[i].x, z[i + 1].x); mb = max3abs(mb, z[i].y, z[i + 1].y); }
+                ma = max2abs(ma, z[15].x); mb = max2abs(mb, z[15].y);
+                const PairBalance pb = pair_balance(ma, mb);
+                if (pb.scaled()) {
+                    const float sa = pb.sa(), sb = pb.sb();
+#pragma unroll
+                    for (int i = 0; i < 16; ++i) z[i] = make_float2(z[i].x * sa, z[i].y * sb);
+                }
+                fft1024c<false, 3>(z, buf, lane, tab, lc, [&]() {
+                    B = (srow + pr * 64)[(unsigned)lane];
+                    if (pr < NP - 1) load_pair(pr + 1);
+                }, lam);
+                const float un_a = pb.un_a(), un_b = pb.un_b();
+                zn[pr] = make_float2(z[dr16(8)].x * un_a, z[dr16(8)].y * un_b);
+                const float4 Bu = steer_base(B, un_a, un_b);
+                if (lane == 0) {
+                    float2 t[16];
+#pragma unroll
+                    for (int j = 0; j < 16; ++j) t[j] = z[dr16(j)];
+#pragma unroll
+                    for (int j = 8; j < 16; ++j) z[dr16(j < 12 ? j + 4 : j - 4)] = t[(j + 1) & 15];
+                } else if (self) {
+#pragma unroll
+                    for (int j = 8; j < 12; ++j) { const float2 t = z[dr16(j)]; z[dr16(j)] = z[dr16(j + 4)]; z[dr16(j + 4)] = t; }
+                } else {
+#pragma unroll
+                    for (int j = 8; j < 12; ++j) {
+                        float2 &u = z[dr16(j)], &w = z[dr16(j + 4)];
+                        swap_rows32(u.x, w.x); swap_rows32(w.x, u.x);
+                        swap_rows32(u.y, w.y); swap_rows32(w.y, u.y);
+                    }
+                }
+#pragma unroll
+                for (int s = 0; s < 8; ++s) {
+                    const float2 zk = z[dr16(s)], zm = z[dr16(15 - s < 12 ? 15 - s + 4 : 15 - s - 4)];
+                    const float2 a2 = make_float2(zk.x + zm.x, zk.y - zm.y);
+                    const float2 b2 = make_float2(zk.y + zm.y, zm.x - zk.x);
+                    const float2 y = pr == 0 ? make_float2(0.f, 0.f) : Y[s];
+                    if (s == 0) Y[s] = steer_mac<true>(y, a2, b2, Bu, a2, b2);
+                    else Y[s] = steer_mac<false>(y, a2, b2, Bu, qrow[(2 * pr) * 8 + s], qrow[(2 * pr + 1) * 8 + s]);
+                }
+                wave_lds_fence();
+            }
+#pragma unroll
+            for (int s = 0; s < 8; ++s) yrow[(unsigned)lam + 64 * s] = s == 0 ? steer_dc(Y[s], lane) : Y[s];
+            if (lane == 0) yrow[FFT_H] = make_float2(steer_nyquist<NP>(zn, p.bf.nyq + (bin + 1) * MT), 0.f);
+        }
+        if (missed && lane == 0) { atomicAdd(p.miss, (unsigned long long)missed); if (pred >= 0) atomicAdd(p.miss + 1, (unsigned long long)missed); }
+    }
+}
+
+__global__ __launch_bounds__(256) void k_steer_synth(SteerSynthArgs p)
+{
+    extern __shared__ __attribute__((aligned(16))) unsigned char smem_raw[];
+    float2 *tab = reinterpret_cast<float2 *>(smem_raw);
+    const int tid = threadIdx.x, lane = tid & 63, wave = __builtin_amdgcn_readfirstlane(tid >> 6);
+    float2 *buf = tab + F1K_TWORDS + wave * F1K_SCRATCH;
+    f1k_table_init(tab, tid, 256);
+    F1kLane lc;
+    lc.init(lane);
+    __syncthreads();
+    const int a = blockIdx.y;
+    if (p.pred_out && blockIdx.x == 0 && tid == 0) p.pred_out[a] = p.doa_bin[(long long)a * p.n_frames + p.n_frames - 1];
+    if (p.report && blockIdx.x == 0 && a == 0 && tid == 0) {
+        const unsigned long long tot = p.miss_total[1];
+        p.report[0] = tot - p.miss_total[2];
+        p.miss_total[2] = tot;
+        __hip_atomic_store(&p.report[1], p.seq, __ATOMIC_RELEASE, __HIP_MEMORY_SCOPE_SYSTEM);
+    }
+    const int t0 = p.f0 + ((int)blockIdx.x * 4 + wave) * p.ft, t1 = min(t0 + p.ft, p.f1);
+    if (t0 >= t1) return;
+    const float2 *Yb = p.Y + ((long long)a * p.y_frames - p.y_f0) * STEER_ROW;
+    float *ob = p.out + (long long)a * p.n_frames * FFT_H;
+    float carry[8];
+    if (t0 == p.f0) {
+#pragma unroll
+        for (int i = 0; i < 8; ++i) carry[i] = p.tail_in[(long long)a * FFT_H + lane + 64 * i];
+    }
+    int t = t0 > p.f0 ? t0 - 1 : t0;
+    float2 yv[8], nv[8];
+    float yn, nn = 0.f;
+#pragma unroll
+    for (int i = 0; i < 8; ++i) yv[i] = Yb[(long long)t * STEER_ROW + (unsigned)lane + 64 * i];
+    yn = Yb[(long long)t * STEER_ROW + FFT_H].x;
+    for (; t < t1; ++t) {
+        float2 y[16];
+        steer_inverse(y, yv, yn, buf, lane, tab, lc, [&]() {
+            if (t + 1 < t1) {
+#pragma unroll
+                for (int i = 0; i < 8; ++i) nv[i] = Yb[(long long)(t + 1) * STEER_ROW + (unsigned)lane + 64 * i];
+                nn = Yb[(long long)(t + 1) * STEER_ROW + FFT_H].x;
+            }
+        });
+        if (t >= t0) {
+#pragma unroll
+            for (int i = 0; i < 8; ++i) ob[(long long)t * FFT_H + (unsigned)lane + 64 * i] = carry[i] + y[dr16(i)].x;
+        }
+#pragma unroll
+        for (int i = 0; i < 8; ++i) { carry[i] = y[dr16(i + 8)].x; yv[i] = nv[i]; }
+        yn = nn;
+    }
+    if (t1 == p.f1) {
+#pragma unroll
+        for (int i = 0; i < 8; ++i) p.tail_out[(long long)a * FFT_H + lane + 64 * i] = carry[i];
     }
 }
 
@@ -774,6 +994,7 @@
 template __global__ void k_stft_phat_wave<8, true, _Float16, false, false, false, true>(StftPhatArgs);
 template __global__ void k_stft_phat_wave<8, true, _Float16, false, true, false, true>(StftPhatArgs);
 template __global__ void k_stft_phat_wave<4, true, _Float16, false, false, false, true>(StftPhatArgs);
+template __global__ void k_stft_phat_wave<8, true, _Float16, false, false, false, true, false, true>(StftPhatArgs);
 template __global__ void k_stft_phat_wave<4, true, _Float16, false, true, false, true>(StftPhatArgs);
 template __global__ void k_stft_phat_wave<8, true, _Float16, true, false, false, false, true>(StftPhatArgs);
 template __global__ void k_stft_phat_wave<8, false, _Float16, true, false, false, false, true>(StftPhatArgs);
diff --git a/mcarray_amd/csrc/mca_internal.h b/mcarray_amd/csrc/mca_internal.h
--- a/mcarray_amd/csrc/mca_internal.h
+++ b/mcarray_amd/csrc/mca_internal.h
@@ -45,6 +45,38 @@
     float *hist_C; int hist_base;
 };
 
+constexpr int STEER_QWORDS = 8 * 7;
+constexpr int STEER_LDS_ROWS = 13;
+constexpr int STEER_Y_ZN = 8, STEER_Y_BASE = 11;
+constexpr int STEER_MISS_NUM = 1, STEER_MISS_DEN = 3;
+constexpr int STEER_ROW = 520;
+struct SteerArgs {
+    const float4 *rows;
+    const float2 *q;
+    const float *nyq;
+    const int *pred;
+    float2 *Y;
+};
+constexpr int STEER_PATCH_WGS = 512;
+struct SteerPatchArgs {
+    const float *pcm; long long array_stride, mic_stride;
+    int n_arrays, n_frames;
+    int f0, f1;
+    const float *window;
+    const int *doa_bin;
+    SteerArgs bf;
+    int y_f0, y_frames;
+    int all;
+    unsigned long long *miss;
+};
+struct SteerSynthArgs {
+    const float2 *Y; int n_frames, f0, f1, ft, y_f0, y_frames;
+    float *out;
+    const float *tail_in; float *tail_out;
+    const int *doa_bin; int *pred_out;
+    unsigned long long *report; unsigned long long seq; unsigned long long *miss_total;
+};
+
 struct StftPhatArgs {
     const float *pcm;
     long long array_stride, mic_stride;
@@ -66,6 +98,7 @@
     unsigned char *dead;
     unsigned char *unsure;
     int cand_on; CandArgs cand;
+    SteerArgs bf;
 };
 
 __device__ __forceinline__ void store_a(float *row, const StftPhatArgs &, int cidx, float2 v)
diff --git a/mcarray_amd/csrc/steer.h b/mcarray_amd/csrc/steer.h
--- /dev/null
+++ b/mcarray_amd/csrc/steer.h
@@ -0,0 +1,40 @@
+#pragma once
+#include "fft1024c.h"
+
+namespace mca {
+
+__device__ __forceinline__ float4 steer_base(float4 B, float un_a, float un_b)
+{
+    const float2 a = cscale(make_float2(B.x, B.y), un_a), b = cscale(make_float2(B.z, B.w), un_b);
+    return make_float4(a.x, a.y, b.x, b.y);
+}
+template <bool FIRST>
+__device__ __forceinline__ float2 steer_mac(float2 y, float2 a2, float2 b2, float4 B, float2 qa, float2 qb)
+{
+    if (!FIRST) { a2 = cmul(a2, qa); b2 = cmul(b2, qb); }
+    y = cmac(y, a2, make_float2(B.x, B.y));
+    return cmac(y, b2, make_float2(B.z, B.w));
+}
+__device__ __forceinline__ float2 steer_dc(float2 y0, int lane) { return cscale(y0, lane == 0 ? 0.5f : 1.f); }
+
+template <int NP>
+__device__ __forceinline__ float steer_nyquist(const float2 (&zn)[NP], const float *pn)
+{
+    float yn = 0.f;
+#pragma unroll
+    for (int pr = 0; pr < NP; ++pr) yn = fmaf(zn[pr].y, pn[2 * pr + 1], fmaf(zn[pr].x, pn[2 * pr], yn));
+    return yn;
+}
+
+template <typename Mid = F1kNoMid>
+__device__ __forceinline__ void steer_inverse(float2 (&y)[16], const float2 (&yv)[8], float yn, float2 *buf, int lane, const float2 *tab, const F1kLane &lc, Mid mid = Mid())
+{
+#pragma unroll
+    for (int i = 0; i < 8; ++i) { y[i] = yv[i]; y[i + 8] = make_float2(0.f, 0.f); }
+    fft1024c<true, 3>(y, buf, lane, tab, lc, mid);
+    const float sn = (lane & 1) ? -yn : yn;
+#pragma unroll
+    for (int i = 0; i < 16; ++i) y[i].x += sn;
+}
+
+}
```

Result: faster. 56.66 million frames/s (median of 6 runs) (+16.8%).
